# facebookresearch/robust_cvd

Hardware: AMD Instinct MI355X
Metric: GN/LM iterations/sec (and ms/iter) on 300-frame 384x224 video, 1/2/4/8 GPU (higher is better)
Workload: dtype f64

## Files before the change

include/cvd_hip_debug.h:

```cpp
#ifndef CVD_HIP_DEBUG_H
#define CVD_HIP_DEBUG_H

#include "cvd_hip.h"

#ifdef __cplusplus
extern "C" {
#endif

typedef struct cvd_debug_options {
  uint64_t struct_size;
  int32_t force_iterations;
  int32_t force_sharded_path;
  int32_t pcg_lockstep;
  int32_t stall_fused_tail_once;
  int32_t tail_no_row_staging;
  int32_t tail_closes_scalars;
  int32_t asm_force_stage_depth;
  int32_t asm_force_part_units;
} cvd_debug_options;
void cvd_debug_options_default(cvd_debug_options* o);
int32_t cvd_set_debug_options(cvd_handle* h, const cvd_debug_options* o);

int32_t cvd_set_generic_kernels(cvd_handle* h, int32_t enabled);

int32_t cvd_comm_init_local_group(cvd_handle* h, int32_t rank, int32_t world, uint64_t group_key);
int32_t cvd_comm_init_phantom(cvd_handle* h, int32_t rank, int32_t world);

int32_t cvd_block_inverse_debug(cvd_handle* h, int32_t num_blocks, int32_t block_size, const double* a, int32_t variant,
                                float* inverse, int32_t* failed);

int32_t cvd_epipolar_debug(cvd_handle* h, int32_t num_pairs, const int64_t* offsets, const float* loc, double pixel_scale,
                           double threshold_px, int32_t iterations, uint64_t seed, uint8_t* is_static_out,
                           double* fundamental_out, int32_t* best_out, int32_t* counts_out, double* hypotheses_out);
int32_t cvd_flow_masks_debug(cvd_handle* h, int32_t num_frames, int32_t height, int32_t width, int32_t channels,
                             const float* color, int32_t num_pairs, const int32_t* pair_frames, const float* flow_ab,
                             const float* flow_ba, float flow_thresh, float color_thresh, uint8_t* mask_ab, uint8_t* mask_ba,
                             int32_t* kept, float* errors, double* kernel_ms, int32_t pixels_per_thread);
int32_t cvd_dense_inverse_debug(cvd_handle* h, int32_t n, const double* a, double* inverse, int32_t* failed);
int32_t cvd_coarse_debug(cvd_handle* h, int32_t* num_unknowns, double* a_c, double* a_c_inverse, int32_t* failed);
int32_t cvd_temporal_debug(cvd_handle* h, int32_t* dims6, double* a_t, double* a_t_inverse, double* lam, int32_t* failed);
int32_t cvd_product_launch_debug(cvd_handle* h, int32_t* out6);
int32_t cvd_assembly_launch_debug(cvd_handle* h, int32_t* out8, double* cost_frame);

#ifdef __cplusplus
}
#endif
#endif
```

robust_cvd_amd/api.py:

```python
import collections
import ctypes as C
import os
import sys

from . import build as _build
from .binding import Binding
from .ctypes_types import OptParams, SolveSummary, XformDesc

_lib = None
_variant = None


class SolverOptions(C.Structure):
    _fields_ = [
        ("struct_size", C.c_uint64),
        ("pcg_relative_tolerance", C.c_double),
        ("pcg_max_iterations", C.c_int32),
        ("verbose", C.c_int32),
        ("coarse_level", C.c_int32),
        ("robust_loss", C.c_int32),
        ("dense_matrix_free", C.c_int32),
        ("block_inverse_variant", C.c_int32),
        ("coarse_dense_max_unknowns", C.c_int32),
        ("coarse_rebuild_excess", C.c_int32),
        ("coarse_update_budget", C.c_int64),
        ("coarse_dense_shift", C.c_double),
        ("constraint_order", C.c_int32),
        ("coarse_rebuild_excess_dense", C.c_int32),
        ("pcg_fused_tail", C.c_int32),
        ("coarse_dense_row_split", C.c_int32),
        ("dist_owner_update", C.c_int32),
        ("temporal_level", C.c_int32),
        ("temporal_step", C.c_int32),
        ("temporal_grid_x", C.c_int32),
        ("temporal_grid_y", C.c_int32),
        ("coarse_temporal_step", C.c_int32),
        ("coarse_over_budget", C.c_int32),
        ("coarse_temporal_min_frames", C.c_int32),
        ("temporal_weight", C.c_double),
    ]


class DebugOptions(C.Structure):
    _fields_ = [
        ("struct_size", C.c_uint64),
        ("force_iterations", C.c_int32),
        ("force_sharded_path", C.c_int32),
        ("pcg_lockstep", C.c_int32),
        ("stall_fused_tail_once", C.c_int32),
        ("tail_no_row_staging", C.c_int32),
        ("tail_closes_scalars", C.c_int32),
        ("asm_force_stage_depth", C.c_int32),
        ("asm_force_part_units", C.c_int32),
    ]


class ConsistencyDesc(C.Structure):
    _fields_ = [
        ("struct_size", C.c_uint64),
        ("precision", C.c_int32),
        ("num_frames", C.c_int32),
        ("num_pairs", C.c_int32),
        ("height", C.c_int32),
        ("width", C.c_int32),
        ("distance_type", C.c_int32),
        ("have_warp", C.c_int32),
        ("reserved", C.c_int32),
        ("lambda_reprojection", C.c_double),
        ("lambda_disparity", C.c_double),
        ("lambda_depth_ratio", C.c_double),
        ("distance_scale", C.c_double),
        ("distance_alpha", C.c_double),
    ]


class SceneFlowDesc(C.Structure):
    _fields_ = [
        ("struct_size", C.c_uint64),
        ("precision", C.c_int32),
        ("num_frames", C.c_int32),
        ("num_pairs", C.c_int32),
        ("height", C.c_int32),
        ("width", C.c_int32),
        ("distance_type_static", C.c_int32),
        ("distance_type_smooth", C.c_int32),
        ("have_warp", C.c_int32),
        ("lambda_static", C.c_double),
        ("lambda_smooth_reprojection", C.c_double),
        ("lambda_smooth_disparity", C.c_double),
        ("lambda_smooth_depth_ratio", C.c_double),
        ("distance_scale", C.c_double),
        ("distance_alpha", C.c_double),
    ]


class SpatialDesc(C.Structure):
    _fields_ = [
        ("struct_size", C.c_uint64),
        ("precision", C.c_int32),
        ("num_frames", C.c_int32),
        ("frames_per_sample", C.c_int32),
        ("height", C.c_int32),
        ("width", C.c_int32),
        ("reserved", C.c_int32),
        ("lambda_disparity_smooth", C.c_double),
        ("sigma_color_grad", C.c_double),
        ("lambda_contrast_loss", C.c_double),
        ("contrast_thresh", C.c_double),
    ]


class ParamDesc(C.Structure):
    _fields_ = [
        ("struct_size", C.c_uint64),
        ("precision", C.c_int32),
        ("num_tensors", C.c_int32),
    ]


class ParamRecord(C.Structure):
    _fields_ = [
        ("beta1", C.c_double),
        ("beta2", C.c_double),
        ("eps", C.c_double),
        ("grad_decay", C.c_double),
        ("param_decay", C.c_double),
        ("step", C.c_double),
        ("denom_scale", C.c_double),
        ("rule", C.c_int32),
        ("reserved", C.c_int32),
    ]


class DatasetDesc(C.Structure):
    _fields_ = [
        ("struct_size", C.c_uint64),
# ... 2245 lines not shown
                          + [(C.c_void_p * n)(*[d.value for d in group]) for group in outs],
                          ([(dgx, gx)] if input_gradient else []) + [(d, a) for group, arrays in zip(outs, (gw, gg, gb))
                                                                     for d, a in zip(group, arrays)])
        return gx, gw, gg, gb

    def midas_backbone(self, images, weights, norms, blocks=RESNEXT101_32X8D[0], groups=RESNEXT101_32X8D[1],
                       width_per_group=RESNEXT101_32X8D[2], eps=RESNEXT_EPS, kernel_ms=None):
        import numpy as np
        images = np.asarray(images)
        weights = [np.asarray(a) for a in weights]
        norms = [[np.asarray(a) for a in four] for four in norms]
        self._midas_f32("midas_backbone", [images] + weights + [a for four in norms for a in four])
        B, H, W, table, out_shapes = resnext_check_backbone(images.shape, blocks, groups, width_per_group, [a.shape for a in weights],
                                                            [[a.shape for a in four] for four in norms], eps)
        outs = [np.zeros(s, np.float32) for s in out_shapes]
        n = len(table)
        with _DeviceArrays() as dev:
            di = dev.upload(np.ascontiguousarray(images))
            dw = (C.c_void_p * n)(*[dev.upload(np.ascontiguousarray(a)).value for a in weights])
            dn = (C.c_void_p * (4 * n))(*[dev.upload(np.ascontiguousarray(a)).value for four in norms for a in four])
            douts = [dev.alloc(o.nbytes) for o in outs]
            do = (C.c_void_p * 4)(*[d.value for d in douts])
            args = (self._h, C.c_int32(B), C.c_int32(H), C.c_int32(W), (C.c_int32 * 4)(*[int(b) for b in blocks]), C.c_int32(groups),
                    C.c_int32(width_per_group), C.c_float(eps), di, dw, dn, do, None)
            if kernel_ms is None:
                self._check(self._fn("midas_backbone_device")(*args))
            else:
                ms = (C.c_double * (2 * n + 1))()
                self._check(self._fn("midas_backbone_timed")(*args, ms))
                kernel_ms[:] = list(ms)
            if _hip_runtime().hipDeviceSynchronize() != 0:
                raise RuntimeError("midas_backbone: the device reported an error")
            for d, o in zip(douts, outs):
                dev.download(d, o)
        return outs

    def num_active_constraints(self):
        return int(self._lib.cvd_num_active_constraints(self._h))

    def block_inverse_debug(self, blocks, variant=0):
        import numpy as np
        a = np.ascontiguousarray(blocks, dtype=np.float64)
        n, B, B2 = a.shape
        assert B == B2
        out = np.zeros((n, B, B), dtype=np.float32)
        fl = C.c_int32(0)
        self._check(self._fn("block_inverse_debug")(self._h, C.c_int32(n), C.c_int32(B), a.ctypes.data_as(C.POINTER(C.c_double)),
                                                    C.c_int32(variant), out.ctypes.data_as(C.POINTER(C.c_float)), C.byref(fl)))
        return out, fl.value

    def dense_inverse_debug(self, a):
        import numpy as np
        a = np.ascontiguousarray(a, dtype=np.float64)
        n = a.shape[0]
        assert a.shape == (n, n)
        out = np.zeros((n, n), dtype=np.float64)
        fl = C.c_int32(0)
        self._check(self._fn("dense_inverse_debug")(self._h, C.c_int32(n), a.ctypes.data_as(C.POINTER(C.c_double)),
                                                    out.ctypes.data_as(C.POINTER(C.c_double)), C.byref(fl)))
        return out, fl.value

    def temporal_debug(self):
        import numpy as np
        dims = (C.c_int32 * 6)()
        self._check(self._fn("temporal_debug")(self._h, dims, None, None, None, None))
        if dims[0] == 0:
            return None
        n = dims[0]
        a = np.zeros((n, n))
        ai = np.zeros((n, n))
        lam = np.zeros(self.num_frames * self.block_size())
        fl = C.c_int32(0)
        dp = lambda x: x.ctypes.data_as(C.POINTER(C.c_double))
        self._check(self._fn("temporal_debug")(self._h, dims, dp(a), dp(ai), dp(lam), C.byref(fl)))
        return {"NT": n, "S": dims[1], "nn": dims[2], "step": dims[3], "Sx": dims[4], "Sy": dims[5], "a_t": a, "a_t_inverse": ai,
                "lam": lam, "failed": fl.value}

    def path_info(self):
        out = (C.c_int32 * 8)()
        self._check(self._fn("path_info")(self._h, out))
        form = {-1: "none", 0: "exact sparse factor", 1: "exact dense inverse", 2: "temporal pose level"}[out[1]]
        return {"pose_graph_level": form, "depth_grid_level": bool(out[2]), "fused_tail": bool(out[3] & 1), "tail_rows_staged": bool(out[3] & 2),
                "product_sums_shares": bool(out[3] & 4), "rz_shares": out[3] >> 8,
                "tail_disabled": bool(out[4]),
                "taps": out[5], "work_items": out[6], "cross_blocks": bool(out[7])}

    def product_launch_debug(self):
        out = (C.c_int32 * 6)()
        self._check(self._fn("product_launch_debug")(self._h, out))
        kind = {-1: "none", 0: "generic list", 1: "fast list", 2: "fast dense", 3: "cross blocks"}[out[3]]
        return {"threads": out[0], "spec": out[1], "kd": out[2], "kind": out[3], "kind_name": kind, "work_items": out[4],
                "num_cu": out[5]}

    def assembly_launch_debug(self):
        import numpy as np
        out = (C.c_int32 * 8)()
        cost = np.zeros(self.num_frames, dtype=np.float64)
        self._check(self._fn("assembly_launch_debug")(self._h, out, cost.ctypes.data_as(C.POINTER(C.c_double))))
        kind = {-1: "none", 0: "generic", 1: "fast list", 2: "fast dense", 3: "dense fold"}[out[3]]
        return {"threads": out[0], "spec": out[1], "kd": out[2], "kind": out[3], "kind_name": kind, "workgroups": out[4],
                "split_parts": out[5], "stage_depth": out[6], "segments": out[7], "cost_frame": cost}

    def coarse_debug(self):
        import numpy as np
        n = C.c_int32(0)
        self._check(self._fn("coarse_debug")(self._h, C.byref(n), None, None, None))
        if n.value == 0:
            return None
        a = np.zeros((n.value, n.value))
        ai = np.zeros((n.value, n.value))
        fl = C.c_int32(0)
        self._check(self._fn("coarse_debug")(self._h, C.byref(n), a.ctypes.data_as(C.POINTER(C.c_double)),
                                             ai.ctypes.data_as(C.POINTER(C.c_double)), C.byref(fl)))
        return {"a_c": a, "a_c_inverse": ai, "failed": fl.value}
```

robust_cvd_amd/csrc/cvd_api.hip:

```cpp
#include "cvd_host.h"
#include "cvd_coarse.h"

namespace cvd {

static void poseOptimizationStep(cvd_handle* h, const cvd_opt_params& p, double depthDeformReg) {
  solve(h, p, depthDeformReg, PK_POSE_STEP);
  paramsToPoses(h, p);
}

static void poseOptimization(cvd_handle* h, const cvd_opt_params& p) {
  posesToParams(h);
  h->records.clear();
  int ctfRows = p.ctf_long, ctfCols = p.ctf_short;
  int dsoRows = p.dso_long, dsoCols = p.dso_short;
  if (h->aspect >= 1.f) {
    std::swap(ctfCols, ctfRows);
    std::swap(dsoCols, dsoRows);
  }
  int initGrid[3] = {1, 1, 1};
  if (h->ddesc.depth_type == CVD_DEPTH_GRID)
    for (int i = 0; i < 3; ++i) initGrid[i] = h->ddesc.grid_size[i];
  const int Nval = (h->ddesc.depth_type == CVD_DEPTH_IDENTITY) ? 0 : valueNumParams(h->ddesc.value_xform);
  size_t nDmax = static_cast<size_t>(h->nD());
  if (p.coarse_to_fine && h->ddesc.depth_type != CVD_DEPTH_IDENTITY && p.num_steps > 1)
// ... 175 lines not shown
  p->focal_reg = 1.0;
  p->coarse_to_fine = 1;
  p->ctf_long = 17;
  p->ctf_short = 10;
  p->dso_long = 4;
  p->dso_short = 3;
  p->focal_long = 0.3461538376301239;
  p->intr_opt = CVD_INTR_PER_FRAME;
  p->normalize_depth_from_first_frame = 1;
}

void cvd_solver_options_default(cvd_solver_options* o) {
  o->struct_size = CVD_STRUCT_STAMP(cvd_solver_options);
  o->pcg_relative_tolerance = 1e-3;
  o->pcg_max_iterations = 300;
  o->verbose = 0;
  o->coarse_level = 1;
  o->robust_loss = 0;
  o->dense_matrix_free = 0;
  o->block_inverse_variant = 0;
  o->coarse_dense_max_unknowns = 4096;
  o->coarse_rebuild_excess = 16;
  o->coarse_update_budget = 40000;
  o->coarse_dense_shift = 1e-5;
  o->constraint_order = 1;
  o->coarse_rebuild_excess_dense = 0;
  o->pcg_fused_tail = 1;
  o->coarse_dense_row_split = 5;
  o->dist_owner_update = 1;
  o->temporal_level = 1;
  o->temporal_step = 32;
  o->temporal_grid_x = 0;
  o->temporal_grid_y = 0;
  o->coarse_temporal_step = 8;
  o->coarse_over_budget = 0;
  o->coarse_temporal_min_frames = 128;
  o->temporal_weight = 0.7;
}
int32_t cvd_set_solver_options(cvd_handle* h, const cvd_solver_options* o) {
  CVD_TRY(h, {
    if (o->struct_size != CVD_STRUCT_STAMP(cvd_solver_options))
      throw std::runtime_error(fmt("cvd_solver_options: struct_size %#llx != %#llx = sizeof | revision << 32 (caller built against "
                                   "another cvd_hip.h; start from cvd_solver_options_default)",
                                   static_cast<unsigned long long>(o->struct_size),
                                   static_cast<unsigned long long>(CVD_STRUCT_STAMP(cvd_solver_options))));
    if (o->pcg_fused_tail < 0 || o->pcg_fused_tail > 1) throw std::runtime_error("pcg_fused_tail in {0, 1}");
    if (!(o->pcg_relative_tolerance > 0.0 && o->pcg_relative_tolerance < 1.0)) throw std::runtime_error("pcg_relative_tolerance must lie in (0, 1)");
    if (o->pcg_max_iterations < 1) throw std::runtime_error("pcg_max_iterations must be >= 1");
    if (!(o->coarse_dense_shift >= 0.0 && o->coarse_dense_shift < 1.0)) throw std::runtime_error("coarse_dense_shift must lie in [0, 1)");
    if (o->coarse_rebuild_excess < 0 || o->coarse_rebuild_excess_dense < -1 || o->coarse_update_budget < 0)
      throw std::runtime_error("coarse_rebuild_excess / coarse_update_budget must be >= 0, coarse_rebuild_excess_dense >= -1");
    if (o->coarse_dense_max_unknowns < 0 || o->coarse_dense_max_unknowns > kDenseCoarseMaxUnknowns)
      throw std::runtime_error(fmt("coarse_dense_max_unknowns must lie in [0, %d] (what k_dense_spd_inverse holds in registers)",
                                   kDenseCoarseMaxUnknowns));
    if (o->coarse_level < 0 || o->coarse_level > 3 || o->coarse_temporal_step < 2 || o->robust_loss < 0 || o->robust_loss > 1 || o->block_inverse_variant < 0 ||
        o->block_inverse_variant > 2)
      throw std::runtime_error("coarse_level in {0, 1, 2, 3}, coarse_temporal_step >= 2, robust_loss in {0, 1}, block_inverse_variant in {0, 1, 2}");
    if (o->coarse_over_budget < 0 || o->coarse_over_budget > 1) throw std::runtime_error("coarse_over_budget in {0, 1}");
    if (o->coarse_temporal_min_frames < 0) throw std::runtime_error("coarse_temporal_min_frames must be >= 0");
    if (!(o->temporal_weight > 0.0 && o->temporal_weight <= 2.0)) throw std::runtime_error("temporal_weight must lie in (0, 2]");
    if (o->coarse_dense_row_split < 0 || o->coarse_dense_row_split > 8) throw std::runtime_error("coarse_dense_row_split must lie in [0, 8]");
    if (o->temporal_level < 0 || o->temporal_level > 2 || o->temporal_step < 2 || o->temporal_grid_x < 0 || o->temporal_grid_y < 0 ||
        o->temporal_grid_x == 1 || o->temporal_grid_y == 1)
      throw std::runtime_error("temporal_level in {0, 1, 2}, temporal_step >= 2, temporal_grid_x / _y 0 (automatic) or >= 2");
    if (o->coarse_update_budget != h->opt.coarse_update_budget || o->coarse_dense_max_unknowns != h->opt.coarse_dense_max_unknowns ||
        (o->coarse_level == 3) != (h->opt.coarse_level == 3) || o->coarse_temporal_step != h->opt.coarse_temporal_step ||
        o->coarse_over_budget != h->opt.coarse_over_budget || o->coarse_temporal_min_frames != h->opt.coarse_temporal_min_frames ||
        o->pcg_fused_tail != h->opt.pcg_fused_tail)
      h->tableValid = false;
    if (o->constraint_order != h->opt.constraint_order) h->orderGx = h->orderGy = -1;
    h->opt = *o;
  });
}
void cvd_debug_options_default(cvd_debug_options* o) {
  o->struct_size = CVD_STRUCT_STAMP(cvd_debug_options);
  o->force_iterations = 0;
  o->force_sharded_path = 0;
  o->pcg_lockstep = 0;
  o->stall_fused_tail_once = 0;
  o->tail_no_row_staging = 0;
  o->tail_closes_scalars = 0;
  o->asm_force_stage_depth = 0;
  o->asm_force_part_units = 0;
}
int32_t cvd_set_debug_options(cvd_handle* h, const cvd_debug_options* o) {
  CVD_TRY(h, {
    if (o->struct_size != CVD_STRUCT_STAMP(cvd_debug_options))
      throw std::runtime_error("cvd_debug_options: struct_size does not match this library's cvd_hip_debug.h (start from cvd_debug_options_default)");
    if (o->asm_force_stage_depth < 0 || o->asm_force_stage_depth > 3) throw std::runtime_error("asm_force_stage_depth in {0, 1, 2, 3}");
    if (o->asm_force_part_units < 0) throw std::runtime_error("asm_force_part_units >= 0");
    if (o->asm_force_part_units != h->dbg.asm_force_part_units) h->tableValid = false;
    h->dbg = *o;
    h->distForced = h->world == 1 && (h->comm != nullptr || h->localGroup || h->phantom) && o->force_sharded_path != 0;
  });
}
void cvd_comm_unique_id(uint8_t* out128) {
  ncclUniqueId id;
  std::memset(&id, 0, sizeof(id));
  (void)ncclGetUniqueId(&id);
  std::memcpy(out128, &id, sizeof(id));
}
int32_t cvd_comm_init(cvd_handle* h, int32_t rank, int32_t world, const uint8_t* id128) {
  CVD_TRY(h, {
    if (world < 1 || rank < 0 || rank >= world) throw std::runtime_error("invalid rank / world size");
    if (h->comm) { NCCL_CHECK(ncclCommDestroy(h->comm)); h->comm = nullptr; }
    ncclUniqueId id;
    std::memcpy(&id, id128, sizeof(id));
    NCCL_CHECK(ncclCommInitRank(&h->comm, world, id, rank));
    h->rank = rank;
    h->world = world;
    h->localGroup.reset();
    h->distForced = world == 1 && h->dbg.force_sharded_path != 0;
    h->tableValid = false;
  });
}
int32_t cvd_comm_init_local_group(cvd_handle* h, int32_t rank, int32_t world, uint64_t group_key) {
  CVD_TRY(h, {
    if (world < 1 || rank < 0 || rank >= world) throw std::runtime_error("invalid rank / world size");
    if (h->comm) { NCCL_CHECK(ncclCommDestroy(h->comm)); h->comm = nullptr; }
    h->localGroup = joinLocalGroup(group_key, world);
    h->rank = rank;
    h->world = world;
    h->distForced = world == 1 && h->dbg.force_sharded_path != 0;
    h->tableValid = false;
  });
}
int32_t cvd_comm_init_phantom(cvd_handle* h, int32_t rank, int32_t world) {
  CVD_TRY(h, {
    if (world < 1 || rank < 0 || rank >= world) throw std::runtime_error("invalid rank / world size");
    if (h->comm) { NCCL_CHECK(ncclCommDestroy(h->comm)); h->comm = nullptr; }
    if (h->localGroup) { leaveLocalGroup(*h->localGroup); h->localGroup.reset(); }
    h->phantom = true;
    h->rank = rank;
    h->world = world;
    h->distForced = world == 1;
    h->tableValid = false;
  });
}
int32_t cvd_set_generic_kernels(cvd_handle* h, int32_t enabled) { CVD_TRY(h, h->forceGeneric = enabled != 0); }

int32_t cvd_set_video(cvd_handle* h, int32_t numFrames, int32_t width, int32_t height, float aspect, float invAspect) {
  CVD_TRY(h, {
    if (numFrames <= 0 || width <= 0 || height <= 0) throw std::runtime_error("invalid video dimensions");
    h->F = numFrames; h->W = width; h->H = height; h->aspect = aspect; h->invAspect = invAspect;
    h->haveDynMasks = false;
    h->adaptGx = h->adaptGy = 0;
    h->dDepth.ensure(static_cast<size_t>(numFrames) * width * height);
    HIP_CHECK(hipMemsetAsync(h->dDepth.p, 0, static_cast<size_t>(numFrames) * width * height * sizeof(float), h->stream));
    h->median.assign(numFrames, 0.f);
    h->medianDirty = true;
    h->poses.assign(numFrames, cvd_frame_pose{{0, 0, 0}, {0, 0, 0, 1}, 0.f, 0.f});
    h->poseParamsValid = false;
    cvd_xform_desc dd{};
    dd.type = CVD_XFORM_DEPTH;
    dd.depth_type = CVD_DEPTH_IDENTITY;
    cvd_xform_desc sd{};
    sd.type = CVD_XFORM_SPATIAL;
    sd.spatial_type = CVD_SPATIAL_IDENTITY;
    resetXforms(h, dd, false);
    resetXforms(h, sd, true);
    h->tableValid = false;
    h->P = 0;
    h->C = 0;
    h->dense = false;
    h->denseListValid = false;
    h->haveTriplets = false;
// ... 732 lines not shown
    if (variant < 0 || variant > 2) throw std::runtime_error("block_inverse_debug: variant must be 0, 1 or 2");
    const size_t n = static_cast<size_t>(num_blocks) * block_size * block_size;
    DevBuf<double> dA;
    DevBuf<double> dL;
    DevBuf<float> dM;
    DevBuf<int> dF;
    dA.ensure(n);
    dL.ensure(static_cast<size_t>(num_blocks) * block_size);
    dM.ensure(n);
    dF.ensure(1);
    hipStream_t s = h->stream;
    dA.upload(a, n, s);
    HIP_CHECK(hipMemsetAsync(dL.p, 0, static_cast<size_t>(num_blocks) * block_size * sizeof(double), s));
    HIP_CHECK(hipMemsetAsync(dM.p, 0, n * sizeof(float), s));
    HIP_CHECK(hipMemsetAsync(dF.p, 0, sizeof(int), s));
    Layout L{};
    L.F = num_blocks;
    L.B = block_size;
    launchBlockInverseRaw(h, L, dA.p, dL.p, dM.p, dF.p, variant);
    int fl = 0;
    dM.download(inverse, n, s);
    dF.download(&fl, 1, s);
    HIP_CHECK(hipStreamSynchronize(s));
    if (failed) *failed = fl;
  });
}

int32_t cvd_epipolar_debug(cvd_handle* h, int32_t num_pairs, const int64_t* offsets, const float* loc, double pixel_scale,
                           double threshold_px, int32_t iterations, uint64_t seed, uint8_t* is_static_out,
                           double* fundamental_out, int32_t* best_out, int32_t* counts_out, double* hypotheses_out) {
  CVD_TRY(h, epipolarStaticFlags(h, num_pairs, offsets, loc, pixel_scale, threshold_px, iterations, seed, is_static_out,
                                 fundamental_out, best_out, nullptr, counts_out, hypotheses_out));
}

int32_t cvd_dense_inverse_debug(cvd_handle* h, int32_t n, const double* a, double* inverse, int32_t* failed) {
  CVD_TRY(h, {
    if (n <= 0 || n > 8192) throw std::runtime_error("dense_inverse_debug: bad size");
    const size_t nn = static_cast<size_t>(n) * n;
    DevBuf<double> dA;
    DevBuf<double> dM;
    DevBuf<int> dF;
    dA.ensure(nn);
    dM.ensure(nn);
    dF.ensure(2);
    hipStream_t s = h->stream;
    dA.upload(a, nn, s);
    HIP_CHECK(hipMemsetAsync(dM.p, 0, nn * sizeof(double), s));
    HIP_CHECK(hipMemsetAsync(dF.p, 0, 2 * sizeof(int), s));
    launchDenseSpdInverse(h, n, dA.p, dM.p, dF.p, s, dF.p + 1);
    int fl[2] = {0, 0};
    dM.download(inverse, nn, s);
    dF.download(fl, 2, s);
    HIP_CHECK(hipStreamSynchronize(s));
    if (failed) *failed = fl[0];
  });
}

int32_t cvd_temporal_debug(cvd_handle* h, int32_t* dims6, double* a_t, double* a_t_inverse, double* lam, int32_t* failed) {
  CVD_TRY(h, {
    auto& T = h->temporal;
    hipStream_t s = h->stream;
    const bool on = T.on && T.built;
    const int dims[6] = {on ? T.NT : 0, T.S, T.nn, T.step, T.Sx, T.Sy};
    for (int i = 0; i < 6; ++i) dims6[i] = dims[i];
    if (on) {
      const size_t n2 = static_cast<size_t>(T.NT) * T.NT;
      if (a_t) T.A.download(a_t, n2, s);
      if (a_t_inverse) T.Ainv.download(a_t_inverse, n2, s);
      if (lam) h->dLam.download(lam, static_cast<size_t>(h->F) * h->Bsz(), s);
      int fl = 0;
      T.fail.download(&fl, 1, s);
      HIP_CHECK(hipStreamSynchronize(s));
      if (failed) *failed = fl;
    }
  });
}
int32_t cvd_path_info(cvd_handle* h, int32_t* out8) {
  CVD_TRY(h, {
    out8[0] = h->coarseOn ? 1 : 0;
    out8[1] = !h->coarseOn ? -1 : (h->coarse.temporalPose ? 2 : (h->coarse.denseMode ? 1 : 0));
    out8[2] = h->temporal.on ? 1 : 0;
    out8[3] = h->lastFusedTail ? (h->tailStageRows ? 3 : 1) : 0;
    if (h->lastFusedTail && h->lastShares) out8[3] |= 4 | (h->lastShareCount << 8);
    out8[4] = h->tailDisabled ? 1 : 0;
    out8[5] = h->lastKD;
    out8[6] = static_cast<int32_t>(h->itemFa.size());
    out8[7] = h->lastCross ? 1 : 0;
  });
}
int32_t cvd_product_launch_debug(cvd_handle* h, int32_t* out6) {
  CVD_TRY(h, {
    for (int i = 0; i < 6; ++i) out6[i] = h->lastProduct[i];
  });
}
int32_t cvd_assembly_launch_debug(cvd_handle* h, int32_t* out8, double* cost_frame) {
  CVD_TRY(h, {
    for (int i = 0; i < 8; ++i) out8[i] = h->lastAssembly[i];
    const size_t F = static_cast<size_t>(h->F);
    if (cost_frame && h->lastAssembly[3] >= 0 && h->dCostFrame.n >= F) {
      h->dCostFrame.download(cost_frame, F, h->stream);
      HIP_CHECK(hipStreamSynchronize(h->stream));
    }
  });
}
int32_t cvd_coarse_debug(cvd_handle* h, int32_t* num_unknowns, double* a_c, double* a_c_inverse, int32_t* failed) {
  CVD_TRY(h, {
    auto& C = h->coarse;
    if (!C.valid || !h->coarseOn) {
      *num_unknowns = 0;
    } else if (C.temporalPose) {
      const size_t n = static_cast<size_t>(C.ptN);
      *num_unknowns = static_cast<int32_t>(n);
      hipStream_t s = h->stream;
      int fl = 0;
      C.fail.download(&fl, 1, s);
      if (a_c) C.ptMat.download(a_c, n * n, s);
      if (a_c_inverse) C.ptInv.download(a_c_inverse, n * n, s);
      HIP_CHECK(hipStreamSynchronize(s));
      if (failed) *failed = fl;
    } else {
      const int F = h->F;
      const size_t n = static_cast<size_t>(F) * kCB;
      *num_unknowns = static_cast<int32_t>(n);
      hipStream_t s = h->stream;
      int fl = 0;
      C.fail.download(&fl, 1, s);
      if (a_c_inverse) {
        std::vector<double> save(n), unit(n, 0.0);
        C.rc.download(save.data(), n, s);
        HIP_CHECK(hipStreamSynchronize(s));
        DevBuf<double> scalTmp;
        scalTmp.ensure(S_COUNT);
        HIP_CHECK(hipMemsetAsync(scalTmp.p, 0, S_COUNT * sizeof(double), s));
        for (size_t k = 0; k < n; ++k) {
          unit[k] = 1.0;
          C.rc.upload(unit.data(), n, s);
          if (C.denseMode) {
            hipLaunchKernelGGL(k_coarse_dense_apply, dim3(F), dim3(256), 0, s, F, C.denseInv.p, C.rc.p, C.c.p, C.modeActive.p,
                               C.dotPart.p, scalTmp.p, h->dCounters.p + 3, C.fail.p, 1, 0.0, static_cast<double*>(nullptr));
          } else {
            hipLaunchKernelGGL(k_coarse_apply_w, dim3(F), dim3(1024), 0, s, C.plan, C.Wb.p, C.rc.p, C.y.p, C.dotPart.p,
                               scalTmp.p, h->dCounters.p + 3, C.fail.p, 1, 0.0, static_cast<double*>(nullptr));
            hipLaunchKernelGGL(k_coarse_apply_wt, dim3(F), dim3(256), 0, s, coarseView(h, true, true), F, C.c.p,
                               scalTmp.p, 1);
          }
          C.c.download(a_c_inverse + k * n, n, s);
          HIP_CHECK(hipStreamSynchronize(s));
          unit[k] = 0.0;
        }
        C.rc.upload(save.data(), n, s);
        HIP_CHECK(hipStreamSynchronize(s));
      }
      std::vector<double> diag(static_cast<size_t>(F) * kCBB), edges(static_cast<size_t>(std::max(C.nEdges, 1)) * kCBB);
      std::vector<unsigned char> act(n);
      std::vector<int> efa(C.nEdges), efb(C.nEdges);
      C.diag.download(diag.data(), diag.size(), s);
      C.edges.download(edges.data(), static_cast<size_t>(C.nEdges) * kCBB, s);
      C.modeActive.download(act.data(), n, s);
      C.edgeFa.download(efa.data(), efa.size(), s);
      C.edgeFb.download(efb.data(), efb.size(), s);
      HIP_CHECK(hipStreamSynchronize(s));
      if (failed) *failed = fl;
      if (a_c) {
        std::fill(a_c, a_c + n * n, 0.0);
        for (int f = 0; f < F; ++f)
          for (int i = 0; i < kCB; ++i)
// ... 16 lines not shown
```

robust_cvd_amd/csrc/cvd_cost.h:

```cpp
#pragma once

#include "cvd_kernels.h"

namespace cvd {

template <int KD, int KS>
inline __global__ __launch_bounds__(256) void k_cost_items(Layout L, Table T, Items it, const double* __restrict__ x,
                                                    const FrameConst* __restrict__ fc, double* __restrict__ costItem) {
  extern __shared__ __attribute__((aligned(16))) double sm[];
  const int B = L.B;
  double* xa = sm;
  double* xb = sm + B;
  FrameConst* fcs = reinterpret_cast<FrameConst*>(sm + 2 * B);
  double* red = reinterpret_cast<double*>(fcs + 2);
  const int item = blockIdx.x;
  const int fa = it.fa[item], fb = it.fb[item];
  for (int i = threadIdx.x; i < B; i += blockDim.x) {
    xa[i] = x[static_cast<size_t>(fa) * B + i];
    xb[i] = x[static_cast<size_t>(fb) * B + i];
  }
  if (threadIdx.x < 2 * (sizeof(FrameConst) / 8)) {
    const int which = threadIdx.x / (sizeof(FrameConst) / 8);
    const int k = threadIdx.x % (sizeof(FrameConst) / 8);
    reinterpret_cast<double*>(fcs + which)[k] = reinterpret_cast<const double*>(fc + (which ? fb : fa))[k];
  }
  __syncthreads();
  double acc = 0.0;
  for (int dir = 0; dir < 2; ++dir) {
    const long long cb = it.range[item * 4 + dir * 2], ce = it.range[item * 4 + dir * 2 + 1];
    const FrameConst& Fs = fcs[dir];
    const FrameConst& Ft = fcs[dir ^ 1];
    const double* xs = dir ? xb : xa;
    const double* xt = dir ? xa : xb;
    for (long long c = cb + threadIdx.x; c < ce; c += blockDim.x) {
      const float2 d = T.dsrc[c];
      if (d.x > 0.f) {
        Sample<KD, KS> s;
        evalSample<KD, KS, false>(L, Fs, Ft, xs, xt, T.ndc[c], d, s);
        acc += s.rho0;
      }
    }
  }
  acc = waveSum(acc);
  if ((threadIdx.x & 63) == 0) red[threadIdx.x >> 6] = acc;
  __syncthreads();
  if (threadIdx.x == 0) {
    double t = 0.0;
    for (int w = 0; w < (blockDim.x >> 6); ++w) t += red[w];
    costItem[item] = 0.5 * t;
  }
}

template <int KD>
inline __global__ __launch_bounds__(256) void k_cost_frames(Layout L, const double* __restrict__ x,
                                                     const float* __restrict__ median,
                                                     const unsigned char* __restrict__ inRange,
                                                     const unsigned char* __restrict__ rangeFlags,
                                                     double* __restrict__ costFrame) {
  extern __shared__ __attribute__((aligned(16))) double sm[];
  __shared__ double red[4];
  const int f = blockIdx.x;
  double acc = 0.0;
  if (threadIdx.x == 0 && L.positionRegSqrt > 0.0) {
    double o3[3] = {0, 0, 0}, dg = 0.0, cst = 0.0;
    if (posRegValid(L, rangeFlags, f)) posRegFrame(L, rangeFlags, f, x, nullptr, o3, dg, cst);
    acc += cst;
  }
  const bool active = inRange[f] != 0;
  if (active)
    for (int i = threadIdx.x; i < L.B; i += 256) sm[i] = x[static_cast<size_t>(f) * L.B + i];
  __syncthreads();
  if (active) {
    const float med = median[f];
    const int nr = numRegResiduals<KD>(L);
    for (int i = threadIdx.x; i < nr; i += 256) {
      double r;
      int n;
      int cols[2 * KD + 2];
      double jac[2 * KD + 2];
      regResidual<KD>(L, f, i, sm, med, r, n, cols, jac);
      acc += r * r;
    }
  }
  acc = waveSum(acc);
  if ((threadIdx.x & 63) == 0) red[threadIdx.x >> 6] = acc;
  __syncthreads();
  if (threadIdx.x == 0) costFrame[f] = 0.5 * ((red[0] + red[1]) + (red[2] + red[3]));
}

inline __global__ __launch_bounds__(256) void k_sum2(const double* __restrict__ a, int na, const double* __restrict__ b,
                                              int nb, double* __restrict__ out, int slot) {
  __shared__ double red[4];
  double acc = 0.0;
  for (int i = threadIdx.x; i < na; i += 256) acc += a[i];
  for (int i = threadIdx.x; i < nb; i += 256) acc += b[i];
  acc = waveSum(acc);
  if ((threadIdx.x & 63) == 0) red[threadIdx.x >> 6] = acc;
  __syncthreads();
  if (threadIdx.x == 0) out[slot] = red[0] + red[1] + red[2] + red[3];
}

template <int KD, bool DENSE = false>
inline __global__ __launch_bounds__(256) void k_cost_items_fast(Layout L, Table T, Items it, const double* __restrict__ x,
                                                         const FrameConst* __restrict__ fc, double* __restrict__ costItem) {
  extern __shared__ __attribute__((aligned(16))) double sm[];
  const int B = L.B;
  double* xa = sm;
  double* xb = sm + B;
  FrameConst* fcs = reinterpret_cast<FrameConst*>(sm + 2 * B);
  double* red = reinterpret_cast<double*>(fcs + 2);
  const int item = blockIdx.x;
  const int tid = threadIdx.x;
  const int fa = it.fa[item], fb = it.fb[item];
  for (int i = tid; i < B; i += 256) {
    xa[i] = x[static_cast<size_t>(fa) * B + i];
    xb[i] = x[static_cast<size_t>(fb) * B + i];
  }
  constexpr int FCW = sizeof(FrameConst) / 8;
  if (tid < 2 * FCW) {
    const int which = tid / FCW, k = tid % FCW;
    reinterpret_cast<double*>(fcs + which)[k] = reinterpret_cast<const double*>(fc + (which ? fb : fa))[k];
  }
  __syncthreads();
  const int N = L.N;
  const double A = L.aspect;
  double acc = 0.0;
  for (int dir = 0; dir < 2; ++dir) {
    const long long cb = it.range[item * 4 + dir * 2], ce = it.range[item * 4 + dir * 2 + 1];
    const FrameConst& Fa = fcs[dir];
    const FrameConst& Fb = fcs[dir ^ 1];
    const double* xs = dir ? xb : xa;
    const double* xt = dir ? xa : xb;
    const double fya = Fa.fy, fxa = Fa.fy * A;
    const double fyb = Fb.fy;
    const double ifyb = 1.0 / fyb, ifxb = 1.0 / (fyb * A);
    const int fsrc = dir ? fb : fa, ftgt = dir ? fa : fb;
    const long long pixBase = DENSE ? (cb / (static_cast<long long>(T.W) * T.H)) * (static_cast<long long>(T.W) * T.H) : 0;
    std::conditional_t<DENSE, DenseStreamAhead, RecordStream<false>> rs;
    const int nDir = static_cast<int>(ce - cb);
    if constexpr (DENSE) rs.prime(T, cb, tid, 256, nDir, pixBase, fsrc, ftgt);
    else rs.prime(T, cb, tid, nDir);
    for (int ci = tid; ci < nDir; ci += 256) {
      float4 nd;
      float2 d;
      if (!rs.take(T, cb, ci, 256, nDir, pixBase, fsrc, ftgt, nd, d)) continue;
      const double da = static_cast<double>(d.x), db = static_cast<double>(d.y);
      double Da, Db;
      if (N == 0) {
        Da = da;
        Db = db;
      } else {
        FastTaps<KD> ta, tb;
        fastGather<KD>(L, nd.x, nd.y, ta);
        fastGather<KD>(L, nd.z, nd.w, tb);
        Da = 0.0;
        Db = 0.0;
#pragma unroll
        for (int k = 0; k < KD; ++k) {
          if (ta.ok(k)) {
            const int ia = ta.I(k);
            const double wa = ta.Wt(k);
            Da += (N == 2 ? da * xs[7 + ia * 2] + xs[7 + ia * 2 + 1] : da * xs[7 + ia]) * wa;
          }
          if (tb.ok(k)) {
            const int ib = tb.I(k);
            const double wb = tb.Wt(k);
            Db += (N == 2 ? db * xt[7 + ib * 2] + xt[7 + ib * 2 + 1] : db * xt[7 + ib]) * wb;
          }
        }
      }
      const double pax = static_cast<double>(nd.x), pay = static_cast<double>(nd.y);
      const double pbx = static_cast<double>(nd.z), pby = static_cast<double>(nd.w);
      double ca[3], Rca[3];
      fastRay(Fa.R, pax, pay, fxa, fya, ca, Rca);
      const double v[3] = {Fa.t[0] + Rca[0] * Da - Fb.t[0], Fa.t[1] + Rca[1] * Da - Fb.t[1], Fa.t[2] + Rca[2] * Da - Fb.t[2]};
      double zz, iz, u, vv, r0, r1, r2, dr2dA, dr2dDb;
      fastProject<false>(L, Fb.R, v, ifxb, ifyb, pbx, pby, zz, iz, u, vv, r0, r1);
      fastDepthResidual<false>(L, L.lossType, zz, iz, Db, r2, dr2dA, dr2dDb);
      double rho0, rho1;
      robustRho(L, r0 * r0 + r1 * r1 + r2 * r2, rho0, rho1);
      acc += rho0;
    }
  }
  acc = waveSum(acc);
  if ((tid & 63) == 0) red[tid >> 6] = acc;
  __syncthreads();
  if (tid == 0) costItem[item] = 0.5 * ((red[0] + red[1]) + (red[2] + red[3]));
}

inline __global__ __launch_bounds__(256) void k_step_stats(size_t n, const double* __restrict__ dx,
                                                    const double* __restrict__ g, const double* __restrict__ r,
                                                    const double* __restrict__ lam, const double* __restrict__ x,
                                                    const double* __restrict__ hdiagActive, double* __restrict__ scal,
                                                    double* __restrict__ part, unsigned int* __restrict__ counter) {
  constexpr int NQ = 7;
  __shared__ double red[NQ][4];
  __shared__ int flag;
  const int G = gridDim.x;
  double a[NQ] = {0, 0, 0, 0, 0, 0, 0};
  for (size_t i = static_cast<size_t>(blockIdx.x) * 256 + threadIdx.x; i < n; i += static_cast<size_t>(G) * 256) {
    const double d = dx[i];
    a[0] += d * g[i];
    a[1] += d * r[i];
    a[2] += d * lam[i] * d;
    a[3] += d * d;
    if (hdiagActive[i] != 0.0) { a[4] += x[i] * x[i]; a[6] += 1.0; }
    a[5] = fmax(a[5], fabs(g[i]));
  }
#pragma unroll
  for (int k = 0; k < NQ; ++k)
    if (k != 5) a[k] = waveSum(a[k]);
#pragma unroll
  for (int off = 32; off > 0; off >>= 1) a[5] = fmax(a[5], __shfl_xor(a[5], off, 64));
  if ((threadIdx.x & 63) == 0)
    for (int k = 0; k < NQ; ++k) red[k][threadIdx.x >> 6] = a[k];
  __syncthreads();
  if (threadIdx.x < NQ) {
    const int k = threadIdx.x;
    part[k * G + blockIdx.x] = (k != 5) ? (red[k][0] + red[k][1]) + (red[k][2] + red[k][3])
                                        : fmax(fmax(red[5][0], red[5][1]), fmax(red[5][2], red[5][3]));
  }
  if (!lastBlockArrives(counter, G, &flag)) return;
  double t[NQ] = {0, 0, 0, 0, 0, 0, 0};
  for (int b = threadIdx.x; b < G; b += 256) {
#pragma unroll
    for (int k = 0; k < NQ; ++k)
      if (k != 5) t[k] += part[k * G + b];
    t[5] = fmax(t[5], part[5 * G + b]);
  }
#pragma unroll
  for (int k = 0; k < NQ; ++k)
    if (k != 5) t[k] = waveSum(t[k]);
#pragma unroll
  for (int off = 32; off > 0; off >>= 1) t[5] = fmax(t[5], __shfl_xor(t[5], off, 64));
  if ((threadIdx.x & 63) == 0)
    for (int k = 0; k < NQ; ++k) red[k][threadIdx.x >> 6] = t[k];
  __syncthreads();
  if (threadIdx.x == 0) {
    scal[S_DG] = red[0][0] + red[0][1] + red[0][2] + red[0][3];
    scal[S_DR] = red[1][0] + red[1][1] + red[1][2] + red[1][3];
    scal[S_DLD] = red[2][0] + red[2][1] + red[2][2] + red[2][3];
    scal[S_DD] = red[3][0] + red[3][1] + red[3][2] + red[3][3];
    scal[S_XX] = red[4][0] + red[4][1] + red[4][2] + red[4][3];
    scal[S_GMAX] = fmax(fmax(red[5][0], red[5][1]), fmax(red[5][2], red[5][3]));
    scal[S_NACTIVE] = red[6][0] + red[6][1] + red[6][2] + red[6][3];
  }
}

}
```

robust_cvd_amd/csrc/cvd_eval.hip:

```cpp
#include "cvd_host.h"
#include "cvd_cost.h"
#include "cvd_assembly.h"
#include "cvd_triplets.h"
#include "cvd_dense_walk.h"

namespace cvd {

void launchFrameConsts(Ctx& c, const double* x) {
  launchFrameConsts(c.L, x, c.h->dFc.p, c.h->stream);
  HIP_CHECK(hipGetLastError());
}

void spinStream(hipStream_t s) {
  hipError_t e;
  while ((e = hipStreamQuery(s)) == hipErrorNotReady) {}
  HIP_CHECK(e);
}
void spinEvent(hipEvent_t ev) {
  hipError_t e;
  while ((e = hipEventQuery(ev)) == hipErrorNotReady) {}
  HIP_CHECK(e);
}
void readScalars(Ctx& c) {
  HIP_CHECK(hipMemcpyAsync(c.h->hScal, c.h->dScal.p, S_COUNT * sizeof(double), hipMemcpyDeviceToHost, c.h->stream));
  spinStream(c.h->stream);
}

void enqueueCost(Ctx& c, const double* x) {
  cvd_handle* h = c.h;
  hipStream_t s = h->stream;
  launchFrameConsts(c, x);
  const int slot = h->tBegin(KC_COST);
  if (c.L.includeStatic && c.nItems > 0) {
    const size_t lds = (2 * c.L.B) * 8 + 2 * sizeof(FrameConst) + 8 * 8;
    const bool fast = !h->forceGeneric && c.KS == 0 && fastLoss(c.L);
    if (fast) {
      CVD_DISPATCH_KD(c.KD, {
        if (h->dense) {
          allowLds((k_cost_items_fast<KD, true>), lds);
          hipLaunchKernelGGL((k_cost_items_fast<KD, true>), dim3(c.nItems), dim3(256), lds, s, c.L, c.T, c.it, x, h->dFc.p,
                             h->dCostItem.p);
        } else {
          allowLds((k_cost_items_fast<KD, false>), lds);
          hipLaunchKernelGGL((k_cost_items_fast<KD, false>), dim3(c.nItems), dim3(256), lds, s, c.L, c.T, c.it, x, h->dFc.p,
                             h->dCostItem.p);
        }
      });
    } else {
      CVD_DISPATCH(c.KD, c.KS, {
        allowLds(k_cost_items<KD, KS>, lds);
        hipLaunchKernelGGL((k_cost_items<KD, KS>), dim3(c.nItems), dim3(256), lds, s, c.L, c.T, c.it, x, h->dFc.p,
                           h->dCostItem.p);
      });
    }
    HIP_CHECK(hipGetLastError());
  }
  CVD_DISPATCH_KD(c.KD, {
    hipLaunchKernelGGL((k_cost_frames<KD>), dim3(c.L.F), dim3(256), static_cast<size_t>(c.L.B) * 8, s, c.L, x, h->dMedian.p, h->dRegOwner.p, h->dInRange.p,
                       h->dCostFrame.p);
  });
  HIP_CHECK(hipGetLastError());
  if (c.trip && c.TT.nGroups > 0) {
    CVD_DISPATCH(c.KD, c.KS, {
      hipLaunchKernelGGL((k_cost_triplets<KD, KS>), dim3(c.TT.nGroups), dim3(256), 0, s, c.L, c.TT, x, h->dFc.p,
                         h->dCostFrame.p);
    });
    HIP_CHECK(hipGetLastError());
  }
  hipLaunchKernelGGL(k_sum2, dim3(1), dim3(256), 0, s, h->dCostItem.p, (c.L.includeStatic ? c.nItems : 0),
                     h->dCostFrame.p, c.L.F, h->dScal.p, S_COST);
  HIP_CHECK(hipGetLastError());
  if (h->dist()) commAllReduce(h, h->dScal.p + S_COST, 1, CT_F64, s);
  h->tEnd(slot);
}
double evalCost(Ctx& c, const double* x) {
  enqueueCost(c, x);
  readScalars(c);
  return c.h->hScal[S_COST];
}

void enqueueStats(Ctx& c) {
  cvd_handle* h = c.h;
  const int G = static_cast<int>(std::min<size_t>(128, (c.n + 511) / 512));
  h->dStatPart.ensure(7 * 128);
  hipLaunchKernelGGL(k_step_stats, dim3(G), dim3(256), 0, h->stream, c.n, h->dDx.p, h->dG.p, h->dR.p, h->dLam.p,
                     h->dX.p, h->dHd.p, h->dScal.p, h->dStatPart.p, h->dCounters.p + 2);
  HIP_CHECK(hipGetLastError());
}

bool crossScope(cvd_handle* h, const Ctx& c) {
  const bool off = h->opt.dense_matrix_free != 0;
  return h->dense && !off && !h->forceGeneric && c.L.includeStatic && !h->xFa.empty() && c.KS == 0 && fastLoss(c.L) &&
         c.L.N == 1 && c.L.nD > 0 && (c.KD == 4 || (c.KD == 1 && c.L.nD == 1)) && c.L.intrOpt != CVD_INTR_SHARED && !c.trip && !(c.L.positionRegSqrt > 0.0) &&
         c.L.B <= 256 && (static_cast<size_t>(c.L.B) * (c.L.B + 1) / 2 + 2 * c.L.B + 4 * 36) * 8 <= kMaxLds &&
         dwLdsBytes(c.L.nD, c.L.B, kDwThreads) <= kMaxLds;
}
CrossPairs crossPairs(cvd_handle* h) {
  return CrossPairs{h->dXFa.p, h->dXFb.p, h->dXRange.p, h->dXSlot.p, static_cast<int>(h->xFa.size())};
}
DenseRecords denseRecords(cvd_handle* h) {
  return DenseRecords{h->dDwRecords.p, h->dDwRecOff.p, h->dFpOff.p, h->dFpList.p};
}
void launchDenseWalk(Ctx& c, const double* x) {
  cvd_handle* h = c.h;
  const int G = c.L.nD, B = c.L.B;
  h->dDwRecords.ensure(static_cast<size_t>(std::max(1, h->nDwRecords)) * dwRecordDoubles(G));
  h->dDwGg.ensure(static_cast<size_t>(std::max<long long>(1, h->C)));
  if (h->nDwRecords == 0) return;
  const size_t lds = dwLdsBytes(G, B, kDwThreads);
  const DenseWalkList wl{h->dDwPair.p, h->nDwRecords, denseLaneMap(h->W, h->H)};
  allowLds((k_dense_walk<4>), lds);
  const int slot = h->tBegin(KC_DENSE_WALK);
  hipLaunchKernelGGL((k_dense_walk<4>), dim3(h->nDwRecords), dim3(kDwThreads), lds, h->stream, c.L, c.T, wl, x, h->dFc.p,
                     h->dDwRecords.p, h->dDwGg.p);
  h->tEnd(slot);
  HIP_CHECK(hipGetLastError());
}
void launchCrossAssemble(Ctx& c, const double* x) {
  (void)x;
  cvd_handle* h = c.h;
  const size_t B = c.L.B, G = c.L.nD;
  h->dXBlocks.ensure(h->xFa.size() * B * B);
  const unsigned nP = static_cast<unsigned>(h->xFa.size());
  if (nP == 0) return;
  hipLaunchKernelGGL(k_dense_fold_cross, dim3(nP), dim3(256), 0, h->stream, c.L, crossPairs(h), h->dXDir.p, h->dDwRecOff.p,
                     h->dDwRecords.p, h->dXBlocks.p);
  int panelW = static_cast<int>(((kMaxLds - 4096) / 8) / G);
  panelW = std::max(1, std::min<int>(panelW, static_cast<int>(G)));
  const int nPanels = static_cast<int>((G + panelW - 1) / panelW);
  panelW = static_cast<int>((G + nPanels - 1) / nPanels);
  const size_t ldsGrid = static_cast<size_t>(panelW) * G * 8;
  allowLds((k_dense_gg<4>), ldsGrid);
  const int slot = h->tBegin(KC_DENSE_GG);
  for (int dir = 0; dir < 2; ++dir)
    hipLaunchKernelGGL((k_dense_gg<4>), dim3(nP, nPanels), dim3(kGgThreads), ldsGrid, h->stream, c.L, c.T, crossPairs(h), h->dXDir.p,
                       h->dDwGg.p, panelW, dir, h->dXBlocks.p);
  h->tEnd(slot);
  HIP_CHECK(hipGetLastError());
}

double evalFull(Ctx& c, const double* x, bool withStats, bool noReadBack) {
  cvd_handle* h = c.h;
  hipStream_t s = h->stream;
  launchFrameConsts(c, x);
  const size_t B = c.L.B;
  const int slot = h->tBegin(KC_ASSEMBLE);
  const bool fast = !h->forceGeneric && c.KS == 0 && fastLoss(c.L);
  const size_t ldsFast = (B * (B + 1) / 2 + 2 * B + 4 * 36) * 8;
  const size_t ldsRest = 3 * B * 8 + 2 * sizeof(FrameConst) + 4 * 36 * 8;
  int panelCap = 0;
  const bool fastFits = ldsFast <= kMaxLds;
  auto recordAsm = [h](int threads, int spec, int kd, int kind, int groups, int splitParts, int stageDepth = -1, int segments = 0) {
    const int v[8] = {threads, spec, kd, kind, groups, splitParts, stageDepth, segments};
    for (int i = 0; i < 8; ++i) h->lastAssembly[i] = v[i];
  };
  if (fast && fastFits) {
    h->dAsmScratch.ensure(static_cast<size_t>(h->nAsmSlots) * (B * (B + 1) / 2 + B + 4));
    const AsmWork work{h->dAsmParts.p, h->dAsmUnits.p, h->dAsmScratch.p, h->dAsmCount.p};
    const int spec = (!h->dense && c.L.N == 1 && c.L.lossType == CVD_STATIC_REPRO_DISPARITY && c.L.intrOpt != CVD_INTR_SHARED)
                         ? (c.L.robustKind == 0 ? 1 : 2) : 0;
    const size_t ldsRow = static_cast<size_t>(kAsmThreads / 64) * B * 8;
    const bool segWalk = spec != 0 && kAsmThreads > 64;
    int depth = ldsFast + ldsRow <= kMaxLds ? 1 : 0;
    if (segWalk && ldsFast + 2 * ldsRow <= kMaxLds) depth = 2;
    if (segWalk && h->dbg.asm_force_stage_depth != 0) {
      const int forced = h->dbg.asm_force_stage_depth - 1;
      if (forced < 0 || forced > 2 || ldsFast + forced * ldsRow > kMaxLds)
        throw std::runtime_error(fmt("asm_force_stage_depth: %d staging rows per wave do not fit the LDS at B = %d", forced, static_cast<int>(B)));
      depth = forced;
    }
    const size_t ldsStage = ldsFast + static_cast<size_t>(depth) * ldsRow;
    const bool stage = depth > 0;
    const AsmSegs segs{h->dAsmSegs.p, h->dAsmWaveOff.p, depth};
    if (segWalk && !h->dAsmWaveOff.p) throw std::logic_error("assembly: the segment list of the work list is missing");
#define CVD_LAUNCH_ASM_S(DENSEV, STAGEV, SPECV)                                                                            \
    CVD_DISPATCH_KD(c.KD, {                                                                                              \
      if (SPECV != 0 && kAsmThreads > 64) recordAsm(kAsmThreads, SPECV, KD, 1, h->nAsmParts, h->nAsmSlots, depth, h->nAsmSegs); \
      else recordAsm(kAsmThreads, SPECV, KD, DENSEV ? 2 : 1, h->nAsmParts, h->nAsmSlots);                                  \
      allowLds((k_assemble_fast<KD, DENSEV, STAGEV, false, SPECV>), STAGEV ? ldsStage : ldsFast);                          \
      hipLaunchKernelGGL((k_assemble_fast<KD, DENSEV, STAGEV, false, SPECV>), dim3(h->nAsmParts),                          \
                         dim3(kAsmThreads), STAGEV ? ldsStage : ldsFast, s,                                                \
                         c.L, c.T, x, h->dFc.p, h->dMask.p, h->dMedian.p, h->dRegOwner.p, h->dInRange.p, work, h->dG.p, h->dH.p,  \
                         h->dCostFrame.p, h->dFocal.p, h->dFocal.p + c.L.F, asmSegsAsArgument(segs));                    \
    })
#define CVD_LAUNCH_ASM(DENSEV, STAGEV) CVD_LAUNCH_ASM_S(DENSEV, STAGEV, 0)
#ifndef CVD_ASM_STAGE
#define CVD_ASM_STAGE 1
#endif
    if (c.cross) {
      launchDenseWalk(c, x);
      recordAsm(kAsmThreads, 0, c.KD, 3, c.L.F, 0);
      if (c.KD == 1) {
        allowLds((k_assemble_fast<1, true, false, true>), ldsFast);
        hipLaunchKernelGGL((k_assemble_fast<1, true, false, true>), dim3(c.L.F), dim3(kAsmThreads), ldsFast, s, c.L, c.T, x, h->dFc.p,
                           h->dMask.p, h->dMedian.p, h->dRegOwner.p, h->dInRange.p, work, h->dG.p, h->dH.p, h->dCostFrame.p,
                           h->dFocal.p, h->dFocal.p + c.L.F, denseRecords(h));
      } else {
        allowLds((k_assemble_fast<4, true, false, true>), ldsFast);
        hipLaunchKernelGGL((k_assemble_fast<4, true, false, true>), dim3(c.L.F), dim3(kAsmThreads), ldsFast, s, c.L, c.T, x, h->dFc.p,
                           h->dMask.p, h->dMedian.p, h->dRegOwner.p, h->dInRange.p, work, h->dG.p, h->dH.p, h->dCostFrame.p,
                           h->dFocal.p, h->dFocal.p + c.L.F, denseRecords(h));
      }
    } else if (h->dense) { if (stage && CVD_ASM_STAGE) CVD_LAUNCH_ASM(true, true); else CVD_LAUNCH_ASM(true, false); }
    else if (spec == 1) { if (stage && CVD_ASM_STAGE) CVD_LAUNCH_ASM_S(false, true, 1); else CVD_LAUNCH_ASM_S(false, false, 1); }
    else if (spec == 2) { if (stage && CVD_ASM_STAGE) CVD_LAUNCH_ASM_S(false, true, 2); else CVD_LAUNCH_ASM_S(false, false, 2); }
    else { if (stage && CVD_ASM_STAGE) CVD_LAUNCH_ASM(false, true); else CVD_LAUNCH_ASM(false, false); }
#undef CVD_LAUNCH_ASM
#undef CVD_LAUNCH_ASM_S
  } else {
    if (h->dense && c.L.includeStatic) throw std::logic_error("dense mode: the generic assembly has no images to read (DenseListScope should have taken this solve)");
    const AsmPanels panels = makePanels(static_cast<int>(B), (kMaxLds - ldsRest) / 8, panelCap);
    const size_t lds = static_cast<size_t>(panelCap) * 8 + ldsRest;
    recordAsm(256, 0, c.KD, 0, c.L.F, 0);
    CVD_DISPATCH(c.KD, c.KS, {
      allowLds(k_assemble<KD, KS>, lds);
      hipLaunchKernelGGL((k_assemble<KD, KS>), dim3(c.L.F), dim3(256), lds, s, c.L, c.T, x, h->dFc.p, h->dMask.p,
                         h->dMedian.p, h->dRegOwner.p, h->dInRange.p, h->dFpOff.p, h->dFpList.p, h->dG.p, h->dH.p, h->dCostFrame.p,
                       h->dFocal.p, h->dFocal.p + c.L.F, panels, panelCap);
    });
  }
  HIP_CHECK(hipGetLastError());
  if (c.trip && c.TT.nGroups > 0) {
    int panelCapT = 0;
    const AsmPanels panelsT = makePanels(static_cast<int>(B), (kMaxLds - B * 8 - 256) / 8, panelCapT);
    const size_t ldsT = (static_cast<size_t>(panelCapT) + B) * 8;
    CVD_DISPATCH(c.KD, c.KS, {
      allowLds(k_assemble_triplets<KD, KS>, ldsT);
      hipLaunchKernelGGL((k_assemble_triplets<KD, KS>), dim3(c.L.F), dim3(256), ldsT, s, c.L, c.TT, x, h->dFc.p,
                         h->dMask.p, h->dFtOff.p, h->dFtList.p, h->dG.p, h->dH.p, h->dFocal.p, h->dFocal.p + c.L.F,
                         panelsT, panelCapT);
      hipLaunchKernelGGL((k_cost_triplets<KD, KS>), dim3(c.TT.nGroups), dim3(256), 0, s, c.L, c.TT, x, h->dFc.p,
                         h->dCostFrame.p);
    });
    HIP_CHECK(hipGetLastError());
  }
  if (c.L.intrOpt == CVD_INTR_SHARED) {
    hipLaunchKernelGGL(k_shared_focal_fixup, dim3(1), dim3(256), 0, s, c.L, h->dFocal.p, h->dFocal.p + c.L.F, h->dMask.p,
                       h->dG.p, h->dH.p);
    HIP_CHECK(hipGetLastError());
  }
  if (c.cross) launchCrossAssemble(c, x);
  h->tEnd(slot);
  if (h->dist()) {
    const int ct = h->tBegin(KC_COMM_EVAL);
    const size_t chunkH = static_cast<size_t>(h->ownChunk()) * B * B;
    commGroupStart(h);
    commAllReduce(h, h->dG.p, c.n, CT_F64, s);
    commAllReduce(h, h->dCostFrame.p, c.L.F, CT_F64, s);
    commReduceScatter(h, h->dH.p, h->dH.p + static_cast<size_t>(h->rank) * chunkH, chunkH, CT_F64, s);
    commGroupEnd(h);
    Layout own = c.L;
    own.F = h->ownCount();
    if (own.F > 0)
      hipLaunchKernelGGL(k_extract_diag, dim3((static_cast<size_t>(own.F) * B + 255) / 256), dim3(256), 0, s, own,
                         h->dH.p + static_cast<size_t>(h->ownFirst()) * B * B, h->dHd.p + static_cast<size_t>(h->ownFirst()) * B);
    const size_t chunkD = static_cast<size_t>(h->ownChunk()) * B;
    commAllGather(h, h->dHd.p + static_cast<size_t>(h->rank) * chunkD, h->dHd.p, chunkD, CT_F64, s);
    h->tEnd(ct);
  } else {
    hipLaunchKernelGGL(k_extract_diag, dim3((c.n + 255) / 256), dim3(256), 0, s, c.L, h->dH.p, h->dHd.p);
  }
  hipLaunchKernelGGL(k_sum2, dim3(1), dim3(256), 0, s, h->dCostFrame.p, c.L.F, h->dCostFrame.p, 0, h->dScal.p, S_COST);
  HIP_CHECK(hipGetLastError());
  if (noReadBack) return 0.0;
  if (withStats) {
    HIP_CHECK(hipMemsetAsync(h->dLam.p, 0, c.n * sizeof(double), s));
    enqueueStats(c);
  }
  readScalars(c);
  return h->hScal[S_COST];
}

void touchModule_eval() {
  hipFuncAttributes a;
  (void)hipFuncGetAttributes(&a, reinterpret_cast<const void*>(k_sum2));
}

}

#ifdef CVD_ASM_PROFILE
extern "C" int32_t cvd_debug_asm_profile(unsigned long long* out) {
  (void)hipDeviceSynchronize();
  return hipMemcpyFromSymbol(out, HIP_SYMBOL(cvd::g_asmProf), sizeof(unsigned long long) * 2048 * 16) == hipSuccess ? 0 : 1;
}
extern "C" int32_t cvd_debug_asm_waits(unsigned long long* out) {
  (void)hipDeviceSynchronize();
  return hipMemcpyFromSymbol(out, HIP_SYMBOL(cvd::g_asmWait), sizeof(unsigned long long) * 2048 * 8 * 8) == hipSuccess ? 0 : 1;
}
#endif
```

robust_cvd_amd/csrc/cvd_host.h:

```cpp
#pragma once

#include <hip/hip_runtime.h>
#include <hip/hip_ext.h>
#include <rccl/rccl.h>
#include <rocblas/rocblas.h>
#include <rocsolver/rocsolver.h>

#include <algorithm>
#include <array>
#include <atomic>
#include <chrono>
#include <condition_variable>
#include <cmath>
#include <cstdarg>
#include <cstdint>
#include <cstdio>
#include <cstdlib>
#include <cstring>
#include <functional>
#include <limits>
#include <map>
#include <memory>
#include <mutex>
#include <set>
// ... 234 lines not shown
  bool tableIgnoresStatic = false;
  long long numValid = 0;

  std::vector<cvd_frame_pose> poses;
  cvd_xform_desc ddesc{}, sdesc{};
  std::vector<double> dparams, sparams;
  std::vector<std::array<double, 7>> poseParams;
  bool poseParamsValid = false;

  DevBuf<double> dX, dXc, dG, dLam, dMask, dScale, dDx, dR, dR1, dZ, dP0, dP1, dQ, dH, dQPart;
  DevBuf<float> dMinv;
  DevBuf<double> dFdot, dCostItem, dCostFrame, dScal, dHd, dFocal;
  DevBuf<double> dStatPart;
  DevBuf<unsigned char> dDynMask;
  DevBuf<double> dAdaptW;
  int dynW = 0, dynH = 0, adaptGx = 0, adaptGy = 0;
  bool haveDynMasks = false;
  std::shared_ptr<Frontend> frontend;

  struct CoarseHost {
    bool valid = false;
    int nEdges = 0, nBlocks = 0, nLevels = 0;
    std::vector<int> itemEdge;
    DevBuf<int> order, pos, levelPtr, levelCols, lvlBlkPtr, lvlBlks, blkCol, blkRow, colPtr, rowPtr, rowBlk, updPtr, updBlk,
        updA, updB, edgeBlk, edgeFa, edgeFb, wPtr, wRow, wtPtr, wtBlk, wtCol, wtFrame, wuPtr, wuL, wuW, itemEdgeDev, wSlot;
    DevBuf<double> edges, diag, Lb, Linv, Wb, rc, qc, y, c, dotPart, fdotY, wq, dropDiag;
    bool sparsified = false;
    bool temporalPose = false;
    int ptNn = 0, ptStepFrames = 0, ptN = 0, ptBlocks = 0;
    std::vector<int> edgeFaHost, edgeFbHost;
    DevBuf<int> ptA, ptB, ptPtr, ptList;
    DevBuf<double> ptMat, ptInv, ptR, ptT, ptDot, ptRec;
    DevBuf<TlStep> ptStepDev;
    std::vector<unsigned char> ptStepHost;
    DevBuf<unsigned int> ptCounter;
    bool denseMode = false;
    int denseForB = 0;
    bool denseReady = false;
    DevBuf<double> denseA, densePanel;
    DevBuf<double> denseInv;
    DevBuf<int> denseValid;
    int nW = 0;
    DevBuf<unsigned char> modeActive;
    DevBuf<int> fail;
    DevBuf<unsigned int> barrier;
    bool ptInvPending = false;
    int* ptInvFail = nullptr;
    DevBuf<double> Wb2;
    DevBuf<int> fail2;
    CoarsePlan plan{};
  } coarse;
  bool coarseOn = false;
  struct TemporalHost {
    bool on = false;
    bool built = false;
    int S = 0, Sx = 0, Sy = 0, nn = 0, step = 0, NT = 0, width = 0, nGroups = 0, nBlocks = 0;
    std::vector<unsigned char> stepHost;
    int tabGx = 0, tabGy = 0, tabSx = 0, tabSy = 0;
    int grpF = 0, grpStep = 0;
    std::vector<int> grpFa, grpFb;
    DevBuf<float> hx, hy, elW;
    DevBuf<int> bx, by, gOff, gItems, blkA, blkB, gPtr, gather, fail, valid;
    DevBuf<float4> vW;
    DevBuf<unsigned int> vIdx, counter;
    DevBuf<unsigned char> elV;
    DevBuf<double> Cf, E, part, A, Ainv, sq, rT, t, tl, dotPart, rec;
    DevBuf<double> invPanel;
    DevBuf<unsigned int> invBarrier;
    DevBuf<TlStep> stepDev;
    hipEvent_t evIn = nullptr, evDone = nullptr;
    bool sidePending = false;
    double* sqPtr = nullptr;
  } temporal;
  hipEvent_t evRebuild[2] = {nullptr, nullptr};
  bool rebuildTimed = false;
  double coarseRebuildMs = 0.0, pcgIterMs = 0.0;
  std::vector<std::pair<int, int>> globalEdges;
  bool haveGlobalEdges = false;
  DevBuf<double> dRegJac;
  DevBuf<unsigned short> dRegCol;
  DevBuf<unsigned char> dRegCnt;
  RegCache regCache{};
  DevBuf<FrameConst> dFc;
  DevBuf<int> dFail;
  DevBuf<unsigned long long> dCount;
  double* hScal = nullptr;
  double* hStage[2] = {nullptr, nullptr};
  size_t hStageN[2] = {0, 0};
  double* hPcg = nullptr;
  hipEvent_t pcgEvent[2] = {nullptr, nullptr};

  cvd_solve_summary summary{};
  std::vector<cvd_iteration_record> records;

  bool lastFusedTail = false, lastCross = false;
  bool lastShares = false;
  int lastShareCount = 0;
  int sharesF = -1, sharesN = -1;
  bool tailStageRows = false;
  int lastKD = 0;
  int lastProduct[6] = {0, 0, 0, -1, 0, 0};
  int lastAssembly[8] = {0, 0, 0, -1, 0, 0, -1, 0};
  bool tailDisabled = false;
  bool forceGeneric = false;

  int timing = 0;
  int timingStride = 1;
  long long timingCounter = 0;
  long long timingCounterKc[16] = {0};
  std::vector<std::pair<hipEvent_t, hipEvent_t>> evPool;
  std::vector<int> evClass;
  std::vector<int> evIter;
  int curPcgIter = -1;
  size_t evUsed = 0;
  double kcMs[KC_TOTAL] = {0};
  long long kcN[KC_TOTAL] = {0};

  ~cvd_handle_t() {
    for (auto& e : evPool) { (void)hipEventDestroy(e.first); (void)hipEventDestroy(e.second); }
    if (rbMain) (void)rocblas_destroy_handle(rbMain);
    if (comm) (void)ncclCommDestroy(comm);
    if (localGroup) leaveLocalGroup(*localGroup);
    if (hScal) (void)hipHostFree(hScal);
    for (auto& p : hStage) if (p) (void)hipHostFree(p);
    if (hPcg) (void)hipHostFree(hPcg);
    for (auto& e : pcgEvent) if (e) (void)hipEventDestroy(e);
    for (auto& e : evRebuild) if (e) (void)hipEventDestroy(e);
    if (temporal.evIn) (void)hipEventDestroy(temporal.evIn);
    if (temporal.evDone) (void)hipEventDestroy(temporal.evDone);
    if (evCoarseIn) (void)hipEventDestroy(evCoarseIn);
    if (evCoarseDone) (void)hipEventDestroy(evCoarseDone);
    if (evInvIn) (void)hipEventDestroy(evInvIn);
    if (evInvDone) (void)hipEventDestroy(evInvDone);
    if (stream3) (void)hipStreamDestroy(stream3);
    if (stream2) (void)hipStreamDestroy(stream2);
    if (stream) (void)hipStreamDestroy(stream);
  }

  int nD() const { return xformNumBlocks(ddesc) * xformBlockSize(ddesc); }
  int nS() const { return xformNumBlocks(sdesc) * xformBlockSize(sdesc); }
  int Bsz() const { return 7 + nD() + nS(); }

  int tBegin(int kc) {
    if (kc >= KC_COUNT ? timing == 0 : !(timing & (1 << kc))) return -1;
    if (timingStride > 1 && kc < KC_DENSE_WALK && (timingCounterKc[kc]++ % timingStride) != 0) return -1;
    if (evUsed == evPool.size()) {
      hipEvent_t a, b;
      HIP_CHECK(hipEventCreate(&a));
      HIP_CHECK(hipEventCreate(&b));
      evPool.emplace_back(a, b);
      evClass.push_back(kc);
      evIter.push_back(-1);
    }
    evClass[evUsed] = kc;
    evIter[evUsed] = curPcgIter;
    HIP_CHECK(hipEventRecord(evPool[evUsed].first, stream));
    return static_cast<int>(evUsed++);
  }
  void tEnd(int slot) {
    if (slot >= 0) HIP_CHECK(hipEventRecord(evPool[slot].second, stream));
  }
  int tReserve(int kc, hipEvent_t& start, hipEvent_t& stop) {
    start = nullptr;
    stop = nullptr;
    if (!(timing & (1 << kc))) return -1;
    if (timingStride > 1 && (timingCounter++ % timingStride) != 0) return -1;
    if (evUsed == evPool.size()) {
      hipEvent_t a, b;
      HIP_CHECK(hipEventCreate(&a));
      HIP_CHECK(hipEventCreate(&b));
      evPool.emplace_back(a, b);
      evClass.push_back(kc);
      evIter.push_back(-1);
    }
    evClass[evUsed] = kc;
    evIter[evUsed] = curPcgIter;
    start = evPool[evUsed].first;
    stop = evPool[evUsed].second;
    return static_cast<int>(evUsed++);
  }
  void tDropFrom(size_t firstSlot, int firstDeadIter) {
    for (size_t i = firstSlot; i < evUsed; ++i)
      if (evIter[i] >= firstDeadIter) evClass[i] = -1;
// ... 47 lines not shown
  } while (0)

#define CVD_DISPATCH_KD(KDv, ...)                                  \
  do {                                                             \
    if (KDv == 1) { constexpr int KD = 1; __VA_ARGS__; }            \
    else if (KDv == 4) { constexpr int KD = 4; __VA_ARGS__; }       \
    else { constexpr int KD = 16; __VA_ARGS__; }                    \
  } while (0)

constexpr size_t kMaxLds = 160 * 1024;

template <typename K>
void allowLds(K kernel, size_t bytes) {
  if (bytes > kMaxLds)
    throw std::runtime_error(fmt("per-frame block needs %zu B of LDS (> 160 KiB): frame block too large", bytes));
  if (bytes > 48 * 1024) {
    static std::map<std::pair<int, const void*>, size_t> granted;
    static std::mutex grantedMutex;
    int dev = 0;
    HIP_CHECK(hipGetDevice(&dev));
    std::lock_guard<std::mutex> lock(grantedMutex);
    size_t& g = granted[{dev, reinterpret_cast<const void*>(kernel)}];
    if (bytes > g) {
      HIP_CHECK(hipFuncSetAttribute(reinterpret_cast<const void*>(kernel), hipFuncAttributeMaxDynamicSharedMemorySize,
                                    static_cast<int>(bytes)));
      g = bytes;
    }
  }
}

int liveHandles(int device);
struct PersistentGate {
  static constexpr int kMaxDevices = 64;
  struct Slot { std::mutex m; hipEvent_t ev = nullptr; bool recorded = false; };
  static Slot& slot(int device);
  Slot& sl;
  hipStream_t s;
  PersistentGate(int device, hipStream_t stream) : sl(slot(device)), s(stream) {
    sl.m.lock();
    try {
      if (!sl.ev) HIP_CHECK(hipEventCreateWithFlags(&sl.ev, hipEventDisableTiming));
      if (sl.recorded) HIP_CHECK(hipStreamWaitEvent(s, sl.ev, 0));
    } catch (...) {
      sl.m.unlock();
      throw;
    }
  }
  ~PersistentGate() {
    sl.recorded = hipEventRecord(sl.ev, s) == hipSuccess;
    sl.m.unlock();
  }
};

void commAllReduce(cvd_handle* h, void* buf, size_t count, CommType t, hipStream_t s);
void commReduceScatter(cvd_handle* h, const void* send, void* recv, size_t recvCount, CommType t, hipStream_t s);
void commAllGather(cvd_handle* h, const void* send, void* recv, size_t sendCount, CommType t, hipStream_t s);
void commGroupStart(cvd_handle* h);
void commGroupEnd(cvd_handle* h);
std::vector<int> rangeOf(const cvd_opt_params& p, int F);
void posesToParams(cvd_handle* h);
void paramsToPoses(cvd_handle* h, const cvd_opt_params& params);
void resetXforms(cvd_handle* h, const cvd_xform_desc& d, bool spatial);
void gridXformSplit(cvd_handle* h, const cvd_xform_desc& nd);
Layout makeLayout(cvd_handle* h, const cvd_opt_params& p, double depthDeformReg, ProblemKind kind);
void checkFrameBlock(size_t B, const char* what);
void tapCounts(const Layout& L, int& KD, int& KS);
bool fastLoss(const Layout& L);
Table makeTable(cvd_handle* h);
void checkDenseScope(cvd_handle* h, const Layout& L, int KS, bool trip);
bool denseFastScope(const cvd_handle* h, const Layout& L, int KS, bool trip);
bool denseFastBlockFits(long long B);
struct DenseListScope {
  cvd_handle* h;
  bool entered = false;
  DenseListScope(cvd_handle* h, bool needList);
  ~DenseListScope();
};
bool denseModeSupported(const cvd_opt_params& p, const cvd_xform_desc& dd, const cvd_xform_desc& sd, bool haveTriplets, int world,
                        bool normalize);
AsmPanels makePanels(int B, size_t capDoubles, int& panelCap);
void compileTable(cvd_handle* h, const std::vector<int>& range, bool withTriplets = false, bool ignoreStatic = false);
void orderTable(cvd_handle* h, const Layout& L, int KD);
double* pinnedStage(cvd_handle* h, int which, size_t n);
void uploadState(cvd_handle* h, const Layout& L, DevBuf<double>& dst);
void downloadState(cvd_handle* h, const Layout& L, const DevBuf<double>& src);
void buildMask(cvd_handle* h, const Layout& L, const cvd_opt_params& p, ProblemKind kind, const std::vector<int>& range);
void ensureBuffers(Ctx& c);
void refreshMedians(cvd_handle* h);
void launchFrameConsts(const Layout& L, const double* x, FrameConst* fc, hipStream_t s);
void launchFrameConsts(Ctx& c, const double* x);
void launchFlagToBool(int* flag, hipStream_t s);
void launchTlRowsInit(cvd_handle* h, const TlStep* tsp, int NT, int groups, int F, unsigned int* counter, int closeScalars, double tol2,
                      hipStream_t s);
void spinStream(hipStream_t s);
void spinEvent(hipEvent_t ev);
void readScalars(Ctx& c);
void enqueueCost(Ctx& c, const double* x);
double evalCost(Ctx& c, const double* x);
void enqueueStats(Ctx& c);
bool crossScope(cvd_handle* h, const Ctx& c);
CrossPairs crossPairs(cvd_handle* h);
void launchCrossAssemble(Ctx& c, const double* x);
double evalFull(Ctx& c, const double* x, bool withStats = false, bool noReadBack = false);
bool coarseFusedConsumers();
bool fusedExchange(cvd_handle* h, bool withCoarse);
size_t exchangeOffsetQc(const Ctx& c);
size_t exchangeOffsetPq(const Ctx& c, bool withDenseCoarse);
size_t exchangeTemporalCount(cvd_handle* h, bool withCoarse);
bool ownerShardedUpdate(cvd_handle* h, bool withCoarse);
inline int denseRowSplit(const cvd_handle* h) { return std::min(kCB, std::max(0, h->opt.coarse_dense_row_split)); }
void launchDenseSpdInverse(cvd_handle* h, int n, const double* A, double* out, int* fail, hipStream_t s, int* outValid,
                           DevBuf<double>* panelBuf = nullptr, DevBuf<unsigned int>* barrierBuf = nullptr);
struct DinvRequest {
  int n = 0;
  const double* A = nullptr;
  double* out = nullptr;
  int* fail = nullptr;
  int* outValid = nullptr;
  DevBuf<double>* panelBuf = nullptr;
  DevBuf<unsigned int>* barrierBuf = nullptr;
};
void launchDenseSpdInversePair(cvd_handle* h, const DinvRequest& a, const DinvRequest& b, hipStream_t s);
CoarseView coarseView(cvd_handle* h, bool on, bool walk);
void prepareMatvec(Ctx& c, const double* x);
void launchMatvec(Ctx& c, const double* x, const double* z, const double* pOld, double* pNew, int useBeta, const double* lam,
                  double* q, bool withCoarse = false, bool tailFused = false, int sharesIteration = 0);
bool pcgTailScope(Ctx& c, bool coarse, int nThreads, size_t& lds, int& ldsFinish, int& ldsScratch);
struct PcgShares {
  int count = 0;
  int levelShare0 = 0;
  int levelWg0 = 0;
};
bool pcgSharesScope(Ctx& c, bool coarse, PcgShares& sh);
void launchPcgTail(Ctx& c, const double* x, const double* pOld, double* pNew, int useBeta, const double* lam, double* q,
                   bool withCoarse, int nThreads, size_t lds, int ldsFinish, int ldsScratch, double tol2,
                   const PcgShares* shares = nullptr);
void launchPcgClose(Ctx& c, int enqueued);
void launchBlockInverseRaw(cvd_handle* h, const Layout& L, const double* dH, const double* dLam, float* dMinv, int* dFail, int variant,
                           hipStream_t onStream = nullptr);
void launchBlockInverse(Ctx& c, hipStream_t onStream = nullptr);
void launchCoarseSetup(Ctx& c, const double* x, int side = 0);
bool temporalScope(const Ctx& c);
bool temporalPrepare(Ctx& c);
void launchTemporalSetup(Ctx& c, const double* x, int half);
void launchTemporalInit(Ctx& c, bool closeScalars, double tol2);
TlStep temporalStep(cvd_handle* h);
const TlStep* temporalStepDev(cvd_handle* h);
void poseTemporalPlan(cvd_handle* h);
void poseTemporalPrepare(Ctx& c);
void launchPoseTemporalBuild(Ctx& c, hipStream_t s, int* failOut, bool deferInverse = false);
void launchPoseTemporalInit(Ctx& c, double tol2);
const TlStep* poseTemporalStepDev(cvd_handle* h);
void coarseDebug(cvd_handle* h, int32_t* num_unknowns, double* a_c, double* a_c_inverse, int32_t* failed);
int runPcg(Ctx& c, const double* x, const std::function<void()>& tail = nullptr);
bool wantsTriplets(const cvd_opt_params& p, ProblemKind kind);
void bindTriplets(Ctx& c, const cvd_opt_params& p, ProblemKind kind);
void solve(cvd_handle* h, const cvd_opt_params& p, double depthDeformReg, ProblemKind kind);
void evaluate(cvd_handle* h, const cvd_opt_params& p, double depthDeformReg, const double* pose7, double* cost, int32_t* nres,
              double* gradient, double* hdiag, double* hfull);
void sampleConstraints(cvd_handle* h, bool triplet, int num, const int32_t* keyFrames, const float* corner, const float* flow,
                       const uint8_t* mask, const float* flow2, const uint8_t* mask2, const float* dyn, int dw, int dh,
                       int matchSeparation, float minDynamicDistance, int64_t* offsets);
void getSampledConstraints(cvd_handle* h, bool triplet, float* out);
void denseMaps(cvd_handle* h, int kind, int first, int count, int w, int hh, void* out, double* kernelMs);
void imageOps(cvd_handle* h, int kind, int n, int w, int hh, const void* in, float* out, double* kernelMs);
void touchModule_setup();
void touchModule_eval();
void touchModule_matvec();
void touchModule_precond();
void touchModule_solve();
void touchModule_frontend();
void touchModule_temporal();
void flowGuidedFilter(cvd_handle* h, int n, int first, int count, int w, int hh, int dw, int dh, float invAspect, const float* depth,
                      const float* cameras, const float* flowF, const uint8_t* maskF, const float* flowB, const uint8_t* maskB,
                      int frameRadius, int spatialRadius, int median, float* out, double* kernelMs);
void bilateralFilter(cvd_handle* h, int n, int first, int count, int w, int hh, const float* depth, const float* color,
                     int frameRadius, int spatialRadius, float depthSigma, float colorSigma, int median, float* out,
                     double* kernelMs);
void epipolarStaticFlags(cvd_handle* h, int numPairs, const int64_t* offsets, const float* loc, double pixelScale,
                         double thresholdPx, int iterations, uint64_t seed, uint8_t* isStatic, double* fundamental,
                         int32_t* best, double* kernelMs, int32_t* counts, double* hypotheses);
void computeTracks(cvd_handle* h, int F, int H, int W, float invAspect, const uint8_t* active, int first, int last,
                   const float* corner, const float* dyn, int dh, int dw, const float* flow, const uint8_t* mask,
                   const uint8_t* pairPresent, int spawnDistance, int pruneDistance, float minDynamicDistance,
                   int minTrackLength, int64_t* counts, double* kernelMs);
void getTracks(cvd_handle* h, int32_t* startFrame, int32_t* length, uint8_t* kept, float* loc);
void flowConsistencyMasks(cvd_handle* h, int numFrames, int hh, int w, int channels, const float* color, int numPairs,
                          const int32_t* pairFrames, const float* flowAB, const float* flowBA, float flowThresh,
                          float colorThresh, uint8_t* maskAB, uint8_t* maskBA, int32_t* kept, float* errors, double* kernelMs,
                          int pixelsPerThread);
void consistencyLoss(cvd_handle* h, const cvd_consistency_desc* d, const void* depth, const void* ext, const void* intr,
                     const void* warp, const int32_t* pairFrames, const void* flowAB, const void* flowBA, const void* weightAB,
                     const void* weightBA, double* total, double* terms, void* grad, double* kernelMs);
void consistencyLossDevice(cvd_handle* h, const cvd_consistency_desc* d, const void* depth, const void* ext, const void* intr,
                           const void* warp, const int32_t* pairFrames, const void* flowAB, const void* flowBA,
                           const void* weightAB, const void* weightBA, double* total, double* terms, void* grad, hipStream_t s);
void sceneFlowLoss(cvd_handle* h, const cvd_scene_flow_desc* d, const void* depth, const void* ext, const void* intr,
                   const void* warp, const int32_t* pairFrames, const void* const* flows, const void* const* masks,
                   const int32_t* neighborFrames, const void* const* nflows, const void* const* nmasks, const void* valid,
                   double* total, double* terms, void* grad, void* maps, double* kernelMs);
void sceneFlowLossDevice(cvd_handle* h, const cvd_scene_flow_desc* d, const void* depth, const void* ext, const void* intr,
                         const void* warp, const int32_t* pairFrames, const void* const* flows, const void* const* masks,
                         const int32_t* neighborFrames, const void* const* nflows, const void* const* nmasks, const void* valid,
                         double* total, double* terms, void* grad, void* maps, hipStream_t s);
void spatialLosses(cvd_handle* h, const cvd_spatial_desc* d, const void* depth, const void* depthOrig, const void* image,
                   double* total, double* smooth, double* contrast, void* grad, double* kernelMs);
void spatialLossesDevice(cvd_handle* h, const cvd_spatial_desc* d, const void* depth, const void* depthOrig, const void* image,
                         double* total, double* smooth, double* contrast, void* grad, hipStream_t s);
void parameterL1(cvd_handle* h, const cvd_param_desc* d, const int64_t* offsets, const int64_t* counts, int64_t flatCount,
                 const void* p, const void* p0, double lambda, double* total, void* grad, double gradOut, int accumulate,
                 double* kernelMs);
void parameterL1Device(cvd_handle* h, const cvd_param_desc* d, const void* const* p, const void* const* p0, const int64_t* counts,
                       double lambda, double* total, void* const* grad, const void* gradOut, int accumulate, hipStream_t s);
void paramStep(cvd_handle* h, const cvd_param_desc* d, const int64_t* offsets, const int64_t* counts, int64_t flatCount, void* p,
               const void* g, void* m, void* v, const cvd_param_record* records, double* kernelMs);
void paramStepDevice(cvd_handle* h, const cvd_param_desc* d, void* const* p, const void* const* g, void* const* m, void* const* v,
                     const int64_t* counts, const cvd_param_record* records, hipStream_t s);
long long paramChunkElements();
void datasetCreate(cvd_handle* h, const cvd_dataset_desc* d, const int32_t* pairFrames, const int32_t* samples);
void datasetClear(cvd_handle* h);
void datasetSetColors(cvd_handle* h, int first, int count, const float* hwc3);
void datasetSetFlows(cvd_handle* h, int first, int count, const float* flow, const uint8_t* mask);
void datasetSetDepthOrig(cvd_handle* h, int first, int count, const float* depth);
void datasetSetCameras(cvd_handle* h, const float* ext, const float* intr);
void datasetSetXforms(cvd_handle* h, const cvd_xform_desc* dd, const double* dparams, const cvd_xform_desc* sd, const double* sparams);
void datasetSetMaps(cvd_handle* h, const float* scales, int scaleIsMap, const float* warp);
void datasetBatchDevice(cvd_handle* h, int B, const int64_t* indices, const cvd_dataset_batch_out* out, hipStream_t s);
void datasetBatch(cvd_handle* h, int B, const int64_t* indices, const cvd_dataset_batch_out* out, double* kernelMs);
long long datasetBadIndices(cvd_handle* h);
void raftCorrPyramidDevice(cvd_handle* h, long long Q, int h2, int w2, int dim, int levels, const float* raw, float* const* level,
                           hipStream_t s);
void raftCorrLookupDevice(cvd_handle* h, int B, int h1, int w1, int h2, int w2, int levels, int radius, const float* const* level,
                          const float* coords, float* out, hipStream_t s);
void raftUpsampleFlowDevice(cvd_handle* h, int N, int H, int W, const float* flow, const float* mask, float* out, hipStream_t s);
void raftSepConvGruDevice(cvd_handle* h, int B, int H, int W, const float* hidden, int numSegments, const float* const* segments,
                          const int32_t* segmentChannels, const float* const* weights, const float* const* biases, float* out,
                          hipStream_t s, double* kernelMs);
// ... 72 lines not shown
```

robust_cvd_amd/csrc/cvd_matvec.hip:

```cpp
#include "cvd_host.h"
#include "cvd_pcg.h"
#include "cvd_cross.h"
#include "cvd_triplets.h"

namespace cvd {

bool coarseFusedConsumers() {
  return false;
}
bool fusedExchange(cvd_handle* h, bool withCoarse) { return !withCoarse || h->coarse.denseMode; }
size_t exchangeOffsetQc(const Ctx& c) { return c.h->dist() ? static_cast<size_t>(c.h->framesPadded()) * c.L.B : c.n; }
size_t exchangeOffsetPq(const Ctx& c, bool withDenseCoarse) {
  return exchangeOffsetQc(c) + (withDenseCoarse ? static_cast<size_t>(c.L.F) * kCB : 0);
}
size_t exchangeTemporalCount(cvd_handle* h, bool withCoarse) {
  const TlStep ts = temporalStep(h);
  return (ts.Ainv != nullptr && h->dist() && fusedExchange(h, withCoarse)) ? static_cast<size_t>(h->F) * ts.S : 0;
}
bool ownerShardedUpdate(cvd_handle* h, bool withCoarse) {
  return h->dist() && fusedExchange(h, withCoarse) && h->opt.dist_owner_update != 0;
}
CoarseView coarseView(cvd_handle* h, bool on, bool walk) {
  auto& C = h->coarse;
  CoarseView v = on ? CoarseView{C.pos.p, C.wPtr.p, C.wRow.p, walk ? C.Wb.p : nullptr, C.y.p, C.modeActive.p, C.fail.p, C.c.p}
                    : CoarseView{nullptr, nullptr, nullptr, nullptr, nullptr, nullptr, nullptr, nullptr};
  if (h->temporal.on && h->temporal.built) {
    v.tl = h->temporal.tl.p;
    v.tlW = h->temporal.vW.p;
    v.tlIdx = h->temporal.vIdx.p;
    v.tlS = h->temporal.S;
  }
  return v;
}

void prepareMatvec(Ctx& c, const double* x) {
  cvd_handle* h = c.h;
  const Layout& L = c.L;
  launchFrameConsts(c, x);
  int nr = 0;
  if (L.scaleRegSqrt > 0.0) nr += L.sregX * L.sregY;
  if (L.focalRegSqrt > 0.0) nr += 1;
  if (L.depthDeformW > 0.0 && L.depthType == CVD_DEPTH_GRID) nr += gridNumEdges(L.gx, L.gy, L.gz) * L.N;
  if (L.spatialDeformW > 0.0) nr += L.nS;
  const int stride = std::max(2, c.KD * std::max(1, L.N));
  const size_t entries = static_cast<size_t>(L.F) * stride * std::max(nr, 1);
  h->dRegJac.ensure(entries);
  h->dRegCol.ensure(entries);
  h->dRegCnt.ensure(static_cast<size_t>(L.F) * std::max(nr, 1));
  h->regCache = RegCache{h->dRegJac.p, h->dRegCol.p, h->dRegCnt.p, nr, stride};
  HIP_CHECK(hipMemsetAsync(h->dScal.p + S_DONE, 0, sizeof(double), h->stream));
  if (nr == 0) return;
  CVD_DISPATCH_KD(c.KD, {
    hipLaunchKernelGGL((k_reg_cache<KD>), dim3(L.F), dim3(256), static_cast<size_t>(L.B) * 8, h->stream, L, x, h->dMedian.p, h->dRegOwner.p,
                       h->regCache);
  });
  HIP_CHECK(hipGetLastError());
}

static bool productSumsShares(const Ctx& c) {
  const cvd_handle* h = c.h;
  if (c.cross || !c.L.includeStatic || c.nItems <= 0 || h->dense) return false;
  if (h->forceGeneric || c.KS != 0 || !fastLoss(c.L)) return false;
  if (!(c.L.N == 1 && c.L.lossType == CVD_STATIC_REPRO_DISPARITY)) return false;
  if (c.L.robustKind != 0) return false;
  if (c.KD != 4) return false;
  return !(c.trip && c.TT.nGroups > 0);
}

void launchMatvec(Ctx& c, const double* x, const double* z, const double* pOld, double* pNew, int useBeta,
                         const double* lam, double* q, bool withCoarse, bool tailFused, int sharesIteration) {
  cvd_handle* h = c.h;
  if (sharesIteration > 0 && !productSumsShares(c)) throw std::runtime_error("launchMatvec: this product cannot sum the tail's shares");
  hipStream_t s = h->stream;
  const CoarseView cF = coarseView(h, withCoarse, coarseFusedConsumers());
  const size_t B = c.L.B;
  auto recordLaunch = [h](int threads, int spec, int kd, int kind, int items) {
    const int launched[6] = {threads, spec, kd, kind, items, h->numCU};
    std::copy(launched, launched + 6, h->lastProduct);
  };
  if (c.cross) {
    hipEvent_t evStart, evStop;
    (void)h->tReserve(KC_MATVEC_PAIRS, evStart, evStop);
    const size_t ldsX = (3 * B + (kCrossThreads / 64) * B + 2 * kCB + 2 * kTlMaxS) * 8;
    const unsigned nP = static_cast<unsigned>(h->xFa.size()) + (h->xDiagRows ? static_cast<unsigned>(c.L.F) : 0u);
    const int* diagSlot = h->xDiagRows ? h->dXDiagSlot.p : nullptr;
    recordLaunch(kCrossThreads, 0, c.KD, 3, static_cast<int>(nP));
    if (evStart)
      hipExtLaunchKernelGGL(k_cross_matvec, dim3(nP), dim3(kCrossThreads), ldsX, s, evStart, evStop, 0, c.L, crossPairs(h),
                            h->dXBlocks.p, h->dH.p, diagSlot, h->dMask.p, z, pOld, h->dScal.p, useBeta, h->dQPart.p, cF);
    else
      hipLaunchKernelGGL(k_cross_matvec, dim3(nP), dim3(kCrossThreads), ldsX, s, c.L, crossPairs(h), h->dXBlocks.p, h->dH.p, diagSlot,
                         h->dMask.p, z, pOld, h->dScal.p, useBeta, h->dQPart.p, cF);
    HIP_CHECK(hipGetLastError());
  } else if (c.L.includeStatic && c.nItems > 0) {
    const size_t lds = 6 * B * 8 + 2 * sizeof(FrameConst) + (18 + 4 * 24 + 8 + 2 * kCB) * 8;
    const size_t ldsFast = 6 * B * 8 + 2 * sizeof(FrameConst) + (32 + static_cast<size_t>(kRedVals) * kRedStride) * 8;
    hipEvent_t evStart, evStop;
    (void)h->tReserve(KC_MATVEC_PAIRS, evStart, evStop);
    const bool fast = !h->forceGeneric && c.KS == 0 && fastLoss(c.L);
    const FrameConst* fcp = h->dFc.p;
    const double* maskp = h->dMask.p;
    const double* scalp = h->dScal.p;
    if (fast) {
      const int spec = (c.L.N == 1 && c.L.lossType == CVD_STATIC_REPRO_DISPARITY) ? (c.L.robustKind == 0 ? 1 : 2) : 0;
      const int wavesPerSimd = spec ? ((c.KD <= 4) ? CVD_MV_WAVES : 3) : 2;
      const long long slots256 = static_cast<long long>(wavesPerSimd) * h->numCU;
      const long long slots128 = std::min<long long>(2 * slots256, static_cast<long long>(kMaxLds / std::max<size_t>(ldsFast, 1)) * h->numCU);
#ifndef CVD_MV_NT_RULE
#define CVD_MV_NT_RULE 1
#endif
      const int nt = CVD_MV_NT_RULE ? ((c.nItems <= slots256 || c.nItems > slots128) ? 256 : 128)
                                    : (c.nItems > 2 * h->numCU && c.nItems <= 4 * h->numCU ? 128 : 256);
#define CVD_LAUNCH_PAIRS_FAST_S(NTV, SPECV)                                                                              \
      CVD_DISPATCH_KD(c.KD, {                                                                                            \
        recordLaunch(NTV, SPECV, KD, 1, c.nItems);                                                                       \
        if constexpr (SPECV == 1 && KD == 4) {                                                                           \
          if (sharesIteration > 0) {           \
            allowLds((k_matvec_pairs_fast<KD, NTV, SPECV, false, true>), ldsFast);                                       \
            if (evStart)                                                                                                 \
              hipExtLaunchKernelGGL((k_matvec_pairs_fast<KD, NTV, SPECV, false, true>), dim3(c.nItems), dim3(NTV), ldsFast, s, \
                                    evStart, evStop, 0, c.L, c.T, c.it, x, fcp, maskp, z, pOld, scalp, sharesIteration,  \
// ... 258 lines not shown
```

robust_cvd_amd/csrc/cvd_pcg.h:

```cpp
#pragma once

#include "cvd_kernels.h"

namespace cvd {

inline __global__ void k_lm_diag(Layout L, const double* __restrict__ hdiag, double* __restrict__ scale,
                          int computeScale, double radius, double* __restrict__ lam) {
  const size_t n = static_cast<size_t>(L.F) * L.B;
  const size_t i = static_cast<size_t>(blockIdx.x) * blockDim.x + threadIdx.x;
  if (i >= n) return;
  const double h = hdiag[i];
  if (computeScale) scale[i] = 1.0 / (1.0 + sqrt(h));
  const double s = scale[i];
  if (h == 0.0) {
    lam[i] = 1.0;
  } else {
    const double d = fmin(fmax(s * s * h, 1e-6), 1e32);
    lam[i] = d / (radius * s * s);
  }
}

template <int KD>
inline __global__ __launch_bounds__(256) void k_reg_cache(Layout L, const double* __restrict__ x,
                                                   const float* __restrict__ median,
                                                   const unsigned char* __restrict__ owner, RegCache rc) {
  extern __shared__ __attribute__((aligned(16))) double sm[];
  const int f = blockIdx.x;
  if (!owner[f]) return;
  for (int i = threadIdx.x; i < L.B; i += 256) sm[i] = x[static_cast<size_t>(f) * L.B + i];
  __syncthreads();
  const float med = median[f];
  for (int i = threadIdx.x; i < rc.nr; i += 256) {
    double r;
    int n;
    int cols[2 * KD + 2];
    double jac[2 * KD + 2];
    regResidual<KD>(L, f, i, sm, med, r, n, cols, jac);
    rc.cnt[static_cast<size_t>(f) * rc.nr + i] = static_cast<unsigned char>(n);
    for (int a = 0; a < n; ++a) {
      const size_t e = (static_cast<size_t>(f) * rc.stride + a) * rc.nr + i;
      rc.jac[e] = jac[a];
      rc.col[e] = static_cast<unsigned short>(cols[a]);
    }
  }
}

struct TailCarry {
  double pv, qv;
};

template <int KD, bool FUSED>
__device__ __forceinline__ bool matvecFinishBody(const Layout& L, const double* __restrict__ x,
                                                 const double* __restrict__ mask,
                                                 const double* __restrict__ lam, const float* __restrict__ median,
                                                 const unsigned char* __restrict__ inRange,
                                                 const unsigned char* __restrict__ rangeFlags,
                                                 const int* __restrict__ fiOff, const int* __restrict__ fiList,
                                                 const double* __restrict__ qPart, const double* __restrict__ z,
                                                 const double* __restrict__ pOld, double* __restrict__ pNew,
                                                 double* __restrict__ scal, unsigned int* __restrict__ counter,
                                                 int useBeta, double* __restrict__ q, double* __restrict__ fdot,
                                                 int distMode, int nRows, const RegCache& rc, const CoarseView& V,
                                                 double* __restrict__ qc, const CoarseColumns& cc,
                                                 const double* __restrict__ Hdiag, double* __restrict__ pqOut,
                                                 int ownFirst, int ownCount, double* __restrict__ sm, TailCarry& carry,
                                                 const TlStep* __restrict__ tsp, double* __restrict__ tlPart) {
  const double sDone = scal[S_DONE];
  const int nT = FUSED ? static_cast<int>(blockDim.x) : 256;
  const int B = L.B;
  double* xf = sm;
  double* pf = xf + B;
  double* qf = pf + B;
  double* red = qf + B;
  double* cl = red + 8;
  const int f = blockIdx.x;
  const int tid = threadIdx.x;
  const double beta = useBeta ? scal[S_BETA] : 0.0;
  const size_t base = static_cast<size_t>(f) * B;
  int e0 = 0, e1 = 0;
  bool regRowsOn = false;
  if constexpr (FUSED) {
    e0 = fiOff[f];
    e1 = fiOff[f + 1];
    regRowsOn = Hdiag == nullptr && inRange[f];
  }
// ... 957 lines not shown
  int levelShare0, levelWg0;
};

template <int KD>
inline __global__ __launch_bounds__(1024) __attribute__((amdgpu_waves_per_eu(6))) void k_pcg_tail(Layout L, const double* __restrict__ x,
                                                    const double* __restrict__ mask,
                                                    const double* __restrict__ lam, const float* __restrict__ median,
                                                    const unsigned char* __restrict__ inRange,
                                                    const unsigned char* __restrict__ rangeFlags,
                                                    const int* __restrict__ fiOff, const int* __restrict__ fiList,
                                                    const double* __restrict__ qPart, const double* __restrict__ pOld,
                                                    double* __restrict__ pNew, double* __restrict__ scal, int useBeta,
                                                    double* __restrict__ q, double* __restrict__ fdot, int nRows, RegCache rc,
                                                    CoarseView V, double* __restrict__ qc, const double* __restrict__ Hdiag,
                                                    TailUpdate U) {
  extern __shared__ __attribute__((aligned(16))) double sm[];
  const int f = blockIdx.x;
  const CoarseColumns ccOff{nullptr, nullptr, nullptr, nullptr, nullptr};
  const CoarseStep csOff{nullptr, nullptr, nullptr, nullptr, nullptr, nullptr, nullptr, nullptr, nullptr};
  TAIL_STAMP(0);
  const unsigned int barGen = tailGeneration(U.gridBar);
  const double rzOld = scal[S_RZ];
  auto first = [&](double& pv, double& qv) -> bool {
    if (f < L.F) {
      TailCarry carry{0.0, 0.0};
      if (!matvecFinishBody<KD, true>(L, x, mask, lam, median, inRange, rangeFlags, fiOff, fiList, qPart, U.z, pOld, pNew, scal,
                                      nullptr, useBeta, q, fdot, 0, nRows, rc, V, qc, ccOff, Hdiag, nullptr, 0, U.diagInProduct ? 0 : L.F,
                                      sm + U.ldsFinish, carry, U.ts, sm + L.B))
        return false;
      pv = carry.pv;
      qv = carry.qv;
    } else if (scal[S_DONE] != 0.0) {
      return false;
    }
    TAIL_STAMP(1);
    tailArrive(U.gridBar, gridDim.x, barGen, fdot, L.F, sm + U.ldsScratch);
    TAIL_STAMP(10);
    if (f < L.F && static_cast<int>(threadIdx.x) < L.B) {
      pNew[static_cast<size_t>(f) * L.B + threadIdx.x] = pv;
      q[static_cast<size_t>(f) * L.B + threadIdx.x] = qv;
    }
    return true;
  };
  auto second = [&](double& alpha) -> bool {
    double pq;
    TAIL_STAMP(2);
    if (!tailWait(U.gridBar, sm + U.ldsScratch, pq)) {
      if (U.shares != nullptr && threadIdx.x == 0) publishPartial(scal + SH_ABANDON, 1.0);
      return false;
    }
    TAIL_STAMP(3);
    alpha = rzOld / pq;
    if (blockIdx.x == 0 && threadIdx.x == 0) {
      scal[S_PQ] = pq;
      scal[S_ALPHA] = alpha;
    }
    return true;
  };
  struct Mid {
    decltype(first)& f1;
    decltype(second)& f2;
    double* scratch;
    __device__ bool first(double& pv, double& qv) { return f1(pv, qv); }
    __device__ bool second(double& alpha) { return f2(alpha); }
    __device__ unsigned int generation() { return *reinterpret_cast<unsigned int*>(scratch + 17); }
    bool stage;
    __device__ bool stageRows() { return stage; }
    double* shares;
    double* abandonWord;
    int levelShare0, levelWg0;
    __device__ bool closes() { return shares == nullptr; }
    __device__ double* levelShare(double* fromDescriptor) {
      return shares != nullptr ? shares + levelShare0 + (static_cast<int>(blockIdx.x) - levelWg0) : fromDescriptor;
    }
    __device__ void gaveUp() {
      if (shares != nullptr && threadIdx.x == 0) publishPartial(abandonWord, 1.0);
    }
  } mid{first, second, sm + U.ldsScratch, U.stageRows != 0, U.shares, scal + SH_ABANDON, U.levelShare0, U.levelWg0};
  cgUpdateBody<true>(L, 0, nullptr, U.minv, nullptr, nullptr, scal, U.counter, U.dx, U.r, U.z, U.fdotRZ, U.fdotRR, U.tol2, nullptr,
                     U.modeActive, U.hostMirror, csOff, U.ds, nullptr, sm, mid, 0, L.F, nullptr, U.ts, U.tp);
  TAIL_STAMP(4);
}

inline __global__ __launch_bounds__(64) void k_pcg_close(double* __restrict__ scal, int enqueued, double* __restrict__ hostMirror) {
  const int lane = threadIdx.x;
  double wz[8], wr[8];
#pragma unroll
  for (int u = 0; u < 8; ++u) {
    wz[u] = scal[SH_RZ + lane + u * 64];
    wr[u] = scal[SH_RR + lane + u * 64];
  }
  const double done0 = scal[S_DONE], abandon = scal[SH_ABANDON], old = scal[S_RZ], target = scal[S_TARGET];
  const int applied = static_cast<int>(scal[S_ITERS]);
  const double rz = pcgSharesSum(wz), rr = pcgSharesSum(wr);
  if (lane != 0 || abandon != 0.0) return;
  if (done0 == 0.0 && applied == enqueued - 1) {
    const double done = !(rz == rz) ? 2.0 : (rz <= target ? 1.0 : 0.0);
    pcgCloseFromShares(scal, enqueued, rz, old, (old != 0.0) ? rz / old : 0.0, done, hostMirror);
    scal[S_RR] = rr;
  } else if (applied >= 1) {
    scal[S_RR] = rr;
  }
}

inline __global__ void k_apply_step(Layout L, int boundDepth0, const double* __restrict__ x, const double* __restrict__ dx,
                             double* __restrict__ xc) {
  const size_t n = static_cast<size_t>(L.F) * L.B;
  const size_t i = static_cast<size_t>(blockIdx.x) * blockDim.x + threadIdx.x;
  if (i >= n) return;
  double v = x[i] + dx[i];
  if (boundDepth0) {
    const int c = static_cast<int>(i % L.B);
    if (c >= 7 && c < 7 + L.nD && ((c - 7) % L.N) == 0) v = fmax(v, 0.0);
  }
  xc[i] = v;
}

inline __global__ __launch_bounds__(1024) void k_tl_rows_init(const TlStep* __restrict__ tsp, int F, double* __restrict__ scal,
                                                       unsigned int* __restrict__ counter, int closeScalars, double tol2,
                                                       double* __restrict__ hostMirror) {
  extern __shared__ __attribute__((aligned(16))) double sm[];
  __shared__ int flag;
  NoMid mid;
  double alpha = 0.0;
  (void)tlLevelRows<false>(tsp, blockIdx.x, F, alpha, 1, 0.0, scal, sm, mid);
  if (!lastBlockArrivesLite(counter, gridDim.x, &flag)) return;
  if (threadIdx.x == 0) {
    double d = 0.0;
    for (int s = 0; s < tsp->S * tsp->parts; ++s) d += readPartial(tsp->dotPart + s);
    if (closeScalars) pcgFinishScalars(scal, 1, scal[S_RZPART] + d, scal[S_RR], tol2, hostMirror);
    else scal[S_RZPART] += d;
  }
}

}
```

robust_cvd_amd/csrc/cvd_precond.hip:

```cpp
#include "cvd_host.h"
#include "cvd_block_inverse.h"
#include "cvd_coarse.h"
#include "cvd_cross.h"
#include "cvd_dense_walk.h"
#include "cvd_dense_inverse.h"

namespace cvd {

void launchFlagToBool(int* flag, hipStream_t s) { hipLaunchKernelGGL(k_flag_to_bool, dim3(1), dim3(1), 0, s, flag); }

void launchBlockInverseRaw(cvd_handle* h, const Layout& L, const double* dH, const double* dLam, float* dMinv,
                                  int* dFail, int variant, hipStream_t onStream) {
  hipStream_t s = onStream ? onStream : h->stream;
  const int B = L.B;
  if (B > 256) {
    if (onStream) throw std::logic_error("launchBlockInverseRaw: the rocSOLVER route runs on the solver's stream");
    if (!h->rbMain) {
      if (rocblas_create_handle(&h->rbMain) != rocblas_status_success) throw std::runtime_error("rocblas_create_handle failed");
      if (rocblas_set_stream(h->rbMain, s) != rocblas_status_success) throw std::runtime_error("rocblas_set_stream failed");
    }
    const size_t bb = static_cast<size_t>(B) * B, total = bb * L.F;
    h->dInvScratch.ensure(total);
    h->dInvInfo.ensure(2 * static_cast<size_t>(L.F));
    HIP_CHECK(hipMemsetAsync(h->dInvInfo.p, 0, 2 * static_cast<size_t>(L.F) * sizeof(int), s));
// ... 81 lines not shown

namespace {
struct DinvPlan { DinvJob job; int tpw; size_t lds; };
DinvPlan planDenseSpdInverse(cvd_handle* h, int n, const double* A, double* out, int* fail, hipStream_t s, int* outValid,
                             DevBuf<double>* panelBuf, DevBuf<unsigned int>* barrierBuf) {
  DevBuf<double>& densePanel = panelBuf ? *panelBuf : h->coarse.densePanel;
  DevBuf<unsigned int>& barrier = barrierBuf ? *barrierBuf : h->coarse.barrier;
  const int nT = (n + kInvTS - 1) / kInvTS;
  int S = 1;
  auto groups = [&](int sv) { const int nS = (nT + sv - 1) / sv; return nS * (nS + 1) / 2; };
  while (groups(S) > h->numCU) ++S;
  const int nS = (nT + S - 1) / S;
  DinvPlan P;
  P.tpw = (S * S + kDinvNW - 1) / kDinvNW;
  P.lds = static_cast<size_t>(4 * S + 1 + kDinvNW) * kInvTile * sizeof(double);
  if (P.tpw > 25 || P.lds > kMaxLds) throw std::runtime_error(fmt("dense coarse level: %d unknowns are too many for the dense inverse", n));
  densePanel.ensure(static_cast<size_t>(2) * nT * 256 + 2 * 256);
  barrier.ensure(4);
  HIP_CHECK(hipMemsetAsync(barrier.p, 0, 4 * sizeof(unsigned int), s));
  P.job = DinvJob{n, S, nS, groups(S), A, out, fail, densePanel.p, densePanel.p + static_cast<size_t>(2) * nT * 256, barrier.p, outValid};
  return P;
}
}
void launchDenseSpdInverse(cvd_handle* h, int n, const double* A, double* out, int* fail, hipStream_t s, int* outValid,
                           DevBuf<double>* panelBuf, DevBuf<unsigned int>* barrierBuf) {
  const DinvPlan P = planDenseSpdInverse(h, n, A, out, fail, s, outValid, panelBuf, barrierBuf);
  const DinvJob& J = P.job;
  const size_t lds = P.lds;
  const int tpw = P.tpw;
#define CVD_LAUNCH_DINV(TPWV)                                                                                            \
  do {                                                                                                                   \
    allowLds((k_dense_spd_inverse<TPWV>), lds);                                                                          \
    int perCu_ = 0;                                                                                                      \
    HIP_CHECK(hipOccupancyMaxActiveBlocksPerMultiprocessor(&perCu_, reinterpret_cast<const void*>(&k_dense_spd_inverse<TPWV>), \
                                                           kDinvNW * 64, lds));                                          \
    if (static_cast<long long>(perCu_) * h->numCU < J.groups)                                                            \
      throw std::runtime_error(fmt("dense coarse level: %d workgroups of the inverse are not co-resident on this device " \
                                   "(%d per CU x %d CUs at %zu B of LDS)", J.groups, perCu_, h->numCU, lds));             \
    PersistentGate gate(h->device, s);                                                                                   \
    hipLaunchKernelGGL((k_dense_spd_inverse<TPWV>), dim3(J.groups), dim3(kDinvNW * 64), lds, s, J.n, J.S, J.nS, J.A, J.out, J.fail, \
                       J.panel, J.pinv, J.barrier, J.outValid);                                                           \
  } while (0)
  if (tpw <= 2) CVD_LAUNCH_DINV(2);
  else if (tpw <= 5) CVD_LAUNCH_DINV(5);
  else if (tpw <= 8) CVD_LAUNCH_DINV(8);
  else if (tpw <= 13) CVD_LAUNCH_DINV(13);
  else if (tpw <= 18) CVD_LAUNCH_DINV(18);
  else CVD_LAUNCH_DINV(25);
#undef CVD_LAUNCH_DINV
  HIP_CHECK(hipGetLastError());
}
void launchDenseSpdInversePair(cvd_handle* h, const DinvRequest& a, const DinvRequest& b, hipStream_t s) {
  const DinvPlan Pa = planDenseSpdInverse(h, a.n, a.A, a.out, a.fail, s, a.outValid, a.panelBuf, a.barrierBuf);
  const DinvPlan Pb = planDenseSpdInverse(h, b.n, b.A, b.out, b.fail, s, b.outValid, b.panelBuf, b.barrierBuf);
  const size_t lds = std::max(Pa.lds, Pb.lds);
  bool pair = Pa.tpw <= 2 && Pb.tpw <= 2 && CVD_DETERMINISTIC == 0;
  if (pair) {
    allowLds((k_dense_spd_inverse_pair<2>), lds);
    int perCu = 0;
    HIP_CHECK(hipOccupancyMaxActiveBlocksPerMultiprocessor(&perCu, reinterpret_cast<const void*>(&k_dense_spd_inverse_pair<2>), kDinvNW * 64, lds));
    pair = static_cast<long long>(perCu) * h->numCU >= 2ll * std::max(Pa.job.groups, Pb.job.groups);
  }
  if (!pair) {
    launchDenseSpdInverse(h, a.n, a.A, a.out, a.fail, s, a.outValid, a.panelBuf, a.barrierBuf);
    launchDenseSpdInverse(h, b.n, b.A, b.out, b.fail, s, b.outValid, b.panelBuf, b.barrierBuf);
    return;
  }
  PersistentGate gate(h->device, s);
  hipLaunchKernelGGL((k_dense_spd_inverse_pair<2>), dim3(std::max(Pa.job.groups, Pb.job.groups), 2), dim3(kDinvNW * 64), lds, s, Pa.job, Pb.job);
  HIP_CHECK(hipGetLastError());
}

void launchCoarseSetup(Ctx& c, const double* x, int side) {
  cvd_handle* h = c.h;
  hipStream_t s = side ? h->stream2 : h->stream;
  auto& C = h->coarse;
  const size_t B = c.L.B;
  double* WbOut = side ? C.Wb2.p : C.Wb.p;
  int* failOut = side ? C.fail2.p : C.fail.p;
  FrameConst* fcBuf = side ? h->dFc2.p : h->dFc.p;
  HIP_CHECK(hipMemsetAsync(failOut, 0, sizeof(int), s));
  {
    launchFrameConsts(c.L, x, fcBuf, s);
    HIP_CHECK(hipMemsetAsync(C.edges.p, 0, static_cast<size_t>(std::max(C.nEdges, 1)) * kCBB * sizeof(double), s));
    if (C.sparsified) HIP_CHECK(hipMemsetAsync(C.dropDiag.p, 0, static_cast<size_t>(c.L.F) * kCBB * sizeof(double), s));
    const size_t ldsE = 2 * B * 8 + 2 * sizeof(FrameConst) + 4 * kCBB * 8;
    if (c.cross && !C.sparsified) {
      hipLaunchKernelGGL(k_coarse_edges_cross, dim3(static_cast<unsigned>(h->xFa.size())), dim3(256), 0, s, c.L, crossPairs(h),
                         h->dXBlocks.p, h->dXPairEdge.p, C.edges.p);
    } else if (c.nItems > 0) {
      const bool fast = !h->forceGeneric && c.KS == 0 && fastLoss(c.L) &&
                        c.L.intrOpt != CVD_INTR_SHARED;
      const bool gram = fast && !h->dense && c.KD == 4 && c.L.N == 1 && !C.sparsified && CVD_DETERMINISTIC == 0;
      if (gram) {
        const size_t ldsG = (2 * B + 512 + 4 * 64 * kDwLd) * 8;
        allowLds(k_coarse_edges_mfma, ldsG);
        hipLaunchKernelGGL(k_coarse_edges_mfma, dim3(c.nItems), dim3(256), ldsG, s, c.L, c.T, c.it, x, fcBuf, C.itemEdgeDev.p, C.edges.p);
      } else if (fast) {
        CVD_DISPATCH_KD(c.KD, {
          if (h->dense) {
            allowLds((k_coarse_edges_fast<KD, true>), ldsE);
            hipLaunchKernelGGL((k_coarse_edges_fast<KD, true>), dim3(c.nItems), dim3(256), ldsE, s, c.L, c.T, c.it, x, fcBuf,
                               C.itemEdgeDev.p, C.edges.p, C.dropDiag.p);
          } else {
            allowLds((k_coarse_edges_fast<KD, false>), ldsE);
            hipLaunchKernelGGL((k_coarse_edges_fast<KD, false>), dim3(c.nItems), dim3(256), ldsE, s, c.L, c.T, c.it, x, fcBuf,
                               C.itemEdgeDev.p, C.edges.p, C.dropDiag.p);
          }
        });
      } else {
        CVD_DISPATCH(c.KD, c.KS, {
          allowLds(k_coarse_edges<KD, KS>, ldsE);
          hipLaunchKernelGGL((k_coarse_edges<KD, KS>), dim3(c.nItems), dim3(256), ldsE, s, c.L, c.T, c.it, x, fcBuf,
                             C.itemEdgeDev.p, C.edges.p, C.dropDiag.p);
        });
      }
    }
    HIP_CHECK(hipGetLastError());
    if (h->dist()) {
      const int ct = h->tBegin(KC_COMM_COARSE);
      commAllReduce(h, C.edges.p, static_cast<size_t>(C.nEdges) * kCBB, CT_F64, s);
      if (C.sparsified)
        commAllReduce(h, C.dropDiag.p, static_cast<size_t>(c.L.F) * kCBB, CT_F64, s);
      h->tEnd(ct);
    }
  }
  constexpr double lamPredict = 1.0 / 3.0;
  hipLaunchKernelGGL(k_coarse_diag, dim3(c.L.F), dim3(256), 0, s, c.L, h->dH.p, h->dLam.p, h->dMask.p, C.diag.p,
                     C.modeActive.p, side ? lamPredict : 1.0, C.sparsified ? C.dropDiag.p : nullptr);
  if (h->dist()) {
    const int ct = h->tBegin(KC_COMM_COARSE);
    const size_t chunk = static_cast<size_t>(h->ownChunk()) * kCBB;
    commAllGather(h, C.diag.p + static_cast<size_t>(h->rank) * chunk, C.diag.p, chunk, CT_F64, s);
    h->tEnd(ct);
  }
  if (C.denseMode) {
    if (side) throw std::logic_error("the dense coarse level is built in line");
    if (C.temporalPose) {
      C.denseValid.ensure(1);
      if (!(C.denseReady && C.denseForB == static_cast<int>(c.L.B))) HIP_CHECK(hipMemsetAsync(C.denseValid.p, 0, sizeof(int), s));
      launchPoseTemporalBuild(c, s, failOut, h->temporal.on && !h->dist());
      if (h->dist()) {
        launchFlagToBool(failOut, s);
        const int ct = h->tBegin(KC_COMM_COARSE);
        commAllReduce(h, failOut, 1, CT_I32, s);
        h->tEnd(ct);
      }
      C.denseReady = true;
      C.denseForB = c.L.B;
      return;
    }
    const int n = c.L.F * kCB;
    C.denseA.ensure(static_cast<size_t>(n) * n);
    C.denseInv.ensure(static_cast<size_t>(n) * n);
    HIP_CHECK(hipMemsetAsync(C.denseA.p, 0, static_cast<size_t>(n) * n * sizeof(double), s));
    hipLaunchKernelGGL(k_coarse_dense_assemble, dim3(c.L.F + C.nEdges), dim3(64), 0, s, c.L.F, C.nEdges, C.diag.p, C.edges.p,
                       C.edgeFa.p, C.edgeFb.p, C.modeActive.p, C.denseA.p, h->opt.coarse_dense_shift);
    HIP_CHECK(hipGetLastError());
    C.denseValid.ensure(1);
    if (!(C.denseReady && C.denseForB == static_cast<int>(c.L.B))) HIP_CHECK(hipMemsetAsync(C.denseValid.p, 0, sizeof(int), s));
    launchDenseSpdInverse(h, n, C.denseA.p, C.denseInv.p, failOut, s, C.denseValid.p);
    if (h->dist()) {
      launchFlagToBool(failOut, s);
      const int ct = h->tBegin(KC_COMM_COARSE);
      commAllReduce(h, failOut, 1, CT_I32, s);
      h->tEnd(ct);
// ... 24 lines not shown
```

robust_cvd_amd/csrc/cvd_setup.hip:

```cpp
#include "cvd_host.h"
#include "cvd_table.h"
#include "cvd_triplets.h"
#include "cvd_dense_walk.h"
#include <rocprim/device/device_segmented_radix_sort.hpp>

namespace cvd {

void launchFrameConsts(const Layout& L, const double* x, FrameConst* fc, hipStream_t s) {
  hipLaunchKernelGGL(k_frame_consts, dim3((L.F + 63) / 64), dim3(64), 0, s, L, x, fc);
}

static void quatToMatrix(const double q[4] , double R[3][3]) {
  for (int c = 0; c < 3; ++c) {
    double v[3] = {0, 0, 0};
    v[c] = 1.0;
    const double uv[3] = {2.0 * (q[1] * v[2] - q[2] * v[1]), 2.0 * (q[2] * v[0] - q[0] * v[2]),
                          2.0 * (q[0] * v[1] - q[1] * v[0])};
    R[0][c] = v[0] + q[3] * uv[0] + (q[1] * uv[2] - q[2] * uv[1]);
    R[1][c] = v[1] + q[3] * uv[1] + (q[2] * uv[0] - q[0] * uv[2]);
    R[2][c] = v[2] + q[3] * uv[2] + (q[0] * uv[1] - q[1] * uv[0]);
  }
}
static void matrixToAngleAxis(const double R[3][3], double aa[3]) {
  double q0, q1, q2, q3;
// ... 1002 lines not shown
    std::vector<AsmPart> parts;
    int slots = 0;
    for (int f = 0; f < h->F; ++f) {
      const int nu = fuOff[f + 1] - fuOff[f];
      const int np = std::max(1, (nu + capU - 1) / capU);
      const int per = (nu + np - 1) / np;
      for (int q = 0; q < np; ++q) {
        AsmPart a;
        a.frame = f;
        a.u0 = fuOff[f] + std::min(nu, q * per);
        a.u1 = fuOff[f] + std::min(nu, (q + 1) * per);
        a.part = q;
        a.nParts = np;
        a.slot0 = np > 1 ? slots : 0;
        parts.push_back(a);
      }
      if (np > 1) slots += np;
    }
    std::stable_sort(parts.begin(), parts.end(),
                     [](const AsmPart& a, const AsmPart& b) { return a.u1 - a.u0 > b.u1 - b.u0; });
    h->nAsmParts = static_cast<int>(parts.size());
    h->nAsmSlots = slots;
    h->dAsmParts.upload(parts.data(), parts.size(), s);
    h->dAsmUnits.upload(units.data(), units.size(), s);
    h->nAsmSegs = 0;
    if (!h->dense) {
      std::vector<AsmUnitRange> ranges(parts.size());
      for (size_t q = 0; q < parts.size(); ++q) ranges[q] = AsmUnitRange{parts[q].u0, parts[q].u1};
      std::vector<AsmUnitDesc> descs(units.size());
      for (size_t u = 0; u < units.size(); ++u) descs[u] = AsmUnitDesc{units[u].x, units[u].y};
      std::vector<AsmSegment> segs;
      std::vector<int32_t> waveOff;
      cutAsmSegments(ranges, descs, h->pairA.data(), h->pairB.data(), h->pairOff.data(), kAsmThreads / 64, kAsmUnit, segs, waveOff);
      h->nAsmSegs = static_cast<int>(segs.size());
      if (segs.empty()) segs.push_back(AsmSegment{});
      h->dAsmSegs.upload(segs.data(), segs.size(), s);
      h->dAsmWaveOff.upload(waveOff.data(), waveOff.size(), s);
    }
    if (h->dAsmCount.n < static_cast<size_t>(h->F)) {
      h->dAsmCount.ensure(h->F);
      HIP_CHECK(hipMemsetAsync(h->dAsmCount.p, 0, sizeof(unsigned int) * h->F, s));
    }
  }
  h->dFiOff.upload(fiOff.data(), fiOff.size(), s);
  h->dFiList.upload(fiList.data(), fiList.size(), s);
  h->dFpOff.upload(fpOff.data(), fpOff.size(), s);
  h->dFpList.upload(fpList.data(), fpList.size(), s);
  HIP_CHECK(hipStreamSynchronize(s));
  h->tableRange = inRange;
  h->tableValid = true;
}
void orderTable(cvd_handle* h, const Layout& L, int KD) {
  int gx = 0, gy = 0;
  if (!h->dense && h->C > 0 && h->opt.constraint_order != 0 && L.depthType == kDepthGrid && L.gz <= 1 && (KD == 4 || KD == 16) &&
      L.gx * L.gy <= kOrderMaxCells) {
    gx = L.gx;
    gy = L.gy;
  }
  if (h->orderGx == gx && h->orderGy == gy) return;
  h->orderGx = gx;
  h->orderGy = gy;
  h->tableOrdered = false;
  if (gx == 0) return;
  h->dNdcOrd.ensure(h->C);
  h->dDsrcOrd.ensure(h->C);
  const size_t lds = static_cast<size_t>(gx * gy + 1) * sizeof(int) + 3 * kOrderCap * sizeof(unsigned short);
  allowLds(k_order_table, lds);
  hipLaunchKernelGGL(k_order_table, dim3(h->P), dim3(64), lds, h->stream, h->dPairOff.p, gx, gy, L.maxcx, L.maxcy, h->dNdc.p,
                     h->dDsrc.p, h->dNdcOrd.p, h->dDsrcOrd.p);
  HIP_CHECK(hipGetLastError());
  h->tableOrdered = true;
}

double* pinnedStage(cvd_handle* h, int which, size_t n) {
  if (h->hStageN[which] < n) {
    if (h->hStage[which]) HIP_CHECK(hipHostFree(h->hStage[which]));
    h->hStage[which] = nullptr;
    HIP_CHECK(hipHostMalloc(reinterpret_cast<void**>(&h->hStage[which]), std::max<size_t>(n, 1) * sizeof(double)));
    h->hStageN[which] = n;
  }
  return h->hStage[which];
}

void uploadState(cvd_handle* h, const Layout& L, DevBuf<double>& dst) {
  const size_t nAll = static_cast<size_t>(L.F) * L.B;
  double* x = pinnedStage(h, 1, nAll);
  const int nD = L.nD, nS = L.nS;
  for (int f = 0; f < L.F; ++f) {
    double* xf = &x[static_cast<size_t>(f) * L.B];
    for (int i = 0; i < 7; ++i) xf[i] = h->poseParams[f][i];
    for (int i = 0; i < nD; ++i) xf[7 + i] = h->dparams[static_cast<size_t>(f) * nD + i];
    for (int i = 0; i < nS; ++i) xf[7 + nD + i] = h->sparams[static_cast<size_t>(f) * nS + i];
  }
  dst.upload(x, nAll, h->stream);
  HIP_CHECK(hipStreamSynchronize(h->stream));
}

void downloadState(cvd_handle* h, const Layout& L, const DevBuf<double>& src) {
  const size_t nAll = static_cast<size_t>(L.F) * L.B;
  double* x = pinnedStage(h, 0, nAll);
  src.download(x, nAll, h->stream);
  HIP_CHECK(hipStreamSynchronize(h->stream));
  const int nD = L.nD, nS = L.nS;
  for (int f = 0; f < L.F; ++f) {
    const double* xf = &x[static_cast<size_t>(f) * L.B];
    for (int i = 0; i < 7; ++i) h->poseParams[f][i] = xf[i];
    for (int i = 0; i < nD; ++i) h->dparams[static_cast<size_t>(f) * nD + i] = xf[7 + i];
    for (int i = 0; i < nS; ++i) h->sparams[static_cast<size_t>(f) * nS + i] = xf[7 + nD + i];
  }
}

void buildMask(cvd_handle* h, const Layout& L, const cvd_opt_params& p, ProblemKind kind,
                      const std::vector<int>& range) {
  const size_t nAll = static_cast<size_t>(L.F) * L.B;
  HIP_CHECK(hipStreamSynchronize(h->stream));
  double* m = pinnedStage(h, 0, nAll);
  std::fill(m, m + nAll, 0.0);
  for (int f : range) {
    double* mf = &m[static_cast<size_t>(f) * L.B];
    const bool poseFree = (kind == PK_POSE_STEP) && !p.fix_poses;
    for (int i = 0; i < 6; ++i) mf[i] = poseFree ? 1.0 : 0.0;
    mf[6] = (kind == PK_POSE_STEP && p.intr_opt != CVD_INTR_FIXED) ? 1.0 : 0.0;
    const bool depthFree = (kind == PK_NORMALIZE) || !p.fix_depth_xforms;
    for (int i = 0; i < L.nD; ++i) mf[7 + i] = depthFree ? 1.0 : 0.0;
    const bool spatialFree = (kind == PK_POSE_STEP) && !p.fix_spatial_xforms;
    for (int i = 0; i < L.nS; ++i) mf[7 + L.nD + i] = spatialFree ? 1.0 : 0.0;
  }
  h->dMask.upload(m, nAll, h->stream);
}

void ensureBuffers(Ctx& c) {
  cvd_handle* h = c.h;
  const size_t n = c.n;
  const size_t B = c.L.B;
  h->dX.ensure(n); h->dXc.ensure(n); h->dG.ensure(n); h->dLam.ensure(n); h->dScale.ensure(n);
  const size_t nVec = static_cast<size_t>(h->framesPadded()) * B;
  if (h->dist() && (h->dDx.n < nVec || h->dZ.n < nVec)) {
    h->dDx.ensure(nVec); h->dR.ensure(nVec); h->dZ.ensure(nVec);
    HIP_CHECK(hipMemsetAsync(h->dDx.p, 0, nVec * sizeof(double), h->stream));
    HIP_CHECK(hipMemsetAsync(h->dR.p, 0, nVec * sizeof(double), h->stream));
    HIP_CHECK(hipMemsetAsync(h->dZ.p, 0, nVec * sizeof(double), h->stream));
  }
  h->dDx.ensure(nVec); h->dR.ensure(nVec); h->dR1.ensure(n); h->dZ.ensure(nVec); h->dP0.ensure(n); h->dP1.ensure(n);
  h->dQ.ensure(nVec + static_cast<size_t>(c.L.F) * (kCB + kTlMaxS) + 8);
  h->dOwnerScal.ensure(2 * static_cast<size_t>(std::max(1, h->world)));
  h->dHd.ensure(n);
  {
    const size_t nPad = static_cast<size_t>(h->framesPadded()) * B;
    const bool grow = h->dH.n < nPad * B;
    h->dH.ensure(nPad * B); h->dMinv.ensure(nPad * B + 4); h->dHd.ensure(nPad);
    if (h->dist() && (grow || nPad > n)) {
      HIP_CHECK(hipMemsetAsync(h->dH.p, 0, nPad * B * sizeof(double), h->stream));
      HIP_CHECK(hipMemsetAsync(h->dMinv.p, 0, nPad * B * sizeof(float), h->stream));
      HIP_CHECK(hipMemsetAsync(h->dHd.p, 0, nPad * sizeof(double), h->stream));
    }
  }
  h->dQPart.ensure(std::max<size_t>(1, static_cast<size_t>(std::max(std::max(h->qRows, c.nItems * 2), c.cross ? h->xRows : 0)) * B));
  h->dFdot.ensure(static_cast<size_t>(c.L.F) * 4 + 64);
  h->dCostItem.ensure(std::max(1, c.nItems));
  h->dCostFrame.ensure(c.L.F);
  h->dFocal.ensure(static_cast<size_t>(c.L.F) * 2);
  const bool newScal = h->dScal.p == nullptr;
  h->dScal.ensure(SH_END);
  h->dFc.ensure(c.L.F);
  h->dFail.ensure(1);
  if (!h->dCounters.p) {
    h->dCounters.ensure(8);
    HIP_CHECK(hipMemsetAsync(h->dCounters.p, 0, 8 * sizeof(unsigned int), h->stream));
  }
  if (!h->hScal) HIP_CHECK(hipHostMalloc(reinterpret_cast<void**>(&h->hScal), (S_COUNT + 1) * sizeof(double)));
  if (!h->hPcg) {
    HIP_CHECK(hipHostMalloc(reinterpret_cast<void**>(&h->hPcg), 16 * sizeof(double)));
    for (auto& e : h->pcgEvent) HIP_CHECK(hipEventCreateWithFlags(&e, hipEventDisableTiming));
  }
  if (newScal) {
    HIP_CHECK(hipMemsetAsync(h->dScal.p, 0, SH_END * sizeof(double), h->stream));
    std::memcpy(h->hPcg + kPcgMirrorAddressSlot, &h->hPcg, sizeof(double*));
    HIP_CHECK(hipMemcpyAsync(h->dScal.p + SH_MIRROR, h->hPcg + kPcgMirrorAddressSlot, sizeof(double), hipMemcpyHostToDevice, h->stream));
    h->sharesF = h->sharesN = -1;
  }
}
__global__ void k_pick_median(const float* __restrict__ sorted, size_t n, int first, int count, float* __restrict__ median) {
  const int i = blockIdx.x * blockDim.x + threadIdx.x;
  if (i < count) median[first + i] = sorted[static_cast<size_t>(i) * n + n / 2];
}
void refreshMedians(cvd_handle* h) {
  if (!h->medianDirty) return;
  hipStream_t s = h->stream;
  const size_t n = static_cast<size_t>(h->W) * h->H;
  const int F = h->F;
  h->dMedian.ensure(F);
  const int PB = static_cast<int>(std::max<size_t>(1, std::min<size_t>(F, (size_t(1) << 28) / (n * sizeof(float)))));
  if (static_cast<size_t>(PB) * n > 0xFFFFFFFFull) throw std::runtime_error("depth maps too large for the median sort");
  DevBuf<float> sorted;
  DevBuf<unsigned int> seg;
  DevBuf<unsigned char> tmp;
  sorted.ensure(static_cast<size_t>(PB) * n);
  std::vector<unsigned int> segH(PB + 1);
// ... 26 lines not shown
```

robust_cvd_amd/csrc/cvd_solve.hip:

```cpp
#include <optional>

#include "cvd_host.h"
#include "cvd_lm.h"
#include "cvd_pcg.h"
#include "cvd_coarse.h"

namespace cvd {

void launchTlRowsInit(cvd_handle* h, const TlStep* tsp, int NT, int groups, int F, unsigned int* counter, int closeScalars, double tol2,
                      hipStream_t s) {
  const size_t lds = static_cast<size_t>(tlRowsLds(NT)) * 8;
  allowLds(k_tl_rows_init, lds);
  hipLaunchKernelGGL(k_tl_rows_init, dim3(groups), dim3(768), lds, s, tsp, F, h->dScal.p, counter, closeScalars, tol2, h->hPcg);
  HIP_CHECK(hipGetLastError());
}

namespace {
struct TailStalled {};
}
static int runPcgAttempt(Ctx& c, const double* x, const std::function<void()>& tail);
int runPcg(Ctx& c, const double* x, const std::function<void()>& tail) {
  const size_t firstTimerSlot = c.h->evUsed;
  try {
    return runPcgAttempt(c, x, tail);
  } catch (const TailStalled&) {
    cvd_handle* h = c.h;
    HIP_CHECK(hipStreamSynchronize(h->stream));
    HIP_CHECK(hipMemsetAsync(h->dCounters.p, 0, 8 * sizeof(unsigned int), h->stream));
    HIP_CHECK(hipMemsetAsync(h->dScal.p + SH_ABANDON, 0, (SH_END - SH_ABANDON) * sizeof(double), h->stream));
    h->sharesF = h->sharesN = -1;
    if (h->temporal.counter.p) HIP_CHECK(hipMemsetAsync(h->temporal.counter.p, 0, 4 * sizeof(unsigned int), h->stream));
    if (h->dTailBar.p)
      HIP_CHECK(hipMemsetAsync(h->dTailBar.p, 0, static_cast<size_t>(kTailBarStride) * (1 + kTailBarCopies) * sizeof(unsigned int), h->stream));
    h->curPcgIter = -1;
    h->tDropFrom(firstTimerSlot, 0);
    h->tailDisabled = true;
    fprintf(stderr, "[cvd] warning: k_pcg_tail's grid barrier was abandoned (device shared with other work?); this handle uses the "
                    "two-launch PCG tail from here on\n");
    return runPcgAttempt(c, x, tail);
  }
}
static int runPcgAttempt(Ctx& c, const double* x, const std::function<void()>& tail) {
  cvd_handle* h = c.h;
  hipStream_t s = h->stream;
  const int F = c.L.F;
  const size_t B = c.L.B;
  if (B > 512) throw std::runtime_error("frame block larger than 512 unknowns is not supported by k_cg_update");
  prepareMatvec(c, x);
  const int nChunks = static_cast<int>((B + 63) / 64);
  const int nThreads = (B > 256 ? 128 : 256) * nChunks;
  double* fd = h->dFdot.p;
  size_t ldsU = (B + cgUpdatePartDoubles(static_cast<int>(B), nThreads) + 48 + 17 * kCB) * 8;
  const double tol2 = c.h->opt.pcg_relative_tolerance * c.h->opt.pcg_relative_tolerance;
  for (int i = 0; i < 9; ++i) h->hPcg[i] = 0.0;
  const bool coarse = h->coarseOn;
  double* rc = coarse ? h->coarse.rc.p : nullptr;
  const bool denseCoarse = coarse && h->coarse.denseMode;
  const bool unfusedY = denseCoarse;
  auto coarseC = [&](int init) {
    if (c.L.positionRegSqrt > 0.0 || c.trip || !coarseFusedConsumers())
      hipLaunchKernelGGL(k_coarse_apply_wt, dim3(F), dim3(256), 0, s, coarseView(h, true, true), F, h->coarse.c.p,
                         h->dScal.p, init);
  };
  const bool poseT = denseCoarse && h->coarse.temporalPose;
  auto coarseApply = [&](int init) {
    if (poseT) {
      launchPoseTemporalInit(c, tol2);
      return;
    }
    if (denseCoarse) {
      hipLaunchKernelGGL(k_coarse_dense_apply, dim3(F), dim3(256), 0, s, F, h->coarse.denseInv.p, h->coarse.rc.p, h->coarse.c.p,
                         h->coarse.modeActive.p, h->coarse.dotPart.p, h->dScal.p, h->dCounters.p + 3, h->coarse.fail.p, init,
                         tol2, h->hPcg);
      return;
    }
    hipLaunchKernelGGL(k_coarse_apply_w, dim3(F), dim3(1024), 0, s, h->coarse.plan, h->coarse.Wb.p, h->coarse.rc.p,
                       h->coarse.y.p, h->coarse.dotPart.p, h->dScal.p, h->dCounters.p + 3, h->coarse.fail.p, init, tol2,
                       h->hPcg);
    coarseC(init);
  };
  const CoarseStep csOff{nullptr, nullptr, nullptr, nullptr, nullptr, nullptr, nullptr, nullptr, nullptr};
  const CoarseStep csOn = (coarse && !unfusedY)
                              ? CoarseStep{h->coarse.wtPtr.p, h->coarse.wtBlk.p, h->coarse.wtFrame.p, h->coarse.Wb.p,
                                           h->coarse.qc.p, h->coarse.y.p, h->coarse.fdotY.p, h->coarse.fail.p, h->coarse.wq.p}
                              : csOff;
  const DenseStep dsOff{nullptr, nullptr, nullptr, nullptr, nullptr, nullptr, nullptr, kCB, 0, nullptr};
  const bool denseFused = denseCoarse;
  const bool fusedX = h->dist() && fusedExchange(h, coarse);
  const double* pqReduced = fusedX ? h->dQ.p + exchangeOffsetPq(c, denseFused) : nullptr;
  const bool denseRows = denseFused && !poseT;
  const DenseStep dsOn = denseRows ? DenseStep{h->coarse.denseInv.p, fusedX ? h->dQ.p + exchangeOffsetQc(c) : h->coarse.qc.p, h->coarse.rc.p, h->coarse.c.p,
                                                h->coarse.dotPart.p, h->coarse.modeActive.p, h->coarse.fail.p,
                                                kCB, static_cast<int>(ldsU / 8), h->coarse.dotPart.p + F}
                                    : dsOff;
  if (denseRows) {
    const size_t dense = static_cast<size_t>(F) * kCB + nThreads + 16;
    ldsU = std::max((dsOn.rowSplit < kCB ? ldsU / 8 + dense : ldsU / 8), dense) * 8;
  }
  const TlStep tsOn = temporalStep(h);
  const int nTlWg = tsOn.Ainv != nullptr ? tsOn.S * tsOn.parts : 0;
  if (nTlWg) ldsU = std::max(ldsU, static_cast<size_t>(tlRowsLds(tsOn.NT)) * 8);
  const int nPtWg = poseT ? kCB * tlParts(h->coarse.ptNn) : 0;
  if (poseT) ldsU = std::max(ldsU, static_cast<size_t>(tlRowsLds(h->coarse.ptN)) * 8);
  const TlStep* tpDev = poseT ? poseTemporalStepDev(h) : nullptr;
  allowLds(k_cg_update, ldsU);
  hipLaunchKernelGGL(k_cg_update, dim3(F), dim3(nThreads), ldsU, s, c.L, 1, h->dG.p, h->dMinv.p, h->dP0.p, h->dQ.p,
                     h->dScal.p, h->dCounters.p + 1, h->dDx.p, h->dR.p, h->dZ.p, fd + F, fd + 2 * F, tol2, rc,
                     h->coarse.modeActive.p, h->hPcg, csOff, dsOff, static_cast<const double*>(nullptr), 0, F,
                     static_cast<double*>(nullptr), nTlWg ? temporalStepDev(h) : static_cast<const TlStep*>(nullptr),
                     static_cast<const TlStep*>(nullptr));
  if (nTlWg) launchTemporalInit(c, !coarse, tol2);
  if (coarse) coarseApply(1);
  HIP_CHECK(hipGetLastError());
  double* pOld = h->dP0.p;
  double* pNew = h->dP1.p;
  size_t ldsTail = 0;
  int ldsFinish = 0, ldsScratch = 0;
  const bool fusedTail = pcgTailScope(c, coarse, nThreads, ldsTail, ldsFinish, ldsScratch);
  h->lastFusedTail = fusedTail;
  h->lastKD = c.KD;
  h->lastCross = c.cross;
  if (fusedTail) {
    h->dTailBar.ensure(static_cast<size_t>(kTailBarStride) * (1 + kTailBarCopies));
    HIP_CHECK(hipMemsetAsync(h->dTailBar.p, 0, static_cast<size_t>(kTailBarStride) * (1 + kTailBarCopies) * sizeof(unsigned int), s));
    if (tsOn.rec != nullptr) HIP_CHECK(hipMemsetAsync(tsOn.rec, 0, 2 * static_cast<size_t>(tsOn.NT) * sizeof(double), s));
// ... 8 lines not shown
    h->sharesN = sharesLayout.count;
  }
  const bool ownerMode = ownerShardedUpdate(h, coarse);
  const int maxIt = std::max(1, c.h->opt.pcg_max_iterations);
  const bool lockstep = h->dbg.pcg_lockstep != 0;
  const size_t firstTimerSlot = h->evUsed;
  int enq = 0;
  auto enqueueIteration = [&](int it, int useBeta) {
    h->curPcgIter = it;
    if (fusedTail) {
      launchMatvec(c, x, h->dZ.p, pOld, pNew, useBeta, h->dLam.p, h->dQ.p, coarse, true, shares ? it : 0);
      launchPcgTail(c, x, pOld, pNew, useBeta, h->dLam.p, h->dQ.p, coarse, nThreads, ldsTail, ldsFinish, ldsScratch, tol2,
                    shares ? &sharesLayout : nullptr);
      std::swap(pOld, pNew);
      return;
    }
    launchMatvec(c, x, h->dZ.p, pOld, pNew, useBeta, h->dLam.p, h->dQ.p, coarse);
    if (ownerMode) {
      const int f0 = h->ownFirst(), nOwn = h->ownCount();
      const int slotO = h->tBegin(KC_CG_UPDATE);
      if (nOwn > 0 || nTlWg || nPtWg)
        hipLaunchKernelGGL(k_cg_update, dim3((denseRows && dsOn.rowSplit > 0 ? nOwn + (nOwn + kDenseFramesPerGroup - 1) / kDenseFramesPerGroup : nOwn) + nTlWg + nPtWg),
                           dim3(nThreads), ldsU, s, c.L, 0, h->dG.p, h->dMinv.p, pNew, h->dQ.p, h->dScal.p, h->dCounters.p + 1,
                           h->dDx.p, h->dR.p, h->dZ.p, fd + F, fd + 2 * F, tol2, static_cast<double*>(nullptr),
                           h->coarse.modeActive.p, h->hPcg, csOff, dsOn, pqReduced, f0, nOwn, h->dOwnerScal.p + 2 * h->rank,
                           nTlWg ? temporalStepDev(h) : static_cast<const TlStep*>(nullptr), tpDev);
      else
        HIP_CHECK(hipMemsetAsync(h->dOwnerScal.p + 2 * h->rank, 0, 2 * sizeof(double), s));
      HIP_CHECK(hipGetLastError());
      h->tEnd(slotO);
      const int ct = h->tBegin(KC_COMM_PRODUCT);
      const size_t chunkF = static_cast<size_t>(h->ownChunk());
      commGroupStart(h);
      commAllGather(h, h->dZ.p + h->rank * chunkF * B, h->dZ.p, chunkF * B, CT_F64, s);
      if (denseRows) commAllGather(h, h->coarse.c.p + h->rank * chunkF * kCB, h->coarse.c.p, chunkF * kCB, CT_F64, s);
      commAllGather(h, h->dOwnerScal.p + 2 * h->rank, h->dOwnerScal.p, 2, CT_F64, s);
      commGroupEnd(h);
      h->tEnd(ct);
      hipLaunchKernelGGL(k_pcg_scalars_dist, dim3(1), dim3(64), 0, s, h->dOwnerScal.p, h->world, h->dScal.p, tol2, h->hPcg);
      HIP_CHECK(hipGetLastError());
      std::swap(pOld, pNew);
      return;
    }
    const int slot = h->tBegin(KC_CG_UPDATE);
    hipLaunchKernelGGL(k_cg_update, dim3((denseRows && dsOn.rowSplit > 0 ? F + (F + kDenseFramesPerGroup - 1) / kDenseFramesPerGroup : F) + nTlWg + nPtWg), dim3(nThreads), ldsU, s, c.L, 0, h->dG.p, h->dMinv.p, pNew,
                       h->dQ.p, h->dScal.p, h->dCounters.p + 1, h->dDx.p, h->dR.p, h->dZ.p, fd + F, fd + 2 * F, tol2,
                       (coarse && unfusedY && !denseFused) ? rc : nullptr, h->coarse.modeActive.p, h->hPcg, csOn, dsOn, pqReduced,
                       0, F, static_cast<double*>(nullptr), nTlWg ? temporalStepDev(h) : static_cast<const TlStep*>(nullptr), tpDev);
    if (coarse && !denseFused) { if (unfusedY) coarseApply(0); else coarseC(0); }
    HIP_CHECK(hipGetLastError());
    h->tEnd(slot);
    std::swap(pOld, pNew);
  };
  const int kRunAhead = lockstep ? 1 : 2;
  volatile double* prog = h->hPcg;
  while (enq < maxIt) {
    if (enq >= kRunAhead - 1) {
      const int need = enq - kRunAhead + 1;
      double v;
      for (unsigned long long spins = 0; static_cast<long long>((v = prog[1 + (need & 7)]) * 0.25) != need + 1; ++spins) {
        if ((spins & 0xFFFFF) == 0xFFFFF) {
          const hipError_t e = hipStreamQuery(s);
          if (e != hipErrorNotReady) {
            HIP_CHECK(e);
            if (static_cast<long long>(prog[1 + (need & 7)] * 0.25) != need + 1) {
              if (fusedTail) throw TailStalled{};
              throw std::runtime_error("PCG progress mirror stalled");
            }
          }
        }
      }
      if (v - 4.0 * (need + 1) != 0.0) break;
    }
    enqueueIteration(enq, enq > 0 ? 1 : 0);
    ++enq;
    if (fusedTail && h->dbg.stall_fused_tail_once != 0 && enq == 3) throw TailStalled{};
    if (h->opt.verbose >= 2) {
      readScalars(c);
      std::printf("    pcg %3d  rz %.6e  rzpart %.6e  alpha %.6e  beta %.6e  pq %.6e  done %g\n", enq - 1, h->hScal[S_RZ],
                  h->hScal[S_RZPART], h->hScal[S_ALPHA], h->hScal[S_BETA], h->hScal[S_PQ], h->hScal[S_DONE]);
    }
  }
  h->curPcgIter = -1;
  if (shares && enq > 0) launchPcgClose(c, enq);
  if (ownerMode) {
    const int ct = h->tBegin(KC_COMM_PRODUCT);
    const size_t chunk = static_cast<size_t>(h->ownChunk()) * B;
    commGroupStart(h);
    commAllGather(h, h->dDx.p + h->rank * chunk, h->dDx.p, chunk, CT_F64, s);
    commAllGather(h, h->dR.p + h->rank * chunk, h->dR.p, chunk, CT_F64, s);
    commGroupEnd(h);
    h->tEnd(ct);
  }
  if (tail) tail();
  readScalars(c);
  if (h->hScal[S_DONE] == 2.0) throw std::runtime_error("PCG produced NaN");
  const int iters = static_cast<int>(h->hScal[S_ITERS]);
  if (fusedTail && h->hScal[S_DONE] == 0.0 && iters != enq) throw TailStalled{};
  h->tDropFrom(firstTimerSlot, iters);
  return iters;
}

bool wantsTriplets(const cvd_opt_params& p, ProblemKind kind) {
  return kind == PK_POSE_STEP && (p.smooth_static_weight > 0.0 || p.smooth_dynamic_weight > 0.0);
}
void bindTriplets(Ctx& c, const cvd_opt_params& p, ProblemKind kind) {
  cvd_handle* h = c.h;
  c.trip = wantsTriplets(p, kind) && c.L.includeStatic;
  if (!c.trip) return;
  c.TT = TripletTable{h->dTNdc.p, h->dTDsrc.p, h->dTStatic.p, h->dTOff.p, h->dTCenter.p, h->dTSlot.p,
                      static_cast<int>(h->tripActive.size()),
                      static_cast<int>(p.smooth_loss_type),
                      std::sqrt(std::max(0.0, p.smooth_static_weight)), std::sqrt(std::max(0.0, p.smooth_dynamic_weight))};
}

namespace {

struct SetupPhases {
  bool on;
  double t = nowSeconds();
  void operator()(const char* what) {
    if (!on) return;
    const double now = nowSeconds();
    fprintf(stderr, "[setup] %-14s %8.1f us\n", what, (now - t) * 1e6);
    t = now;
  }
};

struct BindMode {
  bool checkBlock;
  bool staticGuards;
  bool levels;
};
struct BoundProblem {
  Ctx c;
  std::optional<DenseListScope> denseList;
};

void bindProblem(BoundProblem& b, cvd_handle* h, const cvd_opt_params& p, double depthDeformReg, ProblemKind kind,
                 const std::vector<int>& range, const BindMode& mode, SetupPhases& phase) {
  Ctx& c = b.c;
  c.h = h;
  c.L = makeLayout(h, p, depthDeformReg, kind);
  if (mode.checkBlock) checkFrameBlock(static_cast<size_t>(c.L.B), "solve");
  tapCounts(c.L, c.KD, c.KS);
  phase("layout");
  const bool guarded = !mode.staticGuards || c.L.includeStatic;
  b.denseList.emplace(h, h->dense && guarded && !denseFastScope(h, c.L, c.KS, wantsTriplets(p, kind)));
  compileTable(h, range, wantsTriplets(p, kind), kind == PK_NORMALIZE && c.L.includeStatic);
  orderTable(h, c.L, c.KD);
  phase("table");
  refreshMedians(h);
  phase("medians");
  c.T = makeTable(h);
  c.nItems = static_cast<int>(h->itemFa.size());
  c.it = Items{h->dItemFa.p, h->dItemFb.p, h->dItemRange.p, h->dItemSlot.p, c.nItems, h->dItemRec.p};
  c.n = static_cast<size_t>(c.L.F) * c.L.B;
  c.boundDepth0 = (kind == PK_NORMALIZE && c.L.N > 0) ? 1 : 0;
  bindTriplets(c, p, kind);
  if (guarded) checkDenseScope(h, c.L, c.KS, c.trip);
  c.cross = crossScope(h, c);
  h->coarseOn = mode.levels && h->opt.coarse_level != 0 && h->coarse.valid && c.L.includeStatic && h->coarse.nEdges > 0 &&
                !h->forceGeneric && kind == PK_POSE_STEP;
  ensureBuffers(c);
  phase("buffers");
  if (mode.levels) {
    h->coarse.ptInvPending = false;
    h->temporal.on = temporalScope(c);
    if (h->temporal.on) h->temporal.on = temporalPrepare(c);
    phase("level 3 tables");
    if (h->coarseOn && h->coarse.temporalPose) poseTemporalPrepare(c);
    phase("level 2 tables");
  }
  buildMask(h, c.L, p, kind, range);
  phase("mask");
  uploadState(h, c.L, h->dX);
  phase("upload");
}

long long countResidualBlocks(const Ctx& c, const std::vector<int>& range) {
  const cvd_handle* h = c.h;
  const long long nr = static_cast<long long>(range.size());
  long long blocks = c.trip ? h->numValidTrip : 0;
  if (c.L.scaleRegSqrt > 0.0) blocks += nr * c.L.sregX * c.L.sregY;
  if (c.L.focalRegSqrt > 0.0) blocks += nr;
  if (c.L.depthDeformW > 0.0 && c.L.depthType == CVD_DEPTH_GRID) blocks += nr;
  if (c.L.spatialDeformW > 0.0 && c.L.nS > 0) blocks += nr;
  if (c.L.positionRegSqrt > 0.0)
    for (int k = c.L.firstFrame; k < c.L.lastFrame - 1; ++k)
      blocks += (h->tableRange[k] && h->tableRange[k + 1] && h->tableRange[k + 2]) ? 1 : 0;
  return blocks;
}

struct PendingGuard {
  cvd_handle* h;
  const LevelSchedule& schedule;
  bool inverseAside = false;
  ~PendingGuard() {
    if (schedule.pending) (void)hipStreamWaitEvent(h->stream, h->evCoarseDone, 0);
    if (inverseAside) (void)hipStreamWaitEvent(h->stream, h->evInvDone, 0);
    if (h->temporal.sidePending) {
      (void)hipStreamWaitEvent(h->stream, h->temporal.evDone, 0);
      h->temporal.sidePending = false;
    }
  }
};

void rebuildTemporalLevel(Ctx& c) {
  cvd_handle* h = c.h;
  const int slot = h->tBegin(KC_INVERSE);
  launchTemporalSetup(c, h->dX.p, 0);
  launchTemporalSetup(c, h->dX.p, 1);
  h->tEnd(slot);
}

void buildLevels(Ctx& c, const LevelSchedule::Decision& d, PendingGuard& guard) {
  cvd_handle* h = c.h;
  hipStream_t s = h->stream;
  if (d.inverseAside) {
    HIP_CHECK(hipEventRecord(h->evInvIn, s));
    HIP_CHECK(hipStreamWaitEvent(h->stream3, h->evInvIn, 0));
    launchBlockInverse(c, h->stream3);
    HIP_CHECK(hipEventRecord(h->evInvDone, h->stream3));
    guard.inverseAside = true;
  } else {
    const int slot = h->tBegin(KC_INVERSE);
    launchBlockInverse(c);
    h->tEnd(slot);
  }
  if (d.coarse == LevelSchedule::SIDE_STREAM) {
    h->dFc2.ensure(c.L.F);
    if (h->temporal.on) rebuildTemporalLevel(c);
    HIP_CHECK(hipEventRecord(h->evCoarseIn, s));
    HIP_CHECK(hipStreamWaitEvent(h->stream2, h->evCoarseIn, 0));
    launchCoarseSetup(c, h->dX.p, 1);
    HIP_CHECK(hipEventRecord(h->evCoarseDone, h->stream2));
  } else if (d.coarse == LevelSchedule::IN_LINE) {
    const int slot = h->tBegin(KC_INVERSE);
    const bool measure = h->coarse.denseMode && !h->dist() && h->opt.coarse_rebuild_excess_dense < 0;
    if (measure) {
      if (!h->evRebuild[0]) for (auto& e : h->evRebuild) HIP_CHECK(hipEventCreate(&e));
      HIP_CHECK(hipEventRecord(h->evRebuild[0], s));
    }
    if (h->temporal.on) launchTemporalSetup(c, h->dX.p, 0);
    launchCoarseSetup(c, h->dX.p);
    if (d.inverseAside) {
      HIP_CHECK(hipStreamWaitEvent(s, h->evInvDone, 0));
      guard.inverseAside = false;
    }
    if (h->temporal.on) launchTemporalSetup(c, h->dX.p, 1);
    if (measure) {
      HIP_CHECK(hipEventRecord(h->evRebuild[1], s));
      h->rebuildTimed = true;
    }
    h->tEnd(slot);
  }
  if (d.temporalOnly) rebuildTemporalLevel(c);
}

void installPendingCoarse(cvd_handle* h, LevelSchedule& schedule) {
  if (!schedule.pending) return;
  HIP_CHECK(hipStreamWaitEvent(h->stream, h->evCoarseDone, 0));
  std::swap(h->coarse.Wb.p, h->coarse.Wb2.p);
  std::swap(h->coarse.Wb.n, h->coarse.Wb2.n);
  std::swap(h->coarse.fail.p, h->coarse.fail2.p);
  std::swap(h->coarse.fail.n, h->coarse.fail2.n);
  schedule.installed();
}

void notePcgTime(cvd_handle* h, double seconds, int cgIters) {
  if (cgIters <= 0 || h->dist()) return;
  double ms = seconds * 1e3;
  if (h->rebuildTimed) {
    float rb = 0.f;
    if (hipEventElapsedTime(&rb, h->evRebuild[0], h->evRebuild[1]) == hipSuccess && rb > 0.f) {
      h->coarseRebuildMs = h->coarseRebuildMs > 0.0 ? 0.5 * (h->coarseRebuildMs + rb) : rb;
      ms = std::max(0.0, ms - rb);
    }
    h->rebuildTimed = false;
  }
  const double per = ms / cgIters;
  h->pcgIterMs = h->pcgIterMs > 0.0 ? 0.75 * h->pcgIterMs + 0.25 * per : per;
}

void pushRecord(cvd_handle* h, cvd_iteration_record& rec, double cost, double radius, double gmax, bool tableLine = true) {
  rec.cost = cost;
  rec.trust_region_radius = radius;
  h->records.push_back(rec);
  if (tableLine && h->opt.verbose)
    printf("%4d % .6e    % .2e   % .2e   % .2e  % .2e % .2e   %5d\n", rec.iteration, cost, rec.cost_change, gmax, rec.step_norm,
           rec.relative_decrease, radius, rec.linear_iterations);
}

}

void solve(cvd_handle* h, const cvd_opt_params& p, double depthDeformReg, ProblemKind kind) {
  const double t0 = nowSeconds();
  if (h->F <= 0) throw std::runtime_error("no video set");
  if (!h->poseParamsValid) posesToParams(h);
  const std::vector<int> range = rangeOf(p, h->F);
  LevelSchedule schedule;
  PendingGuard guard{h, schedule};
  SetupPhases phase{h->opt.verbose >= 3};
  BoundProblem bound;
  bindProblem(bound, h, p, depthDeformReg, kind, range, BindMode{ true,  true,  true}, phase);
  Ctx& c = bound.c;
  hipStream_t s = h->stream;
  HIP_CHECK(hipMemsetAsync(h->dDx.p, 0, c.n * sizeof(double), s));
  HIP_CHECK(hipMemsetAsync(h->dR.p, 0, c.n * sizeof(double), s));
  HIP_CHECK(hipMemsetAsync(h->dFail.p, 0, sizeof(int), s));

  cvd_solve_summary sum{};
  sum.num_residual_blocks = static_cast<int>((c.L.includeStatic ? h->numValid : 0) + countResidualBlocks(c, range));
  double tEval = 0.0, tLin = 0.0;
  double te = nowSeconds();
  double xCost = evalFull(c, h->dX.p, true, false);
  tEval += nowSeconds() - te;
  sum.initial_cost = xCost;
  phase("first eval");
  double gmax = h->hScal[S_GMAX];
  double xNorm = std::sqrt(h->hScal[S_XX]);
  sum.num_parameters = static_cast<int>(h->hScal[S_NACTIVE] + 0.5);
  phase("stats");

  TrustRegion tr;
  const int rebuildExcess = h->coarse.denseMode ? denseRebuildThreshold(h->opt.coarse_rebuild_excess_dense, h->dist(), h->coarseRebuildMs, h->pcgIterMs)
                                                : h->opt.coarse_rebuild_excess;
  const LevelSchedule::Config levels{h->opt.coarse_level, h->opt.temporal_level, std::max(0, rebuildExcess), h->coarseOn, h->temporal.on,
                                     h->coarse.denseMode, h->dist(), h->stream3 != nullptr, c.L.B <= 256};
  bool gradPending = false;
  const bool deferStats = h->opt.verbose == 0;
  auto gradientConverged = [&]() { return gmax <= Ceres::gradient_tolerance && !h->dbg.force_iterations; };
  int iteration = 0, termination = 1;
  bool scaleDone = false;
  cvd_iteration_record r0{};
  r0.gradient_max_norm = gmax;
  r0.step_is_successful = 1;
  if (h->opt.verbose) printf("iter      cost      cost_change  |gradient|   |step|    tr_ratio  tr_radius  ls_iter\n");
  pushRecord(h, r0, xCost, tr.radius, gmax);

  if (sum.num_parameters == 0 || gradientConverged()) {
    termination = 0;
  } else {
    while (true) {
      if (iteration >= p.max_iterations) { termination = 1; break; }
      if (tr.belowMinRadius()) { termination = 0; break; }
      ++iteration;
      cvd_iteration_record rec{};
      rec.iteration = iteration;

      double tl = nowSeconds();
      hipLaunchKernelGGL(k_lm_diag, dim3((c.n + 255) / 256), dim3(256), 0, s, c.L, h->dHd.p, h->dScale.p,
                         scaleDone ? 0 : 1, tr.radius, h->dLam.p);
      scaleDone = true;
      buildLevels(c, schedule.decide(levels), guard);
      const double tPcgStart = nowSeconds();
      const int cgIters = runPcg(c, h->dX.p, [&]() {
        enqueueStats(c);
        hipLaunchKernelGGL(k_apply_step, dim3((c.n + 255) / 256), dim3(256), 0, s, c.L, c.boundDepth0, h->dX.p,
                           h->dDx.p, h->dXc.p);
        HIP_CHECK(hipGetLastError());
        enqueueCost(c, h->dXc.p);
      });
      notePcgTime(h, nowSeconds() - tPcgStart, cgIters);
      schedule.afterPcg(cgIters);
      installPendingCoarse(h, schedule);
      tLin += nowSeconds() - tl;
      if (gradPending) {
        gradPending = false;
        gmax = h->hScal[S_GMAX];
        xNorm = std::sqrt(h->hScal[S_XX]);
        h->records.back().gradient_max_norm = gmax;
        if (gradientConverged()) {
          --iteration;
          termination = 0;
          break;
        }
      }
      rec.linear_iterations = cgIters;
      sum.total_linear_iterations += cgIters;
      const double dg = h->hScal[S_DG], dr = h->hScal[S_DR], dld = h->hScal[S_DLD], dd = h->hScal[S_DD];
      const double modelCostChange = -0.5 * dg + 0.5 * dr + 0.5 * dld;
      if (!(std::isfinite(modelCostChange) && modelCostChange > 0.0 && std::isfinite(dd))) {
        if (!tr.invalidStep()) { termination = 2; break; }
        pushRecord(h, rec, xCost, tr.radius, gmax, false);
        continue;
      }
      tr.validStep();
      double candCost = h->hScal[S_COST];
      if (!std::isfinite(candCost)) candCost = std::numeric_limits<double>::max();
      rec.step_norm = std::sqrt(dd);
      rec.cost_change = xCost - candCost;
      rec.relative_decrease = (xCost - candCost) / modelCostChange;
      if (!h->dbg.force_iterations &&
          (TrustRegion::parameterToleranceReached(rec.step_norm, xNorm) || TrustRegion::functionToleranceReached(xCost, candCost))) {
        pushRecord(h, rec, xCost, tr.radius, gmax);
        termination = 0;
        break;
      }
      if (rec.relative_decrease > Ceres::min_relative_decrease) {
        std::swap(h->dX.p, h->dXc.p);
        std::swap(h->dX.n, h->dXc.n);
        schedule.accepted(std::abs(xCost - candCost) / std::max(std::abs(xCost), 1e-300));
        xCost = candCost;
        te = nowSeconds();
        gradPending = deferStats && iteration < p.max_iterations;
        (void)evalFull(c, h->dX.p, true, gradPending);
        tEval += nowSeconds() - te;
        if (!gradPending) {
          gmax = h->hScal[S_GMAX];
          xNorm = std::sqrt(h->hScal[S_XX]);
        }
        ++sum.num_successful_steps;
        rec.step_is_successful = 1;
        tr.accept(rec.relative_decrease);
        rec.gradient_max_norm = gmax;
        pushRecord(h, rec, xCost, tr.radius, gmax);
        if (!gradPending && gradientConverged()) { termination = 0; break; }
      } else {
        tr.reject();
        pushRecord(h, rec, xCost, tr.radius, gmax);
      }
    }
  }
  if (gradPending) {
    HIP_CHECK(hipMemsetAsync(h->dLam.p, 0, c.n * sizeof(double), s));
    enqueueStats(c);
    readScalars(c);
    h->records.back().gradient_max_norm = h->hScal[S_GMAX];
  }
  phase("LM loop");
  int* failWord = reinterpret_cast<int*>(h->hScal + S_COUNT);
  *failWord = 0;
  if (h->coarseOn && h->coarse.denseMode && h->coarse.fail.p != nullptr && !h->dist())
    HIP_CHECK(hipMemcpyAsync(failWord, h->coarse.fail.p, sizeof(int), hipMemcpyDeviceToHost, s));
  downloadState(h, c.L, h->dX);
  if (*failWord & 0x40000000)
    fprintf(stderr, "[cvd] warning: the dense coarse inverse timed out at its grid barrier (device shared with other work?); "
                    "the coarse level was off for the last LM iteration(s)\n");
  phase("download");
  h->tCollect();
  sum.num_iterations = iteration;
  sum.termination = termination;
  sum.final_cost = xCost;
  sum.total_seconds = nowSeconds() - t0;
  sum.evaluate_seconds = tEval;
  sum.linear_solve_seconds = tLin;
  h->summary = sum;
}
void evaluate(cvd_handle* h, const cvd_opt_params& p, double depthDeformReg, const double* pose7,
                     double* cost, int32_t* nres, double* gradient, double* hdiag, double* hfull) {
  if (pose7) {
    h->poseParams.resize(h->F);
    for (int f = 0; f < h->F; ++f)
      for (int i = 0; i < 7; ++i) h->poseParams[f][i] = pose7[f * 7 + i];
    h->poseParamsValid = true;
  } else {
    posesToParams(h);
  }
  const std::vector<int> range = rangeOf(p, h->F);
  SetupPhases quiet{false};
  BoundProblem bound;
  bindProblem(bound, h, p, depthDeformReg, PK_POSE_STEP, range, BindMode{ false,  false,  false}, quiet);
  Ctx& c = bound.c;
  hipStream_t s = h->stream;
  double cst;
  if (!gradient && !hdiag && !hfull) {
    cst = evalCost(c, h->dX.p);
  } else {
    cst = evalFull(c, h->dX.p);
  }
  if (cost) *cost = cst;
  if (nres) *nres = static_cast<int32_t>(h->numValid + countResidualBlocks(c, range));
  if (gradient) h->dG.download(gradient, c.n, s);
  if (hdiag) {
    if (h->dist()) {
      const size_t chunk = static_cast<size_t>(h->ownChunk()) * c.L.B * c.L.B;
      commAllGather(h, h->dH.p + static_cast<size_t>(h->rank) * chunk, h->dH.p, chunk, CT_F64, s);
    }
    h->dH.download(hdiag, c.n * c.L.B, s);
  }
  HIP_CHECK(hipStreamSynchronize(s));
  if (hfull) {
    std::vector<double> e(c.n, 0.0), col(c.n);
    HIP_CHECK(hipMemsetAsync(h->dLam.p, 0, c.n * sizeof(double), s));
// ... 20 lines not shown
```

robust_cvd_amd/csrc/cvd_temporal.hip:

```cpp
#include "cvd_host.h"
#include "cvd_temporal.h"

namespace cvd {

static int autoCoarse(int g, int wanted) {
  const int s = wanted > 0 ? wanted : (g + 1) / 2;
  return std::min(g, std::max(2, s));
}

bool temporalScope(const Ctx& c) {
  cvd_handle* h = c.h;
  const Layout& L = c.L;
  if (h->opt.temporal_level == 0 || h->forceGeneric || (h->dense && !c.cross) || c.trip) return false;
  if (c.KD != 4 || c.KS != 0 || !fastLoss(L) || L.intrOpt == CVD_INTR_SHARED) return false;
  if (L.N != 1 || L.gz != 1 || L.depthType != CVD_DEPTH_GRID || L.positionRegSqrt > 0.0 || !L.includeStatic) return false;
  if (L.B > 256 || L.nD > 256 || L.gx < 3 || L.gy < 3 || L.nD != L.gx * L.gy) return false;
  const int step = h->opt.temporal_step;
  if (L.F <= 2 * step) return false;
  const int Sx = autoCoarse(L.gx, h->opt.temporal_grid_x), Sy = autoCoarse(L.gy, h->opt.temporal_grid_y);
  if (Sx * Sy > kTlMaxS) return false;
  const int nn = (L.F - 1 + step - 1) / step + 1;
  if (nn * Sx * Sy > kDenseCoarseMaxUnknowns) return false;
  return true;
}
// ... 108 lines not shown
    if (gItems.empty()) gItems.push_back(0);
    T.gOff.upload(gOff.data(), gOff.size(), s);
    T.gItems.upload(gItems.data(), gItems.size(), s);
    T.blkA.upload(blkA.data(), blkA.size(), s);
    T.blkB.upload(blkB.data(), blkB.size(), s);
    T.gPtr.upload(gPtr.data(), gPtr.size(), s);
    T.gather.upload(gather.data(), gather.size(), s);
    HIP_CHECK(hipStreamSynchronize(s));
    T.nGroups = static_cast<int>(gOff.size()) - 1;
    T.nBlocks = static_cast<int>(blkA.size());
    T.grpF = F; T.grpStep = step; T.grpFa = unitFa; T.grpFb = unitFb;
  }
  const size_t SS = static_cast<size_t>(S) * S, NT = static_cast<size_t>(T.NT);
  T.Cf.ensure(static_cast<size_t>(F) * SS);
  T.E.ensure(std::max<size_t>(1, unitFa.size()) * SS);
  T.part.ensure(std::max<size_t>(1, static_cast<size_t>(T.nGroups)) * 4 * SS);
  T.A.ensure(NT * NT);
  T.Ainv.ensure(NT * NT);
  T.sq.ensure(static_cast<size_t>(F) * S);
  T.tl.ensure(static_cast<size_t>(F) * S);
  T.rT.ensure(NT);
  T.t.ensure(2 * NT);
  T.dotPart.ensure(static_cast<size_t>(S) * tlParts(nn));
  T.rec.ensure(2 * NT);
  T.fail.ensure(1);
  T.valid.ensure(1);
  if (!T.counter.p) {
    T.counter.ensure(4);
    HIP_CHECK(hipMemsetAsync(T.counter.p, 0, 4 * sizeof(unsigned int), s));
  }
  HIP_CHECK(hipMemsetAsync(T.valid.p, 0, sizeof(int), s));
  T.built = false;
  T.sqPtr = (h->dist() && fusedExchange(h, h->coarseOn)) ? h->dQ.p + exchangeOffsetPq(c, h->coarseOn && h->coarse.denseMode) + 1 : T.sq.p;
  return true;
}

static void temporalInverse(Ctx& c);
static TlTables temporalTables(cvd_handle* h) {
  auto& T = h->temporal;
  return TlTables{T.hx.p, T.bx.p, T.hy.p, T.by.p, T.vW.p, T.vIdx.p, T.elW.p, T.elV.p, T.Sx, T.Sy, T.S, T.width};
}

TlStep temporalStep(cvd_handle* h) {
  if (h == nullptr || !h->temporal.on || !h->temporal.built)
    return TlStep{nullptr, nullptr, nullptr, nullptr, nullptr, nullptr, nullptr, nullptr, nullptr, 0, 0, 1, 0, 0, 0, 1, kTlSpan, nullptr, 1.0};
  auto& T = h->temporal;
  return TlStep{T.Ainv.p, T.sqPtr, T.rT.p, T.t.p, T.tl.p, T.dotPart.p, T.fail.p, T.elW.p, T.elV.p, T.S, T.nn, T.step, T.NT, T.NT, T.width,
                tlParts(T.nn), kTlSpan, (!h->dist() && T.step <= 32) ? T.rec.p : nullptr,
                h->opt.temporal_weight};
}

const TlStep* temporalStepDev(cvd_handle* h) {
  return (h != nullptr && h->temporal.on && h->temporal.built) ? h->temporal.stepDev.p : nullptr;
}

void launchTemporalSetup(Ctx& c, const double* x, int half) {
  cvd_handle* h = c.h;
  auto& T = h->temporal;
  const Layout& L = c.L;
  const bool side = !h->dist() && h->stream2 != nullptr;
  hipStream_t s = (half == 0 && side) ? h->stream2 : h->stream;
  if (half == 1) {
    if (side && T.sidePending) {
      HIP_CHECK(hipStreamWaitEvent(h->stream, T.evDone, 0));
      T.sidePending = false;
    }
    temporalInverse(c);
    return;
  }
  const TlTables tb = temporalTables(h);
  const size_t SS = static_cast<size_t>(T.S) * T.S;
  FrameConst* fcBuf = h->dFc.p;
  if (side) {
    if (!T.evIn) {
      HIP_CHECK(hipEventCreateWithFlags(&T.evIn, hipEventDisableTiming));
      HIP_CHECK(hipEventCreateWithFlags(&T.evDone, hipEventDisableTiming));
    }
    h->dFc2.ensure(L.F);
    fcBuf = h->dFc2.p;
    HIP_CHECK(hipEventRecord(T.evIn, h->stream));
    HIP_CHECK(hipStreamWaitEvent(s, T.evIn, 0));
  }
  launchFrameConsts(L, x, fcBuf, s);
  const size_t ldsD = static_cast<size_t>(L.nD) * T.S * 8 + static_cast<size_t>(T.width) * T.S * 5 + 16;
  allowLds(k_tl_diag, ldsD);
  hipLaunchKernelGGL(k_tl_diag, dim3(L.F), dim3(256), ldsD, s, L, h->dH.p, h->dLam.p, h->dMask.p, tb, T.Cf.p,
                     h->dist() ? h->ownFirst() : 0, h->dist() ? h->ownCount() : L.F);
  HIP_CHECK(hipGetLastError());
  if (c.cross) {
    if (!h->xFa.empty()) {
      allowLds(k_tl_edges_cross, ldsD);
      hipLaunchKernelGGL(k_tl_edges_cross, dim3(static_cast<unsigned>(h->xFa.size())), dim3(256), ldsD, s, L, h->dXFa.p, h->dXFb.p,
                         h->dXBlocks.p, h->dMask.p, tb, T.E.p);
      hipLaunchKernelGGL(k_tl_reduce, dim3(T.nGroups), dim3(256), 0, s, T.S, T.step, T.gOff.p, T.gItems.p, h->dXFa.p, h->dXFb.p, T.E.p,
                         T.part.p);
      HIP_CHECK(hipGetLastError());
    }
  } else if (c.nItems > 0) {
    const size_t ldsE = 2 * static_cast<size_t>(L.B) * 8 + 2 * sizeof(FrameConst) + SS * 8 + 3 * static_cast<size_t>(L.gx + L.gy) * 4 + 16;
    allowLds(k_tl_edges<false>, ldsE);
    hipLaunchKernelGGL(k_tl_edges<false>, dim3(c.nItems), dim3(256), ldsE, s, L, c.T, c.it, x, fcBuf, h->dMask.p, tb, T.E.p);
    HIP_CHECK(hipGetLastError());
    hipLaunchKernelGGL(k_tl_reduce, dim3(T.nGroups), dim3(256), 0, s, T.S, T.step, T.gOff.p, T.gItems.p, h->dItemFa.p, h->dItemFb.p,
                       T.E.p, T.part.p);
    HIP_CHECK(hipGetLastError());
  }
  HIP_CHECK(hipMemsetAsync(T.A.p, 0, static_cast<size_t>(T.NT) * T.NT * sizeof(double), s));
  hipLaunchKernelGGL(k_tl_assemble, dim3(T.nBlocks, static_cast<unsigned>((SS + 255) / 256)), dim3(256), 0, s, T.S, T.nn, T.step, L.F, T.NT, T.blkA.p, T.blkB.p, T.gPtr.p,
                     T.gather.p, T.Cf.p, T.part.p, T.A.p);
  HIP_CHECK(hipGetLastError());
  if (h->dist()) {
    const int ct = h->tBegin(KC_COMM_COARSE);
    commAllReduce(h, T.A.p, static_cast<size_t>(T.NT) * T.NT, CT_F64, s);
    h->tEnd(ct);
  }
  hipLaunchKernelGGL(k_tl_shift_diag, dim3((T.NT + 255) / 256), dim3(256), 0, s, T.NT, T.NT, T.A.p, h->opt.coarse_dense_shift);
  HIP_CHECK(hipGetLastError());
  if (side) {
    HIP_CHECK(hipEventRecord(T.evDone, s));
    T.sidePending = true;
  }
}

static void temporalInverse(Ctx& c) {
  cvd_handle* h = c.h;
  auto& T = h->temporal;
  hipStream_t s = h->stream;
  HIP_CHECK(hipMemsetAsync(T.fail.p, 0, sizeof(int), s));
  if (h->coarse.ptInvPending) {
    auto& C = h->coarse;
    C.ptInvPending = false;
    DinvRequest a, b;
    a.n = C.ptN; a.A = C.ptMat.p; a.out = C.ptInv.p; a.fail = C.ptInvFail; a.outValid = C.denseValid.p;
    b.n = T.NT; b.A = T.A.p; b.out = T.Ainv.p; b.fail = T.fail.p; b.outValid = T.valid.p; b.panelBuf = &T.invPanel; b.barrierBuf = &T.invBarrier;
    launchDenseSpdInversePair(h, a, b, s);
  } else {
    launchDenseSpdInverse(h, T.NT, T.A.p, T.Ainv.p, T.fail.p, s, T.valid.p, &T.invPanel, &T.invBarrier);
  }
  if (h->dist()) {
    launchFlagToBool(T.fail.p, s);
    const int ct = h->tBegin(KC_COMM_COARSE);
    commAllReduce(h, T.fail.p, 1, CT_I32, s);
    h->tEnd(ct);
  }
  if (!T.built) {
    T.built = true;
    const TlStep ts = temporalStep(h);
    T.stepDev.ensure(1);
    if (T.stepHost.size() != sizeof(TlStep) || std::memcmp(T.stepHost.data(), &ts, sizeof(TlStep)) != 0) {
      HIP_CHECK(hipMemcpyAsync(T.stepDev.p, &ts, sizeof(TlStep), hipMemcpyHostToDevice, s));
      HIP_CHECK(hipStreamSynchronize(s));
      T.stepHost.assign(reinterpret_cast<const unsigned char*>(&ts), reinterpret_cast<const unsigned char*>(&ts) + sizeof(TlStep));
    }
  }
}

void launchTemporalInit(Ctx& c, bool closeScalars, double tol2) {
  cvd_handle* h = c.h;
  auto& T = h->temporal;
  hipStream_t s = h->stream;
  const TlStep ts = temporalStep(h);
  if (ts.Ainv == nullptr) return;
  const size_t ldsR = (static_cast<size_t>(c.L.B) + static_cast<size_t>(T.S) * T.width) * 8;
  hipLaunchKernelGGL(k_tl_restrict, dim3(c.L.F), dim3(256), ldsR, s, c.L, h->dR.p, temporalStepDev(h));
  launchTlRowsInit(h, temporalStepDev(h), T.NT, T.S * tlParts(T.nn), c.L.F, T.counter.p, closeScalars ? 1 : 0, tol2, s);
}
// ... 116 lines not shown
```

Measured before the change: 359.7.

## Fuse LM glue kernels: step close, cost tail, diag-sum, frame-const reuse

Cuts the small glue launches around each LM iteration. The step statistics, step application and frame-constant computation are merged into one step-close kernel, optionally absorbing the PCG close. Frame-cost and total-cost summation now share one kernel through a last-block-arrives pattern, and the cost sum is folded into the diagonal extraction. Frame constants are reused when the state buffer has not been written since they were computed. A debug flag keeps the old unfused path. This adds write-tracking bookkeeping, which could go stale, and more complex kernels.

```diff
diff --git a/include/cvd_hip_debug.h b/include/cvd_hip_debug.h
--- a/include/cvd_hip_debug.h
+++ b/include/cvd_hip_debug.h
@@ -17,6 +17,7 @@
   int32_t tail_closes_scalars;
   int32_t asm_force_stage_depth;
   int32_t asm_force_part_units;
+  int32_t lm_glue_unfused;
 } cvd_debug_options;
 void cvd_debug_options_default(cvd_debug_options* o);
 int32_t cvd_set_debug_options(cvd_handle* h, const cvd_debug_options* o);
diff --git a/robust_cvd_amd/api.py b/robust_cvd_amd/api.py
--- a/robust_cvd_amd/api.py
+++ b/robust_cvd_amd/api.py
@@ -52,6 +52,7 @@
         ("tail_closes_scalars", C.c_int32),
         ("asm_force_stage_depth", C.c_int32),
         ("asm_force_part_units", C.c_int32),
+        ("lm_glue_unfused", C.c_int32),
     ]
 
 
@@ -2463,6 +2464,9 @@
         form = {-1: "none", 0: "exact sparse factor", 1: "exact dense inverse", 2: "temporal pose level"}[out[1]]
         return {"pose_graph_level": form, "depth_grid_level": bool(out[2]), "fused_tail": bool(out[3] & 1), "tail_rows_staged": bool(out[3] & 2),
                 "product_sums_shares": bool(out[3] & 4), "rz_shares": out[3] >> 8,
+                "frame_consts_reused": bool(out[3] & 8), "cost_tail_merged": bool(out[3] & 16), "diag_tail_merged": bool(out[3] & 32),
+                "step_close": bool(out[3] & 64),
+                "glue_chains": bool(out[3] & 128),
                 "tail_disabled": bool(out[4]),
                 "taps": out[5], "work_items": out[6], "cross_blocks": bool(out[7])}
 
diff --git a/robust_cvd_amd/csrc/cvd_api.hip b/robust_cvd_amd/csrc/cvd_api.hip
--- a/robust_cvd_amd/csrc/cvd_api.hip
+++ b/robust_cvd_amd/csrc/cvd_api.hip
@@ -281,6 +281,7 @@
   o->tail_closes_scalars = 0;
   o->asm_force_stage_depth = 0;
   o->asm_force_part_units = 0;
+  o->lm_glue_unfused = 0;
 }
 int32_t cvd_set_debug_options(cvd_handle* h, const cvd_debug_options* o) {
   CVD_TRY(h, {
@@ -1179,6 +1180,7 @@
     out8[2] = h->temporal.on ? 1 : 0;
     out8[3] = h->lastFusedTail ? (h->tailStageRows ? 3 : 1) : 0;
     if (h->lastFusedTail && h->lastShares) out8[3] |= 4 | (h->lastShareCount << 8);
+    out8[3] |= (h->glueForms & 31) << 3;
     out8[4] = h->tailDisabled ? 1 : 0;
     out8[5] = h->lastKD;
     out8[6] = static_cast<int32_t>(h->itemFa.size());
diff --git a/robust_cvd_amd/csrc/cvd_cost.h b/robust_cvd_amd/csrc/cvd_cost.h
--- a/robust_cvd_amd/csrc/cvd_cost.h
+++ b/robust_cvd_amd/csrc/cvd_cost.h
@@ -1,6 +1,7 @@
 #pragma once
 
 #include "cvd_kernels.h"
+#include "cvd_step_stats.h"
 
 namespace cvd {
 
@@ -52,6 +53,71 @@
 }
 
 template <int KD>
+__device__ __forceinline__ double regResidualValue(const Layout& L, int f, int i, const double* __restrict__ xf, float median) {
+  constexpr double eps = 1e-6;
+  if (L.scaleRegSqrt > 0.0) {
+    const int ns = L.sregX * L.sregY;
+    if (i < ns) {
+      const int y = i / L.sregX, x = i - y * L.sregX;
+      const float lx = __fadd_rn(-1.f, __fdiv_rn(__fmul_rn(2.f, static_cast<float>(x)), static_cast<float>(L.sregX - 1)));
+      const float ly = __fadd_rn(-1.f, __fdiv_rn(__fmul_rn(2.f, static_cast<float>(y)), static_cast<float>(L.sregY - 1)));
+      Taps<KD> t;
+      depthGather<KD>(L, lx, ly, median, t);
+      const double d = static_cast<double>(median);
+      double D = (L.depthType == kDepthIdentity) ? d : 0.0;
+      const double* th = xf + 7;
+#pragma unroll
+      for (int k = 0; k < KD; ++k) {
+        if (k < t.n) {
+          const double v = (L.N == 2) ? (d * th[t.idx[k] * 2] + th[t.idx[k] * 2 + 1]) : (d * th[t.idx[k]]);
+          D += v * t.w[k];
+        }
+      }
+      const double dd = !(D < eps) ? D : eps;
+      return L.scaleRegSqrt * (1.0 / dd - 1.0);
+    }
+    i -= ns;
+  }
+  Layout Lr = L;
+  Lr.scaleRegSqrt = 0.0;
+  double r;
+  int n;
+  int cols[2 * KD + 2];
+  double jac[2 * KD + 2];
+  regResidual<KD>(Lr, f, i, xf, median, r, n, cols, jac);
+  return r;
+}
+
+template <int KD>
+__device__ __forceinline__ double frameRegCost(const Layout& L, const double* __restrict__ x, const float* __restrict__ median,
+                                               const unsigned char* __restrict__ inRange,
+                                               const unsigned char* __restrict__ rangeFlags, double* sm, double* red) {
+  const int f = blockIdx.x;
+  double acc = 0.0;
+  if (threadIdx.x == 0 && L.positionRegSqrt > 0.0) {
+    double o3[3] = {0, 0, 0}, dg = 0.0, cst = 0.0;
+    if (posRegValid(L, rangeFlags, f)) posRegFrame(L, rangeFlags, f, x, nullptr, o3, dg, cst);
+    acc += cst;
+  }
+  const bool active = inRange[f] != 0;
+  if (active)
+    for (int i = threadIdx.x; i < L.B; i += 256) sm[i] = x[static_cast<size_t>(f) * L.B + i];
+  __syncthreads();
+  if (active) {
+    const float med = median[f];
+    const int nr = numRegResiduals<KD>(L);
+    for (int i = threadIdx.x; i < nr; i += 256) {
+      const double r = regResidualValue<KD>(L, f, i, sm, med);
+      acc += r * r;
+    }
+  }
+  acc = waveSum(acc);
+  if ((threadIdx.x & 63) == 0) red[threadIdx.x >> 6] = acc;
+  __syncthreads();
+  return 0.5 * ((red[0] + red[1]) + (red[2] + red[3]));
+}
+
+template <int KD>
 inline __global__ __launch_bounds__(256) void k_cost_frames(Layout L, const double* __restrict__ x,
                                                      const float* __restrict__ median,
                                                      const unsigned char* __restrict__ inRange,
@@ -59,33 +125,8 @@
                                                      double* __restrict__ costFrame) {
   extern __shared__ __attribute__((aligned(16))) double sm[];
   __shared__ double red[4];
-  const int f = blockIdx.x;
-  double acc = 0.0;
-  if (threadIdx.x == 0 && L.positionRegSqrt > 0.0) {
-    double o3[3] = {0, 0, 0}, dg = 0.0, cst = 0.0;
-    if (posRegValid(L, rangeFlags, f)) posRegFrame(L, rangeFlags, f, x, nullptr, o3, dg, cst);
-    acc += cst;
-  }
-  const bool active = inRange[f] != 0;
-  if (active)
-    for (int i = threadIdx.x; i < L.B; i += 256) sm[i] = x[static_cast<size_t>(f) * L.B + i];
-  __syncthreads();
-  if (active) {
-    const float med = median[f];
-    const int nr = numRegResiduals<KD>(L);
-    for (int i = threadIdx.x; i < nr; i += 256) {
-      double r;
-      int n;
-      int cols[2 * KD + 2];
-      double jac[2 * KD + 2];
-      regResidual<KD>(L, f, i, sm, med, r, n, cols, jac);
-      acc += r * r;
-    }
-  }
-  acc = waveSum(acc);
-  if ((threadIdx.x & 63) == 0) red[threadIdx.x >> 6] = acc;
-  __syncthreads();
-  if (threadIdx.x == 0) costFrame[f] = 0.5 * ((red[0] + red[1]) + (red[2] + red[3]));
+  const double cf = frameRegCost<KD>(L, x, median, inRange, rangeFlags, sm, red);
+  if (threadIdx.x == 0) costFrame[blockIdx.x] = cf;
 }
 
 inline __global__ __launch_bounds__(256) void k_sum2(const double* __restrict__ a, int na, const double* __restrict__ b,
@@ -98,6 +139,48 @@
   if ((threadIdx.x & 63) == 0) red[threadIdx.x >> 6] = acc;
   __syncthreads();
   if (threadIdx.x == 0) out[slot] = red[0] + red[1] + red[2] + red[3];
+}
+
+template <int KD>
+inline __global__ __launch_bounds__(256) void k_cost_frames_sum(Layout L, const double* __restrict__ x,
+                                                         const float* __restrict__ median,
+                                                         const unsigned char* __restrict__ inRange,
+                                                         const unsigned char* __restrict__ rangeFlags, double* costFrame,
+                                                         const double* __restrict__ costItem, int nItems,
+                                                         double* __restrict__ out, int slot, unsigned int* counter) {
+  extern __shared__ __attribute__((aligned(16))) double sm[];
+  __shared__ double red[4];
+  __shared__ int flag;
+  const double cf = frameRegCost<KD>(L, x, median, inRange, rangeFlags, sm, red);
+  if (threadIdx.x == 0) publishPartial(costFrame + blockIdx.x, cf);
+  if (!lastBlockArrivesLite(counter, gridDim.x, &flag)) return;
+  double acc = 0.0;
+  for (int i = threadIdx.x; i < nItems; i += 256) acc += costItem[i];
+  for (int i = threadIdx.x; i < L.F; i += 256) acc += readPartial(costFrame + i);
+  acc = waveSum(acc);
+  if ((threadIdx.x & 63) == 0) red[threadIdx.x >> 6] = acc;
+  __syncthreads();
+  if (threadIdx.x == 0) out[slot] = red[0] + red[1] + red[2] + red[3];
+}
+
+inline __global__ __launch_bounds__(256) void k_extract_diag_sum(Layout L, const double* __restrict__ hBlocks,
+                                                          double* __restrict__ diag, const double* __restrict__ costFrame,
+                                                          double* __restrict__ out, int slot) {
+  __shared__ double red[4];
+  if (blockIdx.x == gridDim.x - 1) {
+    double acc = 0.0;
+    for (int i = threadIdx.x; i < L.F; i += 256) acc += costFrame[i];
+    acc = waveSum(acc);
+    if ((threadIdx.x & 63) == 0) red[threadIdx.x >> 6] = acc;
+    __syncthreads();
+    if (threadIdx.x == 0) out[slot] = red[0] + red[1] + red[2] + red[3];
+    return;
+  }
+  const size_t n = static_cast<size_t>(L.F) * L.B;
+  const size_t i = static_cast<size_t>(blockIdx.x) * 256 + threadIdx.x;
+  if (i >= n) return;
+  const size_t f = i / L.B, c = i - f * L.B;
+  diag[i] = hBlocks[(f * L.B + c) * L.B + c];
 }
 
 template <int KD, bool DENSE = false>
@@ -193,58 +276,9 @@
                                                     const double* __restrict__ lam, const double* __restrict__ x,
                                                     const double* __restrict__ hdiagActive, double* __restrict__ scal,
                                                     double* __restrict__ part, unsigned int* __restrict__ counter) {
-  constexpr int NQ = 7;
-  __shared__ double red[NQ][4];
+  __shared__ double red[7][4];
   __shared__ int flag;
-  const int G = gridDim.x;
-  double a[NQ] = {0, 0, 0, 0, 0, 0, 0};
-  for (size_t i = static_cast<size_t>(blockIdx.x) * 256 + threadIdx.x; i < n; i += static_cast<size_t>(G) * 256) {
-    const double d = dx[i];
-    a[0] += d * g[i];
-    a[1] += d * r[i];
-    a[2] += d * lam[i] * d;
-    a[3] += d * d;
-    if (hdiagActive[i] != 0.0) { a[4] += x[i] * x[i]; a[6] += 1.0; }
-    a[5] = fmax(a[5], fabs(g[i]));
-  }
-#pragma unroll
-  for (int k = 0; k < NQ; ++k)
-    if (k != 5) a[k] = waveSum(a[k]);
-#pragma unroll
-  for (int off = 32; off > 0; off >>= 1) a[5] = fmax(a[5], __shfl_xor(a[5], off, 64));
-  if ((threadIdx.x & 63) == 0)
-    for (int k = 0; k < NQ; ++k) red[k][threadIdx.x >> 6] = a[k];
-  __syncthreads();
-  if (threadIdx.x < NQ) {
-    const int k = threadIdx.x;
-    part[k * G + blockIdx.x] = (k != 5) ? (red[k][0] + red[k][1]) + (red[k][2] + red[k][3])
-                                        : fmax(fmax(red[5][0], red[5][1]), fmax(red[5][2], red[5][3]));
-  }
-  if (!lastBlockArrives(counter, G, &flag)) return;
-  double t[NQ] = {0, 0, 0, 0, 0, 0, 0};
-  for (int b = threadIdx.x; b < G; b += 256) {
-#pragma unroll
-    for (int k = 0; k < NQ; ++k)
-      if (k != 5) t[k] += part[k * G + b];
-    t[5] = fmax(t[5], part[5 * G + b]);
-  }
-#pragma unroll
-  for (int k = 0; k < NQ; ++k)
-    if (k != 5) t[k] = waveSum(t[k]);
-#pragma unroll
-  for (int off = 32; off > 0; off >>= 1) t[5] = fmax(t[5], __shfl_xor(t[5], off, 64));
-  if ((threadIdx.x & 63) == 0)
-    for (int k = 0; k < NQ; ++k) red[k][threadIdx.x >> 6] = t[k];
-  __syncthreads();
-  if (threadIdx.x == 0) {
-    scal[S_DG] = red[0][0] + red[0][1] + red[0][2] + red[0][3];
-    scal[S_DR] = red[1][0] + red[1][1] + red[1][2] + red[1][3];
-    scal[S_DLD] = red[2][0] + red[2][1] + red[2][2] + red[2][3];
-    scal[S_DD] = red[3][0] + red[3][1] + red[3][2] + red[3][3];
-    scal[S_XX] = red[4][0] + red[4][1] + red[4][2] + red[4][3];
-    scal[S_GMAX] = fmax(fmax(red[5][0], red[5][1]), fmax(red[5][2], red[5][3]));
-    scal[S_NACTIVE] = red[6][0] + red[6][1] + red[6][2] + red[6][3];
-  }
-}
-
-}
+  stepStatsBody<false>(blockIdx.x, gridDim.x, n, dx, g, r, lam, x, hdiagActive, scal, part, counter, red, &flag, 1, 0, 1, 0, nullptr);
+}
+
+}
diff --git a/robust_cvd_amd/csrc/cvd_eval.hip b/robust_cvd_amd/csrc/cvd_eval.hip
--- a/robust_cvd_amd/csrc/cvd_eval.hip
+++ b/robust_cvd_amd/csrc/cvd_eval.hip
@@ -10,6 +10,27 @@
   launchFrameConsts(c.L, x, c.h->dFc.p, c.h->stream);
   HIP_CHECK(hipGetLastError());
 }
+static int stateIndex(const cvd_handle* h, const double* x) { return x == h->dX.p ? 0 : (x == h->dXc.p ? 1 : -1); }
+void stateWritten(cvd_handle* h, const double* x) {
+  const int k = stateIndex(h, x);
+  if (k >= 0) ++h->xWrites[k];
+  if (h->fcPoint == x) h->fcPoint = nullptr;
+}
+void frameConstsHold(cvd_handle* h, const double* x) {
+  const int k = stateIndex(h, x);
+  h->fcPoint = k >= 0 ? x : nullptr;
+  if (k >= 0) h->fcWrites = h->xWrites[k];
+}
+void ensureFrameConsts(Ctx& c, const double* x) {
+  cvd_handle* h = c.h;
+  const int k = stateIndex(h, x);
+  if (h->dbg.lm_glue_unfused == 0 && k >= 0 && h->fcPoint == x && h->fcWrites == h->xWrites[k]) {
+    h->glueForms |= GLUE_FC_REUSED;
+    return;
+  }
+  launchFrameConsts(c, x);
+  frameConstsHold(h, x);
+}
 
 void spinStream(hipStream_t s) {
   hipError_t e;
@@ -29,7 +50,7 @@
 void enqueueCost(Ctx& c, const double* x) {
   cvd_handle* h = c.h;
   hipStream_t s = h->stream;
-  launchFrameConsts(c, x);
+  ensureFrameConsts(c, x);
   const int slot = h->tBegin(KC_COST);
   if (c.L.includeStatic && c.nItems > 0) {
     const size_t lds = (2 * c.L.B) * 8 + 2 * sizeof(FrameConst) + 8 * 8;
@@ -55,6 +76,19 @@
     }
     HIP_CHECK(hipGetLastError());
   }
+  const int nItemCosts = c.L.includeStatic ? c.nItems : 0;
+  if (h->dbg.lm_glue_unfused == 0 && !(c.trip && c.TT.nGroups > 0)) {
+    CVD_DISPATCH_KD(c.KD, {
+      hipLaunchKernelGGL((k_cost_frames_sum<KD>), dim3(c.L.F), dim3(256), static_cast<size_t>(c.L.B) * 8, s, c.L, x, h->dMedian.p,
+                         h->dRegOwner.p, h->dInRange.p, h->dCostFrame.p, h->dCostItem.p, nItemCosts, h->dScal.p, S_COST,
+                         h->dCounters.p + 4);
+    });
+    HIP_CHECK(hipGetLastError());
+    h->glueForms |= GLUE_COST_TAIL;
+    if (h->dist()) commAllReduce(h, h->dScal.p + S_COST, 1, CT_F64, s);
+    h->tEnd(slot);
+    return;
+  }
   CVD_DISPATCH_KD(c.KD, {
     hipLaunchKernelGGL((k_cost_frames<KD>), dim3(c.L.F), dim3(256), static_cast<size_t>(c.L.B) * 8, s, c.L, x, h->dMedian.p, h->dRegOwner.p, h->dInRange.p,
                        h->dCostFrame.p);
@@ -67,8 +101,7 @@
     });
     HIP_CHECK(hipGetLastError());
   }
-  hipLaunchKernelGGL(k_sum2, dim3(1), dim3(256), 0, s, h->dCostItem.p, (c.L.includeStatic ? c.nItems : 0),
-                     h->dCostFrame.p, c.L.F, h->dScal.p, S_COST);
+  hipLaunchKernelGGL(k_sum2, dim3(1), dim3(256), 0, s, h->dCostItem.p, nItemCosts, h->dCostFrame.p, c.L.F, h->dScal.p, S_COST);
   HIP_CHECK(hipGetLastError());
   if (h->dist()) commAllReduce(h, h->dScal.p + S_COST, 1, CT_F64, s);
   h->tEnd(slot);
@@ -142,7 +175,7 @@
 double evalFull(Ctx& c, const double* x, bool withStats, bool noReadBack) {
   cvd_handle* h = c.h;
   hipStream_t s = h->stream;
-  launchFrameConsts(c, x);
+  ensureFrameConsts(c, x);
   const size_t B = c.L.B;
   const int slot = h->tBegin(KC_ASSEMBLE);
   const bool fast = !h->forceGeneric && c.KS == 0 && fastLoss(c.L);
@@ -257,10 +290,15 @@
     const size_t chunkD = static_cast<size_t>(h->ownChunk()) * B;
     commAllGather(h, h->dHd.p + static_cast<size_t>(h->rank) * chunkD, h->dHd.p, chunkD, CT_F64, s);
     h->tEnd(ct);
+  } else if (h->dbg.lm_glue_unfused == 0) {
+    hipLaunchKernelGGL(k_extract_diag_sum, dim3((c.n + 255) / 256 + 1), dim3(256), 0, s, c.L, h->dH.p, h->dHd.p, h->dCostFrame.p,
+                       h->dScal.p, S_COST);
+    h->glueForms |= GLUE_DIAG_TAIL;
   } else {
     hipLaunchKernelGGL(k_extract_diag, dim3((c.n + 255) / 256), dim3(256), 0, s, c.L, h->dH.p, h->dHd.p);
   }
-  hipLaunchKernelGGL(k_sum2, dim3(1), dim3(256), 0, s, h->dCostFrame.p, c.L.F, h->dCostFrame.p, 0, h->dScal.p, S_COST);
+  if (h->dist() || h->dbg.lm_glue_unfused != 0)
+    hipLaunchKernelGGL(k_sum2, dim3(1), dim3(256), 0, s, h->dCostFrame.p, c.L.F, h->dCostFrame.p, 0, h->dScal.p, S_COST);
   HIP_CHECK(hipGetLastError());
   if (noReadBack) return 0.0;
   if (withStats) {
diff --git a/robust_cvd_amd/csrc/cvd_host.h b/robust_cvd_amd/csrc/cvd_host.h
--- a/robust_cvd_amd/csrc/cvd_host.h
+++ b/robust_cvd_amd/csrc/cvd_host.h
@@ -340,6 +340,9 @@
   DevBuf<unsigned char> dRegCnt;
   RegCache regCache{};
   DevBuf<FrameConst> dFc;
+  const double* fcPoint = nullptr;
+  unsigned long long fcWrites = 0;
+  unsigned long long xWrites[2] = {0, 0};
   DevBuf<int> dFail;
   DevBuf<unsigned long long> dCount;
   double* hScal = nullptr;
@@ -357,6 +360,7 @@
   int sharesF = -1, sharesN = -1;
   bool tailStageRows = false;
   int lastKD = 0;
+  int glueForms = 0;
   int lastProduct[6] = {0, 0, 0, -1, 0, 0};
   int lastAssembly[8] = {0, 0, 0, -1, 0, 0, -1, 0};
   bool tailDisabled = false;
@@ -570,13 +574,23 @@
 void compileTable(cvd_handle* h, const std::vector<int>& range, bool withTriplets = false, bool ignoreStatic = false);
 void orderTable(cvd_handle* h, const Layout& L, int KD);
 double* pinnedStage(cvd_handle* h, int which, size_t n);
-void uploadState(cvd_handle* h, const Layout& L, DevBuf<double>& dst);
+void uploadState(cvd_handle* h, const Layout& L, DevBuf<double>& dst, bool wait = true);
 void downloadState(cvd_handle* h, const Layout& L, const DevBuf<double>& src);
 void buildMask(cvd_handle* h, const Layout& L, const cvd_opt_params& p, ProblemKind kind, const std::vector<int>& range);
 void ensureBuffers(Ctx& c);
 void refreshMedians(cvd_handle* h);
 void launchFrameConsts(const Layout& L, const double* x, FrameConst* fc, hipStream_t s);
 void launchFrameConsts(Ctx& c, const double* x);
+enum : int {
+  GLUE_FC_REUSED = 1,
+  GLUE_COST_TAIL = 2,
+  GLUE_DIAG_TAIL = 4,
+  GLUE_STEP_CLOSE = 8,
+  GLUE_CHAINS = 16
+};
+void ensureFrameConsts(Ctx& c, const double* x);
+void stateWritten(cvd_handle* h, const double* x);
+void frameConstsHold(cvd_handle* h, const double* x);
 void launchFlagToBool(int* flag, hipStream_t s);
 void launchTlRowsInit(cvd_handle* h, const TlStep* tsp, int NT, int groups, int F, unsigned int* counter, int closeScalars, double tol2,
                       hipStream_t s);
@@ -640,7 +654,7 @@
 void launchPoseTemporalInit(Ctx& c, double tol2);
 const TlStep* poseTemporalStepDev(cvd_handle* h);
 void coarseDebug(cvd_handle* h, int32_t* num_unknowns, double* a_c, double* a_c_inverse, int32_t* failed);
-int runPcg(Ctx& c, const double* x, const std::function<void()>& tail = nullptr);
+int runPcg(Ctx& c, const double* x, const std::function<void(int)>& tail = nullptr);
 bool wantsTriplets(const cvd_opt_params& p, ProblemKind kind);
 void bindTriplets(Ctx& c, const cvd_opt_params& p, ProblemKind kind);
 void solve(cvd_handle* h, const cvd_opt_params& p, double depthDeformReg, ProblemKind kind);
diff --git a/robust_cvd_amd/csrc/cvd_matvec.hip b/robust_cvd_amd/csrc/cvd_matvec.hip
--- a/robust_cvd_amd/csrc/cvd_matvec.hip
+++ b/robust_cvd_amd/csrc/cvd_matvec.hip
@@ -36,7 +36,7 @@
 void prepareMatvec(Ctx& c, const double* x) {
   cvd_handle* h = c.h;
   const Layout& L = c.L;
-  launchFrameConsts(c, x);
+  ensureFrameConsts(c, x);
   int nr = 0;
   if (L.scaleRegSqrt > 0.0) nr += L.sregX * L.sregY;
   if (L.focalRegSqrt > 0.0) nr += 1;
diff --git a/robust_cvd_amd/csrc/cvd_pcg.h b/robust_cvd_amd/csrc/cvd_pcg.h
--- a/robust_cvd_amd/csrc/cvd_pcg.h
+++ b/robust_cvd_amd/csrc/cvd_pcg.h
@@ -1,6 +1,7 @@
 #pragma once
 
 #include "cvd_kernels.h"
+#include "cvd_step_stats.h"
 
 namespace cvd {
 
@@ -1124,7 +1125,7 @@
   TAIL_STAMP(4);
 }
 
-inline __global__ __launch_bounds__(64) void k_pcg_close(double* __restrict__ scal, int enqueued, double* __restrict__ hostMirror) {
+__device__ __forceinline__ void pcgCloseBody(double* __restrict__ scal, int enqueued, double* __restrict__ hostMirror) {
   const int lane = threadIdx.x;
   double wz[8], wr[8];
 #pragma unroll
@@ -1144,6 +1145,9 @@
     scal[S_RR] = rr;
   }
 }
+inline __global__ __launch_bounds__(64) void k_pcg_close(double* __restrict__ scal, int enqueued, double* __restrict__ hostMirror) {
+  pcgCloseBody(scal, enqueued, hostMirror);
+}
 
 inline __global__ void k_apply_step(Layout L, int boundDepth0, const double* __restrict__ x, const double* __restrict__ dx,
                              double* __restrict__ xc) {
@@ -1156,6 +1160,38 @@
     if (c >= 7 && c < 7 + L.nD && ((c - 7) % L.N) == 0) v = fmax(v, 0.0);
   }
   xc[i] = v;
+}
+
+inline __global__ __launch_bounds__(256) void k_step_close(Layout L, int G, int boundDepth0, const double* __restrict__ dx,
+                                                    const double* __restrict__ g, const double* __restrict__ r,
+                                                    const double* __restrict__ lam, const double* __restrict__ x,
+                                                    const double* __restrict__ hdiagActive, double* scal,
+                                                    double* __restrict__ part, unsigned int* __restrict__ counter,
+                                                    double* __restrict__ xc, FrameConst* __restrict__ fc, int closeEnqueued,
+                                                    double* __restrict__ hostMirror) {
+  __shared__ double red[7][4];
+  __shared__ int flag;
+  const int block = blockIdx.x;
+  if (block < G) {
+    stepStatsBody<true>(block, G, static_cast<size_t>(L.F) * L.B, dx, g, r, lam, x, hdiagActive, scal, part, counter, red, &flag, L.B,
+                        L.nD, L.N, boundDepth0, xc);
+    return;
+  }
+  if (block == static_cast<int>(gridDim.x) - 1) {
+    if (closeEnqueued > 0 && threadIdx.x < 64) pcgCloseBody(scal, closeEnqueued, hostMirror);
+    return;
+  }
+  const int f = (block - G) * 256 + threadIdx.x;
+  if (f >= L.F) return;
+  double xf[7], x0[7];
+#pragma unroll
+  for (int i = 0; i < 7; ++i) {
+    xf[i] = x[static_cast<size_t>(f) * L.B + i] + dx[static_cast<size_t>(f) * L.B + i];
+    x0[i] = x[i] + dx[i];
+  }
+  FrameConst c;
+  frameConstFromParams(xf, L.intrOpt, L.vFocal, x0, c);
+  fc[f] = c;
 }
 
 inline __global__ __launch_bounds__(1024) void k_tl_rows_init(const TlStep* __restrict__ tsp, int F, double* __restrict__ scal,
diff --git a/robust_cvd_amd/csrc/cvd_precond.hip b/robust_cvd_amd/csrc/cvd_precond.hip
--- a/robust_cvd_amd/csrc/cvd_precond.hip
+++ b/robust_cvd_amd/csrc/cvd_precond.hip
@@ -187,6 +187,7 @@
   HIP_CHECK(hipMemsetAsync(failOut, 0, sizeof(int), s));
   {
     launchFrameConsts(c.L, x, fcBuf, s);
+    if (fcBuf == h->dFc.p) frameConstsHold(h, x);
     HIP_CHECK(hipMemsetAsync(C.edges.p, 0, static_cast<size_t>(std::max(C.nEdges, 1)) * kCBB * sizeof(double), s));
     if (C.sparsified) HIP_CHECK(hipMemsetAsync(C.dropDiag.p, 0, static_cast<size_t>(c.L.F) * kCBB * sizeof(double), s));
     const size_t ldsE = 2 * B * 8 + 2 * sizeof(FrameConst) + 4 * kCBB * 8;
diff --git a/robust_cvd_amd/csrc/cvd_setup.hip b/robust_cvd_amd/csrc/cvd_setup.hip
--- a/robust_cvd_amd/csrc/cvd_setup.hip
+++ b/robust_cvd_amd/csrc/cvd_setup.hip
@@ -1108,7 +1108,7 @@
   return h->hStage[which];
 }
 
-void uploadState(cvd_handle* h, const Layout& L, DevBuf<double>& dst) {
+void uploadState(cvd_handle* h, const Layout& L, DevBuf<double>& dst, bool wait) {
   const size_t nAll = static_cast<size_t>(L.F) * L.B;
   double* x = pinnedStage(h, 1, nAll);
   const int nD = L.nD, nS = L.nS;
@@ -1119,14 +1119,16 @@
     for (int i = 0; i < nS; ++i) xf[7 + nD + i] = h->sparams[static_cast<size_t>(f) * nS + i];
   }
   dst.upload(x, nAll, h->stream);
-  HIP_CHECK(hipStreamSynchronize(h->stream));
+  h->fcPoint = nullptr;
+  if (&dst == &h->dX) ++h->xWrites[0];
+  if (wait) HIP_CHECK(hipStreamSynchronize(h->stream));
 }
 
 void downloadState(cvd_handle* h, const Layout& L, const DevBuf<double>& src) {
   const size_t nAll = static_cast<size_t>(L.F) * L.B;
   double* x = pinnedStage(h, 0, nAll);
   src.download(x, nAll, h->stream);
-  HIP_CHECK(hipStreamSynchronize(h->stream));
+  if (h->dbg.lm_glue_unfused != 0) HIP_CHECK(hipStreamSynchronize(h->stream)); else spinStream(h->stream);
   const int nD = L.nD, nS = L.nS;
   for (int f = 0; f < L.F; ++f) {
     const double* xf = &x[static_cast<size_t>(f) * L.B];
@@ -1139,7 +1141,7 @@
 void buildMask(cvd_handle* h, const Layout& L, const cvd_opt_params& p, ProblemKind kind,
                       const std::vector<int>& range) {
   const size_t nAll = static_cast<size_t>(L.F) * L.B;
-  HIP_CHECK(hipStreamSynchronize(h->stream));
+  if (h->dbg.lm_glue_unfused != 0) HIP_CHECK(hipStreamSynchronize(h->stream)); else spinStream(h->stream);
   double* m = pinnedStage(h, 0, nAll);
   std::fill(m, m + nAll, 0.0);
   for (int f : range) {
diff --git a/robust_cvd_amd/csrc/cvd_solve.hip b/robust_cvd_amd/csrc/cvd_solve.hip
--- a/robust_cvd_amd/csrc/cvd_solve.hip
+++ b/robust_cvd_amd/csrc/cvd_solve.hip
@@ -18,8 +18,8 @@
 namespace {
 struct TailStalled {};
 }
-static int runPcgAttempt(Ctx& c, const double* x, const std::function<void()>& tail);
-int runPcg(Ctx& c, const double* x, const std::function<void()>& tail) {
+static int runPcgAttempt(Ctx& c, const double* x, const std::function<void(int)>& tail);
+int runPcg(Ctx& c, const double* x, const std::function<void(int)>& tail) {
   const size_t firstTimerSlot = c.h->evUsed;
   try {
     return runPcgAttempt(c, x, tail);
@@ -40,7 +40,7 @@
     return runPcgAttempt(c, x, tail);
   }
 }
-static int runPcgAttempt(Ctx& c, const double* x, const std::function<void()>& tail) {
+static int runPcgAttempt(Ctx& c, const double* x, const std::function<void(int)>& tail) {
   cvd_handle* h = c.h;
   hipStream_t s = h->stream;
   const int F = c.L.F;
@@ -215,7 +215,8 @@
     }
   }
   h->curPcgIter = -1;
-  if (shares && enq > 0) launchPcgClose(c, enq);
+  const bool tailCloses = shares && enq > 0 && tail && !ownerMode && h->dbg.lm_glue_unfused == 0;
+  if (shares && enq > 0 && !tailCloses) launchPcgClose(c, enq);
   if (ownerMode) {
     const int ct = h->tBegin(KC_COMM_PRODUCT);
     const size_t chunk = static_cast<size_t>(h->ownChunk()) * B;
@@ -225,7 +226,7 @@
     commGroupEnd(h);
     h->tEnd(ct);
   }
-  if (tail) tail();
+  if (tail) tail(tailCloses ? enq : 0);
   readScalars(c);
   if (h->hScal[S_DONE] == 2.0) throw std::runtime_error("PCG produced NaN");
   const int iters = static_cast<int>(h->hScal[S_ITERS]);
@@ -307,7 +308,7 @@
   }
   buildMask(h, c.L, p, kind, range);
   phase("mask");
-  uploadState(h, c.L, h->dX);
+  uploadState(h, c.L, h->dX,  h->dbg.lm_glue_unfused != 0);
   phase("upload");
 }
 
@@ -323,6 +324,17 @@
     for (int k = c.L.firstFrame; k < c.L.lastFrame - 1; ++k)
       blocks += (h->tableRange[k] && h->tableRange[k + 1] && h->tableRange[k + 2]) ? 1 : 0;
   return blocks;
+}
+
+void launchStepClose(Ctx& c, int closeEnqueued) {
+  cvd_handle* h = c.h;
+  const int G = static_cast<int>(std::min<size_t>(128, (c.n + 511) / 512));
+  h->dStatPart.ensure(7 * 128);
+  hipLaunchKernelGGL(k_step_close, dim3(G + (c.L.F + 255) / 256 + 1), dim3(256), 0, h->stream, c.L, G, c.boundDepth0, h->dDx.p,
+                     h->dG.p, h->dR.p, h->dLam.p, h->dX.p, h->dHd.p, h->dScal.p, h->dStatPart.p, h->dCounters.p + 2, h->dXc.p,
+                     h->dFc.p, closeEnqueued, h->hPcg);
+  HIP_CHECK(hipGetLastError());
+  h->glueForms |= GLUE_STEP_CLOSE;
 }
 
 struct PendingGuard {
@@ -439,6 +451,7 @@
   bindProblem(bound, h, p, depthDeformReg, kind, range, BindMode{ true,  true,  true}, phase);
   Ctx& c = bound.c;
   hipStream_t s = h->stream;
+  h->glueForms = h->dbg.lm_glue_unfused != 0 ? GLUE_CHAINS : 0;
   HIP_CHECK(hipMemsetAsync(h->dDx.p, 0, c.n * sizeof(double), s));
   HIP_CHECK(hipMemsetAsync(h->dR.p, 0, c.n * sizeof(double), s));
   HIP_CHECK(hipMemsetAsync(h->dFail.p, 0, sizeof(int), s));
@@ -488,11 +501,18 @@
       scaleDone = true;
       buildLevels(c, schedule.decide(levels), guard);
       const double tPcgStart = nowSeconds();
-      const int cgIters = runPcg(c, h->dX.p, [&]() {
-        enqueueStats(c);
-        hipLaunchKernelGGL(k_apply_step, dim3((c.n + 255) / 256), dim3(256), 0, s, c.L, c.boundDepth0, h->dX.p,
-                           h->dDx.p, h->dXc.p);
-        HIP_CHECK(hipGetLastError());
+      const int cgIters = runPcg(c, h->dX.p, [&](int closeEnqueued) {
+        if (h->dbg.lm_glue_unfused == 0) {
+          launchStepClose(c, closeEnqueued);
+          stateWritten(h, h->dXc.p);
+          frameConstsHold(h, h->dXc.p);
+        } else {
+          enqueueStats(c);
+          hipLaunchKernelGGL(k_apply_step, dim3((c.n + 255) / 256), dim3(256), 0, s, c.L, c.boundDepth0, h->dX.p,
+                             h->dDx.p, h->dXc.p);
+          HIP_CHECK(hipGetLastError());
+          stateWritten(h, h->dXc.p);
+        }
         enqueueCost(c, h->dXc.p);
       });
       notePcgTime(h, nowSeconds() - tPcgStart, cgIters);
@@ -534,6 +554,7 @@
       if (rec.relative_decrease > Ceres::min_relative_decrease) {
         std::swap(h->dX.p, h->dXc.p);
         std::swap(h->dX.n, h->dXc.n);
+        std::swap(h->xWrites[0], h->xWrites[1]);
         schedule.accepted(std::abs(xCost - candCost) / std::max(std::abs(xCost), 1e-300));
         xCost = candCost;
         te = nowSeconds();
diff --git a/robust_cvd_amd/csrc/cvd_step_stats.h b/robust_cvd_amd/csrc/cvd_step_stats.h
--- /dev/null
+++ b/robust_cvd_amd/csrc/cvd_step_stats.h
@@ -0,0 +1,76 @@
+#pragma once
+
+#include "cvd_kernels.h"
+
+namespace cvd {
+
+template <bool APPLY>
+__device__ __forceinline__ void stepStatsBody(int block, int G, size_t n, const double* __restrict__ dx, const double* __restrict__ g,
+                                              const double* __restrict__ r, const double* __restrict__ lam,
+                                              const double* __restrict__ x, const double* __restrict__ hdiagActive,
+                                              double* __restrict__ scal, double* __restrict__ part, unsigned int* __restrict__ counter,
+                                              double (*red)[4], int* flag, int B, int nD, int N, int boundDepth0,
+                                              double* __restrict__ xc) {
+  constexpr int NQ = 7;
+  double a[NQ] = {0, 0, 0, 0, 0, 0, 0};
+  for (size_t i = static_cast<size_t>(block) * 256 + threadIdx.x; i < n; i += static_cast<size_t>(G) * 256) {
+    const double d = dx[i];
+    a[0] += d * g[i];
+    a[1] += d * r[i];
+    a[2] += d * lam[i] * d;
+    a[3] += d * d;
+    if constexpr (APPLY) {
+      const double xi = x[i];
+      if (hdiagActive[i] != 0.0) { a[4] += xi * xi; a[6] += 1.0; }
+      double v = xi + d;
+      if (boundDepth0) {
+        const int c = static_cast<int>(i % B);
+        if (c >= 7 && c < 7 + nD && ((c - 7) % N) == 0) v = fmax(v, 0.0);
+      }
+      xc[i] = v;
+    } else {
+      if (hdiagActive[i] != 0.0) { a[4] += x[i] * x[i]; a[6] += 1.0; }
+    }
+    a[5] = fmax(a[5], fabs(g[i]));
+  }
+#pragma unroll
+  for (int k = 0; k < NQ; ++k)
+    if (k != 5) a[k] = waveSum(a[k]);
+#pragma unroll
+  for (int off = 32; off > 0; off >>= 1) a[5] = fmax(a[5], __shfl_xor(a[5], off, 64));
+  if ((threadIdx.x & 63) == 0)
+    for (int k = 0; k < NQ; ++k) red[k][threadIdx.x >> 6] = a[k];
+  __syncthreads();
+  if (threadIdx.x < NQ) {
+    const int k = threadIdx.x;
+    part[k * G + block] = (k != 5) ? (red[k][0] + red[k][1]) + (red[k][2] + red[k][3])
+                                   : fmax(fmax(red[5][0], red[5][1]), fmax(red[5][2], red[5][3]));
+  }
+  if (!lastBlockArrives(counter, G, flag)) return;
+  double t[NQ] = {0, 0, 0, 0, 0, 0, 0};
+  for (int b = threadIdx.x; b < G; b += 256) {
+#pragma unroll
+    for (int k = 0; k < NQ; ++k)
+      if (k != 5) t[k] += part[k * G + b];
+    t[5] = fmax(t[5], part[5 * G + b]);
+  }
+#pragma unroll
+  for (int k = 0; k < NQ; ++k)
+    if (k != 5) t[k] = waveSum(t[k]);
+#pragma unroll
+  for (int off = 32; off > 0; off >>= 1) t[5] = fmax(t[5], __shfl_xor(t[5], off, 64));
+  if ((threadIdx.x & 63) == 0)
+    for (int k = 0; k < NQ; ++k) red[k][threadIdx.x >> 6] = t[k];
+  __syncthreads();
+  if (threadIdx.x == 0) {
+    scal[S_DG] = red[0][0] + red[0][1] + red[0][2] + red[0][3];
+    scal[S_DR] = red[1][0] + red[1][1] + red[1][2] + red[1][3];
+    scal[S_DLD] = red[2][0] + red[2][1] + red[2][2] + red[2][3];
+    scal[S_DD] = red[3][0] + red[3][1] + red[3][2] + red[3][3];
+    scal[S_XX] = red[4][0] + red[4][1] + red[4][2] + red[4][3];
+    scal[S_GMAX] = fmax(fmax(red[5][0], red[5][1]), fmax(red[5][2], red[5][3]));
+    scal[S_NACTIVE] = red[6][0] + red[6][1] + red[6][2] + red[6][3];
+  }
+}
+
+}
diff --git a/robust_cvd_amd/csrc/cvd_temporal.hip b/robust_cvd_amd/csrc/cvd_temporal.hip
--- a/robust_cvd_amd/csrc/cvd_temporal.hip
+++ b/robust_cvd_amd/csrc/cvd_temporal.hip
@@ -214,6 +214,7 @@
     HIP_CHECK(hipStreamWaitEvent(s, T.evIn, 0));
   }
   launchFrameConsts(L, x, fcBuf, s);
+  if (fcBuf == h->dFc.p) frameConstsHold(h, x);
   const size_t ldsD = static_cast<size_t>(L.nD) * T.S * 8 + static_cast<size_t>(T.width) * T.S * 5 + 16;
   allowLds(k_tl_diag, ldsD);
   hipLaunchKernelGGL(k_tl_diag, dim3(L.F), dim3(256), ldsD, s, L, h->dH.p, h->dLam.p, h->dMask.p, tb, T.Cf.p,
```

Result: no change. 362.0, median of 3 (+0.6%).
